# Kyaw-Thiha/animal-vision

Hardware: AMD Instinct MI355X
Metric: megapixels/sec per-frame pipeline (higher is better)
Workload: dtype f16

## Files before the change

### animal-vision_amd/_lib.py

```python
from __future__ import annotations

import ctypes
import os

_HERE = os.path.dirname(os.path.abspath(__file__))
LIB_PATH = os.path.join(_HERE, "libavx.so")

AVX_OK = 0
AVX_ERR_INVALID, AVX_ERR_NO_DEVICE, AVX_ERR_HIP, AVX_ERR_UNSUPPORTED, AVX_ERR_NOMEM = -1, -2, -3, -4, -5
AVX_COLOR_MATRIX, AVX_COLOR_CAT_MERGE = 0, 1
AVX_POST_NONE, AVX_POST_GAUSS, AVX_POST_ROWGAIN, AVX_POST_STREAK = 0, 1, 2, 3
AVX_MAX_KSIZE = 33
AVX_PIX_FMTS = {"yuv420p": 0, "nv12": 1, "yuv422p": 2, "yuv444p": 3, "gray": 4, "yuv420p10le": 5, "yuv422p10le": 6, "yuv444p10le": 7,
                "p010le": 8}
AVX_TRANSFERS = {"pq": 1, "hlg": 2}
AVX_TONEMAPS = {"clip": 0, "mobius": 1}


class AvxError(RuntimeError):
    def __init__(self, code: int, msg: str):
        super().__init__(f"libavx error {code}: {msg}")
        self.code = code


# ... 182 lines not shown
    _fields_ = [("op", ctypes.c_uint8), ("dst", ctypes.c_uint8), ("a", ctypes.c_uint8), ("b", ctypes.c_uint8), ("imm", ctypes.c_uint32)]


class EwPlane(ctypes.Structure):
    _fields_ = [("ptr", ctypes.c_void_p), ("stride", ctypes.c_int32), ("kind", ctypes.c_int32)]


class EwProgram(ctypes.Structure):

    _fields_ = [
        ("struct_size", ctypes.c_uint32),
        ("H", ctypes.c_int32),
        ("W", ctypes.c_int32),
        ("n_insn", ctypes.c_int32),
        ("insn_host", ctypes.POINTER(EwInsn)),
        ("n_planes", ctypes.c_int32),
        ("planes_host", ctypes.POINTER(EwPlane)),
        ("n_acc", ctypes.c_int32),
        ("acc_host", ctypes.POINTER(ctypes.c_int32)),
        ("scalars_dev", ctypes.c_void_p),
        ("n_scalars", ctypes.c_int32),
    ]


AVX_EW_MAX_INSN, AVX_EW_MAX_PLANES, AVX_EW_MAX_REGS, AVX_EW_MAX_ACC = 384, 24, 32, 16
AVX_EW_MAX_FRAMES = 16
_EW_OPS = ("CONST SCALAR LOAD STORE ADD SUB MUL DIV MIN MAX POW ATAN2 NEG ABS SQRT EXP LOG SIN COS FLOOR CEIL CLIP01 TANH "
           "LT LE GT GE EQ AND OR NOT SELECT ACCMIN ACCMAX ACCSUM").split()
EW = {name: i + 1 for i, name in enumerate(_EW_OPS)}
EW_PLANE = {"f32": 0, "u8": 1, "u8_lut": 2, "col": 3, "row": 4, "u8_enc": 5}
EW_ACC = {"min": 0, "max": 1, "sum": 2, "mean": 3}

AVX_MAP = {"falsecolor": 0, "custom_matrix": 1, "opponent": 2, "uv_purple_yellow": 3, "falsecolor_uv_mixed": 4}

if not os.path.exists(LIB_PATH):
    raise ImportError(
        f"{LIB_PATH} not found: build it with `python -c 'import __graft_entry__ as g; g.build()'` "
        "or `make -C animal-vision_amd/csrc` (hipcc --offload-arch=gfx950). There is no CPU fallback."
    )


def _preload_torch_hip_runtime():
    import importlib.util

    try:
        spec = importlib.util.find_spec("torch")
    except (ImportError, ValueError):
        spec = None
    if spec is None or not spec.submodule_search_locations:
        return
    cand = os.path.join(list(spec.submodule_search_locations)[0], "lib", "libamdhip64.so")
    if os.path.exists(cand):
        try:
            ctypes.CDLL(cand, mode=ctypes.RTLD_GLOBAL)
        except OSError:
            pass


_preload_torch_hip_runtime()
lib = ctypes.CDLL(LIB_PATH)

_vp, _i, _sz = ctypes.c_void_p, ctypes.c_int, ctypes.c_size_t
_SIGS = {
    "avx_abi_version": (_i, []),
    "avx_device_count": (_i, []),
    "avx_init": (_i, [_i, ctypes.POINTER(_vp)]),
    "avx_destroy": (None, [_vp]),
    "avx_last_error": (ctypes.c_char_p, [_vp]),
    "avx_malloc": (_i, [_vp, _sz, ctypes.POINTER(_vp)]),
    "avx_free": (_i, [_vp, _vp]),
    "avx_host_alloc": (_i, [_vp, _sz, ctypes.POINTER(_vp)]),
    "avx_host_free": (_i, [_vp, _vp]),
    "avx_memcpy_h2d": (_i, [_vp, _vp, _vp, _sz, _vp]),
    "avx_memcpy_d2h": (_i, [_vp, _vp, _vp, _sz, _vp]),
    "avx_memcpy_d2d": (_i, [_vp, _vp, _vp, _sz, _vp]),
    "avx_memset": (_i, [_vp, _vp, _i, _sz, _vp]),
    "avx_stream_create": (_i, [_vp, ctypes.POINTER(_vp)]),
    "avx_stream_destroy": (_i, [_vp, _vp]),
    "avx_sync": (_i, [_vp, _vp]),
    "avx_stream_wait": (_i, [_vp, _vp, _vp]),
    "avx_device_sync": (_i, [_vp]),
    "avx_timer_start": (_i, [_vp, _vp]),
    "avx_timer_stop": (_i, [_vp, _vp, ctypes.POINTER(ctypes.c_float)]),
    "avx_dichromat_u8": (_i, [_vp, _vp, _vp, _i, _i, _i, ctypes.POINTER(DichromatDesc), _vp]),
    "avx_dichromat_last_launch": (_i, [_vp, ctypes.POINTER(DichromatLaunchInfo)]),
    "avx_get_table": (_i, [_i, _vp, _sz]),
    "avx_percentile": (_i, [_vp, _vp, _sz, ctypes.c_double, ctypes.POINTER(ctypes.c_double), _vp]),
    "avx_spectral_integrate": (_i, [_vp, _vp, _i, _i, _i, _i, _i, _vp, _i, _vp, _vp, _vp]),
    "avx_plane_stats": (_i, [_vp, _vp, _i, _sz, _i, ctypes.c_float, _vp, _vp]),
    "avx_planes_gaussian_blur": (_i, [_vp, _vp, _vp, _i, _i, _i, _i, _vp, _i, _vp]),
    "avx_planes_gaussian_blur_batch": (_i, [_vp, _vp, _sz, _vp, _sz, _i, _i, _i, _i, _i, _vp, _i, _vp]),
    "avx_streak_planes_f32": (_i, [_vp, _vp, _vp, _i, _i, _vp, _i, _vp]),
    "avx_rgb_to_hsi_lobes": (_i, [_vp, _vp, _i, _i, _i, _i, _vp, ctypes.c_float, _vp, _vp]),
    "avx_honeybee_u8": (_i, [_vp, _vp, _vp, _i, _i, _i, ctypes.POINTER(HoneybeeDesc), _vp, _vp]),
    "avx_catch_planes_up": (_i, [_vp, _vp, _i, _i, _vp, _i, _i, _vp, ctypes.POINTER(ctypes.c_int), _vp]),
    "avx_uv_front_u8": (_i, [_vp, _vp, _i, _i, _i, _vp, _vp, _vp]),
    "avx_uv_front_u8_batch": (_i, [_vp, _vp, _i, _sz, _i, _i, _i, _vp, _sz, _vp, _sz, _vp]),
    "avx_panorama_warp_f32": (_i, [_vp, _vp, _i, _i, _i, _vp, _vp]),
    "avx_band_stack": (_i, [_vp, _vp, _i, _i, ctypes.POINTER(BandStackDesc), _vp, _vp]),
    "avx_band_stack_batch": (_i, [_vp, _vp, _i, _sz, _i, _i, ctypes.POINTER(BandStackDesc), _vp, _sz, _vp]),
    "avx_percentile_dev": (_i, [_vp, _vp, _sz, ctypes.c_double, _vp, _vp]),
    "avx_percentiles_dev": (_i, [_vp, _i, ctypes.POINTER(ctypes.c_void_p), ctypes.POINTER(ctypes.c_size_t), ctypes.POINTER(ctypes.c_double),
                                 ctypes.POINTER(ctypes.c_void_p), _vp]),
    "avx_ew_run": (_i, [_vp, ctypes.POINTER(EwProgram), _vp]),
    "avx_ew_run_batch": (_i, [_vp, ctypes.POINTER(EwProgram), _i, ctypes.POINTER(ctypes.c_size_t), _sz, _vp]),
    "avx_ew_spec_stats": (_i, [ctypes.POINTER(ctypes.c_ulonglong), ctypes.POINTER(ctypes.c_ulonglong)]),
    "avx_mantis_u8": (_i, [_vp, _vp, _vp, _vp, _i, _i, ctypes.POINTER(MantisDesc), _vp]),
    "avx_mantis_u8_batch": (_i, [_vp, _vp, _vp, _vp, _i, _i, _i, ctypes.POINTER(MantisDesc), _vp]),
    "avx_resize_hwc": (_i, [_vp, _vp, _i, _i, _i, _i, _vp, _i, _i, _i, _vp]),
    "avx_binocular_warp_u8": (_i, [_vp, _vp, _i, _i, _vp, _vp, _vp, _vp, _vp, _i, _i, _vp, _vp]),
    "avx_cat_wide_u8": (_i, [_vp, _vp, _vp, _i, _i, _i, ctypes.POINTER(DichromatDesc), _vp, _vp, _vp, _vp, _vp, _vp]),
    "avx_center_zoom_u8": (_i, [_vp, _vp, _vp, _i, _i, _i, _i, _i, _i, _i, _vp]),
    "avx_split_compose_u8": (_i, [_vp, _vp, _vp, _vp, _i, _i, _i, _vp]),
    "avx_draw_label_u8": (_i, [_vp, _vp, _i, _i, ctypes.POINTER(ctypes.c_int), _fp, _i, ctypes.c_float, ctypes.c_float, _i, _vp]),
    "avx_gallery_compose_u8": (_i, [_vp, ctypes.POINTER(GalleryTile), _i, _fp, _i, _i, _i, _i, ctypes.POINTER(ctypes.c_int), _vp, _i, _i, _vp]),
    "avx_wall_max_tiles": (_i, []),
    "avx_wall_layout_create": (_i, [_vp, _i, _i, _i, _i, _i, ctypes.POINTER(ctypes.c_int), ctypes.POINTER(ctypes.c_int), _fp, _i, _i, _i, _i,
                                    ctypes.POINTER(ctypes.c_int), ctypes.POINTER(_vp)]),
    "avx_wall_layout_destroy": (_i, [_vp, _vp]),
    "avx_wall_canvas_size": (_i, [_vp, ctypes.POINTER(_i), ctypes.POINTER(_i)]),
    "avx_wall_layout_info": (_i, [_vp, ctypes.POINTER(_i), ctypes.POINTER(_i), ctypes.POINTER(_i), ctypes.POINTER(_sz)]),
    "avx_wall_compose_u8": (_i, [_vp, _vp, ctypes.POINTER(_vp), _sz, _i, _vp, _sz, _vp]),
    "avx_i420_to_rgb_u8": (_i, [_vp, _vp, _vp, _i, _i, _i, _i, _i, _vp]),
    "avx_rgb_to_i420_u8": (_i, [_vp, _vp, _vp, _i, _i, _i, _i, _i, _vp]),
    "avx_yuv_coefficients": (_i, [_i, _i, ctypes.POINTER(ctypes.c_int), ctypes.POINTER(ctypes.c_int)]),
    "avx_yuv_coefficients_d": (_i, [_i, _i, _i, ctypes.POINTER(ctypes.c_int), ctypes.POINTER(ctypes.c_int)]),
    "avx_yuv_frame_size": (_sz, [_i, _i, _i]),
    "avx_yuv_to_rgb_u8": (_i, [_vp, _i, _vp, _vp, _i, _i, _i, _i, _i, _vp]),
    "avx_rgb_to_yuv_u8": (_i, [_vp, _i, _vp, _vp, _i, _i, _i, _i, _i, _vp]),
    "avx_yuv_hdr_to_rgb_u8": (_i, [_vp, _i, _vp, _vp, _i, _i, _i, _i, _i, _i, ctypes.c_double, ctypes.c_double, _vp]),
    "avx_yuv_to_rgb_scaled_u8": (_i, [_vp, _i, _vp, _vp, _i, _i, _i, _i, _i, _i, _i, _vp]),
    "avx_yuv_hdr_to_rgb_scaled_u8": (_i, [_vp, _i, _vp, _vp, _i, _i, _i, _i, _i, _i, _i, _i, ctypes.c_double, ctypes.c_double, _vp]),
    "avx_frame_metrics_u8": (_i, [_vp, _vp, _vp, _i, _i, _i, _i, _vp, _vp]),
    "avx_plane_metrics": (_i, [_vp, _i, _vp, _i, _vp, _i, _i, _i, _i, _vp, _vp]),
    "avx_frame_metrics_ms_u8": (_i, [_vp, _vp, _vp, _i, _i, _i, _vp, _vp, _vp]),
    "avx_diff_map_u8": (_i, [_vp, _vp, _vp, _i, _i, _i, _i, ctypes.c_float, _i, _i, _vp, _vp, _vp, _vp]),
    "avx_delta_e_u8": (_i, [_vp, _vp, _vp, _i, _i, _i, _i, ctypes.c_float, ctypes.c_float, _i, _vp, _vp, _vp, _vp]),
    "avx_scielab_u8": (_i, [_vp, _vp, _vp, _i, _i, _i, ctypes.c_double, _i, ctypes.c_float, ctypes.c_float, _i, _vp, _vp, _vp, _vp]),
    "avx_remap_linear_planes": (_i, [_vp, _vp, _i, _i, _i, _vp, _vp, _vp, ctypes.c_float, _vp]),
    "avx_sobel3_plane": (_i, [_vp, _vp, _i, _i, _vp, _vp, _vp]),
    "avx_mst_gram": (_i, [_vp, _vp, _i, _sz, _i, _i, _vp, _vp, _vp, _vp]),
    "avx_mst_qkv_gram": (_i, [_vp, _vp, _vp, _sz, _i, _vp, _vp, _vp, _vp, _vp]),
    "avx_mst_qkv_gram16": (_i, [_vp, _vp, _vp, _sz, _i, _vp, _vp, _vp, _vp, _vp]),
    "avx_mst_ln_gemm_gelu": (_i, [_vp, _vp, _vp, _vp, ctypes.c_float, _vp, _sz, _i, _vp, _vp]),
    "avx_mst_convt2x2": (_i, [_vp, _vp, _vp, _vp, _vp, _i, _i, _i, _i, _vp]),
    "avx_mst_convt2x2_fuse": (_i, [_vp, _vp, _vp, _vp, _vp, _vp, _vp, _i, _i, _i, _i, _vp]),
    "avx_mst_posemb": (_i, [_vp, _vp, _vp, _vp, _vp, _vp, _vp, _i, _i, _i, _i, _vp]),
    "avx_mst_conv3x3_add": (_i, [_vp, _vp, _vp, _vp, _vp, _i, _i, _i, _i, _vp]),
    "avx_mst_attn_pack": (_i, [_vp, _vp, _vp, _vp, _vp, _vp, _i, _vp, _vp]),
    "avx_mst_rowgemm_add": (_i, [_vp, _vp, _vp, _vp, _vp, _vp, _vp, _sz, _i, _vp]),
    "avx_mst_conv_in_u8": (_i, [_vp, _vp, _i, _i, _i, _i, _i, _i, _vp, _vp, _vp]),
    "avx_mst_conv3x3_lds": (_i, [_vp, _vp, _vp, _vp, _vp, _i, _i, _i, _i, _vp]),
    "avx_mst_down4x4": (_i, [_vp, _vp, _vp, _vp, _i, _i, _i, _i, _vp]),
    "avx_mst_conv3x3_lds_gram": (_i, [_vp, _vp, _vp, _vp, _vp, _i, _i, _i, _vp, _vp, _vp, _vp, _vp]),
    "avx_mst_conv3x3_lds_cin": (_i, [_vp, _vp, _vp, _vp, _i, _i, _i, _i, _i, _i, _vp, _vp, _vp]),
    "avx_mst_conv3x3_lds_spectral_cin": (_i, [_vp, _vp, _vp, _vp, _i, _i, _i, _i, _i, _i, _vp, _fp, _i, _i, _i, _i, _vp, _vp, ctypes.POINTER(ctypes.c_int), _vp]),
    "avx_mst_conv3x3_lds_gram_cin": (_i, [_vp, _vp, _i, _i, _i, _i, _i, _i, _vp, _vp, _vp, _vp, _vp, _vp, _vp, _vp]),
    "avx_mst_convt2x2_fuse_gram": (_i, [_vp, _vp, _vp, _vp, _vp, _vp, _vp, _i, _i, _i, _vp, _vp, _vp, _vp, _vp]),
    "avx_mst_attn_pack16": (_i, [_vp, _vp, _vp, _vp, _vp, _vp, _i, _vp, _vp]),
    "avx_mst_attn_pack_mx": (_i, [_vp, _vp, _vp, _vp, _vp, _vp, _i, _vp, _vp]),
    "avx_mst_attn_tail_mx": (_i, [_vp, _vp, _vp, _vp, _vp, _vp, _vp, _vp, _i, _i, _i, _i, _vp]),
    "avx_mst_attn_tail_sp": (_i, [_vp, _vp, _vp, _vp, _vp, _vp, _vp, _vp, _i, _i, _i, _i, _vp]),
    "avx_mst_attn_tail": (_i, [_vp, _vp, _vp, _vp, _vp, _vp, _vp, _vp, _i, _i, _i, _i, _vp]),
    "avx_mst_attn_tail_x": (_i, [_vp, _vp, _vp, _vp, _vp, _vp, _vp, _vp, _i, _i, _i, _i, _vp]),
    "avx_mst_ffn_fused": (_i, [_vp, _vp, _vp, _vp, ctypes.c_float, _vp, _vp, _vp, _vp, _i, _i, _i, _i, _vp]),
    "avx_mst_conv3x3_lds_spectral": (_i, [_vp, _vp, _vp, _vp, _i, _i, _i, _fp, _i, _i, _i, _i, _vp, _vp, ctypes.POINTER(ctypes.c_int), _vp]),
    "avx_mst_ffn_fused_mx": (_i, [_vp, _vp, _vp, _vp, ctypes.c_float, _vp, _vp, _vp, _vp, _i, _i, _i, _i, _vp]),
    "avx_mst_ffn_fused_sp": (_i, [_vp, _vp, _vp, _vp, ctypes.c_float, _vp, _vp, _vp, _vp, _i, _i, _i, _i, _vp]),
    "avx_mst_ffn_fused_mx_col": (_i, [_vp, _vp, _vp, _vp, ctypes.c_float, _vp, _vp, _vp, _vp, _i, _i, _i, _i, _i, _vp]),
    "avx_mst_ffn_fused_sp_col": (_i, [_vp, _vp, _vp, _vp, ctypes.c_float, _vp, _vp, _vp, _vp, _i, _i, _i, _i, _i, _vp]),
    "avx_mst_gelu_prescale": (ctypes.c_float, []),
    "avx_mst_tile_order": (_i, [_i, _i, _i, _i, _i, ctypes.POINTER(ctypes.c_longlong), _i, ctypes.POINTER(ctypes.c_int)]),
    "avx_mst_tile_order_col": (_i, [_i, _i, _i, _i, ctypes.POINTER(ctypes.c_longlong), ctypes.POINTER(ctypes.c_ubyte), _i, ctypes.POINTER(ctypes.c_int)]),
    "avx_mst_dw_gemm_add": (_i, [_vp, _vp, _vp, _vp, _vp, _vp, _i, _i, _i, _i, _vp]),
    "avx_dwconv3x3_nhwc_add": (_i, [_vp, _vp, _vp, _vp, _i, _i, _i, _i, _i, _vp, _vp, _vp]),
    "avx_dwconv3x3_nhwc": (_i, [_vp, _vp, _vp, _vp, _i, _i, _i, _i, _i, _i, _vp]),
    "avx_layernorm_rows": (_i, [_vp, _vp, _vp, _vp, _vp, _i, _sz, _i, ctypes.c_float, _vp]),
    "avx_layernorm_rows_grouped": (_i, [_vp, _vp, _vp, _vp, _vp, _i, _sz, _i, ctypes.c_float, _i, _i, _vp]),
}
for _name, (_res, _args) in _SIGS.items():
    _fn = getattr(lib, _name)
    _fn.restype = _res
    _fn.argtypes = _args

if lib.avx_abi_version() != 1:
    raise ImportError(f"libavx.so ABI {lib.avx_abi_version()} != 1 expected by this package: rebuild")
```

### animal-vision_amd/csrc/mst_fused.hip

```cpp
#include <hip/hip_fp16.h>

#include <cstdio>
#include <cstdlib>
#include <cstring>

#include "avx_internal.h"
#include "mst_common.h"
#include "mst_tile_order.h"

namespace {

typedef float float4_t __attribute__((ext_vector_type(4)));
#ifndef AVX_FFN32_GM2
#define AVX_FFN32_GM2 1
#endif
constexpr int kFT = 512;
constexpr int TS = 16;
constexpr int HS = TS + 2;
#ifndef AVX_FFN_TH
#define AVX_FFN_TH 16
#endif
constexpr int kFfnTH = AVX_FFN_TH;
static_assert(kFfnTH == 14 || kFfnTH == 16, "FeedForward tile rows");
constexpr int kFfnNGRP = (HS * (kFfnTH + 2) + 31) / 32;
// ... 1201 lines not shown
                for (int k = 0; k < 5; ++k) rraw[k] = (h && k == 4) ? 0u : rraw[k] & 0xffffffu;
                conv_in_mfma(rraw, __builtin_bit_cast(half8_t, cwl[lane]), __builtin_bit_cast(half8_t, cwl[64 + lane]), ar);
            }
            if (ahead.live) {
                if constexpr (CINR) fetch_res(tile_at(ahead, TS, TS));
                if constexpr (CINX) fetch_src(tile_at(ahead, TS, TS));
                else fetch(tile_at(ahead, TS, TS));
            }
            const size_t off = ((t.b * H + (live ? yo : 0)) * (size_t)W + (live ? xo : 0)) * C + 16 * h;
            if constexpr (!CIN) {
                if (add) { ar[0] = reinterpret_cast<const uint4*>(add + off)[0]; ar[1] = reinterpret_cast<const uint4*>(add + off)[1]; }
            }
            float16_t d;
#pragma unroll
            for (int v = 0; v < 16; ++v) d[v] = 0.f;
            const unsigned char* src = xt + (size_t)r * RP + (size_t)c * PP + 16 * h;
#pragma unroll
            for (int tap = 0; tap < 9; ++tap)
#pragma unroll
                for (int s2 = 0; s2 < 2; ++s2)
                    d = mfma16(__builtin_bit_cast(half8_t, wl[(2 * tap + s2) * 64 + lane]), __builtin_bit_cast(half8_t, *reinterpret_cast<const uint4*>(src + (size_t)(tap / 3) * RP + (size_t)(tap % 3) * PP + 32 * s2)), d);
            half8_t o0, o1;
            {
                const half8_t r0 = __builtin_bit_cast(half8_t, ar[0]), r1 = __builtin_bit_cast(half8_t, ar[1]);
#pragma unroll
                for (int v = 0; v < 8; ++v) { o0[v] = (_Float16)(d[v] + (float)r0[v]); o1[v] = (_Float16)(d[8 + v] + (float)r1[v]); }
            }
            if constexpr (SPEC) {
                float a3[3] = {0.f, 0.f, 0.f};
                auto chain = [&]() {
#pragma unroll
                    for (int j = 0; j < 16; ++j) {
                        const float v = (float)(j < 8 ? o0[j] : o1[j - 8]);
                        const float* wb = specw + (16 * h + j) * 4;
#pragma unroll
                        for (int k = 0; k < 3; ++k) a3[k] = __builtin_fmaf(v, wb[k], a3[k]);
                    }
                };
                if (h == 0) chain();
#pragma unroll
                for (int k = 0; k < 3; ++k) { const float lo = __shfl_xor(a3[k], 32); a3[k] = h ? lo : a3[k]; }
                if (h == 1) chain();
                const int yc = yo - crop_t, xc = xo - crop_l;
                if (h == 1 && live && yc >= 0 && yc < Hc && xc >= 0 && xc < Wc) {
#pragma unroll
                    for (int k = 0; k < 3; ++k) {
                        planes[(size_t)k * Hc * Wc + (size_t)yc * Wc + xc] = a3[k];
                        smn[k] = fminf(smn[k], a3[k]); smx[k] = fmaxf(smx[k], a3[k]); ssum[k] += (double)a3[k];
                    }
                }
            } else if (live) {
                reinterpret_cast<uint4*>(out + off)[0] = __builtin_bit_cast(uint4, o0);
                reinterpret_cast<uint4*>(out + off)[1] = __builtin_bit_cast(uint4, o1);
            }
            if constexpr (GRAM) {
                if (!live) { o0 = half8_t{0, 0, 0, 0, 0, 0, 0, 0}; o1 = o0; }
                float16_t dq, dk;
#pragma unroll
                for (int v = 0; v < 16; ++v) { dq[v] = 0.f; dk[v] = 0.f; }
                dq = mfma16(o0, __builtin_bit_cast(half8_t, wq[0 * 64 + lane]), dq);
                dq = mfma16(o1, __builtin_bit_cast(half8_t, wq[1 * 64 + lane]), dq);
                dk = mfma16(o0, __builtin_bit_cast(half8_t, wq[2 * 64 + lane]), dk);
                dk = mfma16(o1, __builtin_bit_cast(half8_t, wq[3 * 64 + lane]), dk);
                unsigned aq[8], ak[8];
#pragma unroll
                for (int j = 0; j < 8; ++j) {
                    aq[j] = pack_f16(dq[2 * j], dq[2 * j + 1]);
                    ak[j] = pack_f16(dk[2 * j], dk[2 * j + 1]);
                    fma_mix_lo(nq, aq[j], aq[j]); fma_mix_hi(nq, aq[j], aq[j]);
                    fma_mix_lo(nk, ak[j], ak[j]); fma_mix_hi(nk, ak[j], ak[j]);
                }
#pragma unroll
                for (int b2 = 0; b2 < 2; ++b2)
                    G = mfma16(__builtin_bit_cast(half8_t, uint4{ak[4 * b2], ak[4 * b2 + 1], ak[4 * b2 + 2], ak[4 * b2 + 3]}),
                               __builtin_bit_cast(half8_t, uint4{aq[4 * b2], aq[4 * b2 + 1], aq[4 * b2 + 2], aq[4 * b2 + 3]}), G);
            }
        }
        if (!ahead.live) break;
        t = tile_at(ahead, TS, TS);
        ahead.advance();
        __syncthreads();
    }
    if constexpr (SPEC) {
        __syncthreads();
        float* redf = reinterpret_cast<float*>(xt);
        double* redd = reinterpret_cast<double*>(xt + 256);
#pragma unroll
        for (int k = 0; k < 3; ++k) {
            float a = smn[k], b2 = smx[k];
            double c2 = ssum[k];
#pragma unroll
            for (int o = 32; o > 0; o >>= 1) { a = fminf(a, __shfl_xor(a, o)); b2 = fmaxf(b2, __shfl_xor(b2, o)); c2 += __shfl_xor(c2, o); }
            if (lane == 0) { redf[(wave * 3 + k) * 2] = a; redf[(wave * 3 + k) * 2 + 1] = b2; redd[wave * 3 + k] = c2; }
        }
        __syncthreads();
        if (tid < 3) {
            float a = 3.4e38f, b2 = -3.4e38f;
            double c2 = 0.0;
            for (int w8 = 0; w8 < 8; ++w8) { a = fminf(a, redf[(w8 * 3 + tid) * 2]); b2 = fmaxf(b2, redf[(w8 * 3 + tid) * 2 + 1]); c2 += redd[w8 * 3 + tid]; }
            spart[(size_t)blockIdx.x * 3 + tid] = SpecStat3{a, b2, c2};
        }
    }
    if constexpr (GRAM) {
        static_assert(sizeof(xt) >= sizeof(float) * 4 * 34 * 32, "the halo tile's LDS holds four waves' results at a time");
        float* red = reinterpret_cast<float*>(xt);
        const float sq = nq + __shfl_xor(nq, 32), sk = nk + __shfl_xor(nk, 32);
        float sum[3] = {0.f, 0.f, 0.f};
#pragma unroll
        for (int half = 0; half < 2; ++half) {
            __syncthreads();
            if ((wave >> 2) == half) {
                float* mine = red + (size_t)(wave & 3) * 34 * 32;
#pragma unroll
                for (int v = 0; v < 16; ++v) mine[(8 * (v / 4) + 4 * h + (v % 4)) * 32 + p] = G[v];
                if (h == 0) { mine[32 * 32 + p] = sq; mine[33 * 32 + p] = sk; }
            }
            __syncthreads();
#pragma unroll
            for (int q = 0; q < 3; ++q) {
                const int i = tid + q * kFT;
                if (i < 34 * 32)
#pragma unroll
                    for (int w4 = 0; w4 < 4; ++w4) sum[q] += red[(size_t)w4 * 34 * 32 + i];
            }
        }
#pragma unroll
        for (int q = 0; q < 3; ++q) {
            const int i = tid + q * kFT;
            if (i < 34 * 32) partial[(size_t)blockIdx.x * 34 * 32 + i] = sum[q];
        }
    }
}


template <int C>
struct DownGeo {
    static constexpr int OH = C == 32 ? 8 : 4, OW = 16, IH = 2 * OH + 2, IW = 2 * OW + 2;
    static constexpr int NP = C / 8;
    static constexpr int RPS = IW * NP + (C == 32 ? 2 : 4);
    static constexpr int NI = ((IH * RPS + 63) / 64 + 7) / 8 * 8;
    static constexpr int PER_WAVE = NI / 8, BUF = NI * 1024, NBUF = C == 32 ? 3 : 2, GROUPS = OH / 2;
    static constexpr int PART = C == 32 ? 0 : 2 * 4 * 4096;
    __device__ static int swz(int col) { return C == 32 ? (col >> 2) & 3 : (col >> 1) & 7; }
};
#pragma clang diagnostic push
#pragma clang diagnostic ignored "-Winline-asm"
__device__ __forceinline__ void lds_dma16(const void* g, unsigned lds_base ) {
    asm volatile("s_mov_b32 m0, %0\n\ts_nop 0\n\tglobal_load_lds_dwordx4 %1, off" ::"s"(__builtin_amdgcn_readfirstlane(lds_base)), "v"(g) : "memory", "m0");
}
__device__ __forceinline__ void lds_dma16(const void* base , unsigned ofs, unsigned lds_base) {
    asm volatile("s_mov_b32 m0, %0\n\ts_nop 0\n\tglobal_load_lds_dwordx4 %1, %2" ::"s"(__builtin_amdgcn_readfirstlane(lds_base)), "v"(ofs), "s"(base) : "memory", "m0");
}
#pragma clang diagnostic pop
template <int C>
__global__ __launch_bounds__(kFT, 2) void k_mst_down4x4_dma(const __half* __restrict__ x , const uint4* __restrict__ wpack ,
                                                            __half* __restrict__ out , const void* __restrict__ zero, int B, int H, int W, int order ) {
    using G = DownGeo<C>;
    constexpr int CO = 2 * C, NT = CO / 32, KS = C / 16;
    __shared__ __align__(1024) unsigned char lds[G::NBUF * G::BUF + G::PART];
    const int tid = threadIdx.x, lane = tid & 63, wave = __builtin_amdgcn_readfirstlane(tid >> 6) , p = lane & 31, h = lane >> 5;
    const int g0 = C == 32 ? wave & 3 : 0, nt = C == 32 ? wave >> 2 : wave & 3, kh = C == 32 ? 0 : wave >> 2;
    half8_t wf[32];
#pragma unroll
    for (int i = 0; i < 32; ++i) {
        const int tap = C == 32 ? i >> 1 : 8 * kh + (i >> 2), s2 = C == 32 ? i & 1 : i & 3;
        wf[i] = __builtin_bit_cast(half8_t, wpack[((size_t)(tap * NT + nt) * KS + s2) * 64 + lane]);
    }
    const int Ho = H / 2, Wo = W / 2;
    const int tx = (Wo + G::OW - 1) / G::OW, ty = (Ho + G::OH - 1) / G::OH;
    struct T2 { int ox0, oy0, b; };
    auto tile_at = [&](const TileWalk& w) { return T2{w.xi * G::OW, w.yi * G::OH, w.b}; };
    int rel[G::PER_WAVE], rc[G::PER_WAVE];
#pragma unroll
    for (int k = 0; k < G::PER_WAVE; ++k) {
        const int L = (wave + 8 * k) * 64 + lane, row = L / G::RPS, rem = L - row * G::RPS, col = rem / G::NP, j = (rem - col * G::NP) ^ G::swz(col);
        const bool inside = row < G::IH && col < G::IW;
        rel[k] = inside ? (row * W + col) * (C * 2) + 16 * j : 0;
        rc[k] = inside ? row << 8 | col : -1;
    }
    const unsigned lds0 = __builtin_amdgcn_readfirstlane((unsigned)(size_t)(__attribute__((address_space(3))) unsigned char*)lds);
    auto fill = [&](const TileWalk& w, int slot) {
        const bool exists = w.live;
        const T2 t = tile_at(w);
        const int y0 = 2 * t.oy0 - 1, x0 = 2 * t.ox0 - 1;
        const char* origin = reinterpret_cast<const char*>(x) + (((long)t.b * H + y0) * W + x0) * (long)(C * 2);
        const unsigned lb = lds0 + slot * G::BUF + wave * 1024;
        if (exists && y0 >= 0 && y0 + G::IH <= H && x0 >= 0 && x0 + G::IW <= W) {
#pragma unroll
            for (int k = 0; k < G::PER_WAVE; ++k) lds_dma16(origin , (unsigned)rel[k], lb + k * 8192);
        } else {
#pragma unroll
            for (int k = 0; k < G::PER_WAVE; ++k) {
                const int yy = y0 + (rc[k] >> 8), xx = x0 + (rc[k] & 255);
                const bool ok = exists && rc[k] >= 0 && yy >= 0 && yy < H && xx >= 0 && xx < W;
                lds_dma16(ok ? (const void*)(origin + rel[k]) : zero, lb + k * 8192);
            }
        }
    };
    TileWalk walk, look;
    walk.init(blockIdx.x, gridDim.x, B, ty, tx, order);
    if (!walk.live) return;
    look = walk;
#pragma unroll
    for (int a = 0; a < G::NBUF - 1; ++a) { fill(look, a); look.advance(); }
    const int c2 = 2 * (p & 15);
    int colofs[4];
#pragma unroll
    for (int kx = 0; kx < 4; ++kx) colofs[kx] = (c2 + kx) * G::NP;
    int slot = 0, plain_stores = 0;
    for (;;) {
        if (plain_stores == G::NBUF - 1 && (C == 32 || kh == 0)) asm volatile("s_waitcnt vmcnt(%0)" ::"n"(G::PER_WAVE * (G::NBUF - 2) + 2 * (C == 32 ? 1 : G::GROUPS) * (G::NBUF - 1)) : "memory");
        else asm volatile("s_waitcnt vmcnt(%0)" ::"n"(G::PER_WAVE * (G::NBUF - 2)) : "memory");
        __syncthreads();
        {
            int nslot = slot + G::NBUF - 1;
            nslot -= nslot >= G::NBUF ? G::NBUF : 0;
            fill(look, nslot);
            look.advance();
        }
        const T2 t = tile_at(walk);
        const bool whole = t.oy0 + G::OH <= Ho && t.ox0 + G::OW <= Wo;
        const unsigned char* bt = lds + slot * G::BUF;
#pragma unroll 1
        for (int g = g0; g < (C == 32 ? g0 + 1 : G::GROUPS); ++g) {
            const int r = 2 * g + (p >> 4);
            float16_t d, d1;
#pragma unroll
            for (int v = 0; v < 16; ++v) d[v] = 0.f, d1[v] = 0.f;
            const unsigned char* src = bt + (size_t)(2 * r) * (G::RPS * 16);
            auto frag = [&](int i) {
                const int tap = C == 32 ? i >> 1 : 8 * kh + (i >> 2), s2 = C == 32 ? i & 1 : i & 3, ky = tap >> 2, kx = tap & 3;
                return *reinterpret_cast<const uint4*>(src + ky * (G::RPS * 16) + (colofs[kx] + ((2 * s2 + h) ^ G::swz(c2 + kx))) * 16);
            };
            constexpr int AHEAD = 6;
            uint4 bq[AHEAD];
#pragma unroll
            for (int i = 0; i < AHEAD; ++i) bq[i] = frag(i);
#pragma unroll
            for (int i = 0; i < 32; ++i) {
                if (i & 1) d1 = mfma16(wf[i], __builtin_bit_cast(half8_t, bq[i % AHEAD]), d1);
                else d = mfma16(wf[i], __builtin_bit_cast(half8_t, bq[i % AHEAD]), d);
                if (i + AHEAD < 32) bq[i % AHEAD] = frag(i + AHEAD);
            }
            __builtin_amdgcn_sched_group_barrier(0x100, AHEAD, 0);
#pragma unroll
            for (int i = 0; i < 32; ++i) {
                __builtin_amdgcn_sched_group_barrier(0x008, 1, 0);
                if (i + AHEAD < 32) __builtin_amdgcn_sched_group_barrier(0x100, 1, 0);
            }
#pragma unroll
            for (int v = 0; v < 16; ++v) d[v] += d1[v];
            if constexpr (C == 64) {
                float4* part = reinterpret_cast<float4*>(lds + G::NBUF * G::BUF + ((g & 1) * 4 + nt) * 4096);
                if (kh == 1) {
#pragma unroll
                    for (int v4 = 0; v4 < 4; ++v4) part[v4 * 64 + lane] = float4{d[4 * v4], d[4 * v4 + 1], d[4 * v4 + 2], d[4 * v4 + 3]};
                }
                __syncthreads();
                if (kh == 1) continue;
#pragma unroll
                for (int v4 = 0; v4 < 4; ++v4) {
                    const float4 q = part[v4 * 64 + lane];
                    d[4 * v4] += q.x; d[4 * v4 + 1] += q.y; d[4 * v4 + 2] += q.z; d[4 * v4 + 3] += q.w;
                }
            }
            const int yo = t.oy0 + r, xo = t.ox0 + (p & 15);
            half8_t o0, o1;
#pragma unroll
            for (int v = 0; v < 8; ++v) { o0[v] = (_Float16)d[v]; o1[v] = (_Float16)d[8 + v]; }
            __half* dst = out + (((size_t)t.b * Ho + yo) * Wo + xo) * CO + 32 * nt + 16 * h;
            if (whole) {
                reinterpret_cast<uint4*>(dst)[0] = __builtin_bit_cast(uint4, o0);
                reinterpret_cast<uint4*>(dst)[1] = __builtin_bit_cast(uint4, o1);
            } else if (yo < Ho && xo < Wo) {
                reinterpret_cast<uint4*>(dst)[0] = __builtin_bit_cast(uint4, o0);
                reinterpret_cast<uint4*>(dst)[1] = __builtin_bit_cast(uint4, o1);
            }
        }
        plain_stores = whole ? (plain_stores < G::NBUF - 1 ? plain_stores + 1 : plain_stores) : 0;
        walk.advance();
        if (!walk.live) break;
        slot = slot + 1 == G::NBUF ? 0 : slot + 1;
    }
    asm volatile("s_waitcnt vmcnt(0)" ::: "memory");
}

__global__ __launch_bounds__(256) void k_mst_conv_in_u8(const uint8_t* __restrict__ frame , const float* __restrict__ w ,
                                                        __half* __restrict__ out , int H, int W, int pt, int pl, int Hp, int Wp) {
    __shared__ __align__(16) float wl[27 * 32];
    for (int i = threadIdx.x; i < 27 * 32; i += 256) wl[i] = w[i];
    __syncthreads();
    const size_t total = (size_t)Hp * Wp;
    for (size_t i = (size_t)blockIdx.x * 256 + threadIdx.x; i < total; i += (size_t)gridDim.x * 256) {
        const int y = (int)(i / Wp), x = (int)(i - (size_t)y * Wp);
        float in[27];
#pragma unroll
        for (int t = 0; t < 9; ++t) {
            const int yy = y + t / 3 - 1, xx = x + t % 3 - 1;
            const bool ok = yy >= 0 && yy < Hp && xx >= 0 && xx < Wp;
            int sy = (ok ? yy : 0) - pt, sx = (ok ? xx : 0) - pl;
            sy = sy < 0 ? -sy : (sy >= H ? 2 * (H - 1) - sy : sy);
            sx = sx < 0 ? -sx : (sx >= W ? 2 * (W - 1) - sx : sx);
            const uint8_t* q = frame + ((size_t)sy * W + sx) * 3;
#pragma unroll
            for (int c = 0; c < 3; ++c) in[3 * t + c] = ok ? (float)(_Float16)((float)q[c] / 255.0f) : 0.f;
        }
        uint4* dst = reinterpret_cast<uint4*>(out + i * 32);
#pragma unroll 1
        for (int v = 0; v < 4; ++v) {
            float acc[8];
#pragma unroll
            for (int j = 0; j < 8; ++j) acc[j] = 0.f;
#pragma unroll
            for (int k = 0; k < 27; ++k) {
                const float4 wa = *reinterpret_cast<const float4*>(wl + k * 32 + 8 * v), wb = *reinterpret_cast<const float4*>(wl + k * 32 + 8 * v + 4);
                acc[0] = __builtin_fmaf(in[k], wa.x, acc[0]); acc[1] = __builtin_fmaf(in[k], wa.y, acc[1]);
                acc[2] = __builtin_fmaf(in[k], wa.z, acc[2]); acc[3] = __builtin_fmaf(in[k], wa.w, acc[3]);
                acc[4] = __builtin_fmaf(in[k], wb.x, acc[4]); acc[5] = __builtin_fmaf(in[k], wb.y, acc[5]);
                acc[6] = __builtin_fmaf(in[k], wb.z, acc[6]); acc[7] = __builtin_fmaf(in[k], wb.w, acc[7]);
            }
            half8_t o8;
#pragma unroll
            for (int j = 0; j < 8; ++j) o8[j] = (_Float16)acc[j];
            dst[v] = __builtin_bit_cast(uint4, o8);
        }
    }
}

__global__ __launch_bounds__(256) void k_mst_conv_in_u8_mfma(const uint8_t* __restrict__ frame , const float* __restrict__ w ,
                                                             __half* __restrict__ out , int H, int W, int pt, int pl, int Hp, int Wp) {
    const int lane = threadIdx.x & 63, p = lane & 31, h = lane >> 5;
    const half8_t a0 = conv_in_afrag(w, lane, 0), a1 = conv_in_afrag(w, lane, 1);
    const ConvInFrame cf{frame, H, W, pt, pl, Hp, Wp};
    const size_t total = (size_t)Hp * Wp, ngroups = (total + 31) / 32;
    for (size_t g = (size_t)blockIdx.x * 4 + (threadIdx.x >> 6); g < ngroups; g += (size_t)gridDim.x * 4) {
        const size_t i = g * 32 + p, ic = i < total ? i : total - 1;
        const int y = (int)(ic / Wp), x = (int)(ic - (size_t)y * Wp);
        unsigned raw[5];
        conv_in_fetch(cf, y, x, h, raw);
        uint4 o[2];
        conv_in_mfma(raw, a0, a1, o);
        if (i < total) {
            reinterpret_cast<uint4*>(out + i * 32 + 16 * h)[0] = o[0];
            reinterpret_cast<uint4*>(out + i * 32 + 16 * h)[1] = o[1];
        }
    }
}

}

static int ffn_fused_launch(avx_ctx* ctx, const void* x, const float* gamma, const float* beta, float eps, const void* w1pack, const void* taps_9xhid, const void* dwpack,
                            const void* w2pack, void* out, int B, int H, int W, int C, void* stream, bool sparse = false, bool march = false, int max_workgroups = 0);

extern "C" float avx_mst_gelu_prescale(void) { return kGeluPrescale; }

extern "C" int avx_mst_tile_order(int frames, int ty, int tx, int nwg, int raster, long long* visit, int steps_cap, int* steps_out) {
    if (frames <= 0 || ty <= 0 || tx <= 0 || nwg <= 0 || (visit && steps_cap <= 0) || (long long)frames * ty * tx > 0x7fffffffll) return AVX_ERR_INVALID;
    int most = 0;
    for (int wg = 0; wg < nwg; ++wg) {
        TileWalk wk;
        wk.init((unsigned)wg, (unsigned)nwg, frames, ty, tx, raster ? AVX_TILE_ORDER_RASTER : AVX_TILE_ORDER_XCD);
        int k = 0;
        for (; wk.live; wk.advance(), ++k)
            if (visit && k < steps_cap) visit[(size_t)wg * steps_cap + k] = ((long long)wk.b * ty + wk.yi) * tx + wk.xi;
        if (visit)
            for (int r = k; r < steps_cap; ++r) visit[(size_t)wg * steps_cap + r] = -1;
        most = k > most ? k : most;
    }
    if (steps_out) *steps_out = most;
    return AVX_OK;
}

extern "C" int avx_mst_tile_order_col(int frames, int ty, int tx, int nwg, long long* visit, unsigned char* seg, int steps_cap, int* steps_out) {
    if (frames <= 0 || ty <= 0 || tx <= 0 || nwg <= 0 || ((visit || seg) && steps_cap <= 0) || (long long)frames * ty * tx > 0x7fffffffll) return AVX_ERR_INVALID;
    int most = 0;
    for (int wg = 0; wg < nwg; ++wg) {
        ColumnWalk wk;
        wk.init((unsigned)wg, (unsigned)nwg, frames, ty, tx);
        int k = 0;
        for (; wk.live; wk.advance(), ++k)
            if (k < steps_cap) {
                if (visit) visit[(size_t)wg * steps_cap + k] = ((long long)wk.b * ty + wk.yi) * tx + wk.xi;
                if (seg) seg[(size_t)wg * steps_cap + k] = wk.seg ? 1 : 0;
            }
        for (int r = k; r < steps_cap; ++r) {
            if (visit) visit[(size_t)wg * steps_cap + r] = -1;
            if (seg) seg[(size_t)wg * steps_cap + r] = 0;
        }
        most = k > most ? k : most;
    }
    if (steps_out) *steps_out = most;
    return AVX_OK;
}

extern "C" int avx_mst_ffn_fused(avx_ctx* ctx, const void* x, const float* gamma, const float* beta, float eps, const void* w1pack, const void* taps_9xhid,
                                 const void* w2pack, void* out, int B, int H, int W, int C, void* stream) {
    if (!ctx) return AVX_ERR_INVALID;
    AVX_REQUIRE(ctx, taps_9xhid, "avx_mst_ffn_fused: NULL pointer");
    return ffn_fused_launch(ctx, x, gamma, beta, eps, w1pack, taps_9xhid, nullptr, w2pack, out, B, H, W, C, stream);
}

extern "C" int avx_mst_ffn_fused_mx(avx_ctx* ctx, const void* x, const float* gamma, const float* beta, float eps, const void* w1pack, const void* dwpack,
                                    const void* w2pack, void* out, int B, int H, int W, int C, void* stream) {
    if (!ctx) return AVX_ERR_INVALID;
    AVX_REQUIRE(ctx, dwpack && (((uintptr_t)dwpack) & 15u) == 0, "avx_mst_ffn_fused_mx: dwpack NULL or not 16-byte aligned");
    return ffn_fused_launch(ctx, x, gamma, beta, eps, w1pack, nullptr, dwpack, w2pack, out, B, H, W, C, stream);
}

extern "C" int avx_mst_ffn_fused_sp(avx_ctx* ctx, const void* x, const float* gamma, const float* beta, float eps, const void* w1pack, const void* dwpack,
                                    const void* w2pack, void* out, int B, int H, int W, int C, void* stream) {
    if (!ctx) return AVX_ERR_INVALID;
    AVX_REQUIRE(ctx, dwpack && (((uintptr_t)dwpack) & 15u) == 0, "avx_mst_ffn_fused_sp: dwpack NULL or not 16-byte aligned");
    return ffn_fused_launch(ctx, x, gamma, beta, eps, w1pack, nullptr, dwpack, w2pack, out, B, H, W, C, stream, true);
}

extern "C" int avx_mst_ffn_fused_mx_col(avx_ctx* ctx, const void* x, const float* gamma, const float* beta, float eps, const void* w1pack, const void* dwpack,
                                        const void* w2pack, void* out, int B, int H, int W, int C, int max_workgroups, void* stream) {
    if (!ctx) return AVX_ERR_INVALID;
    AVX_REQUIRE(ctx, dwpack && (((uintptr_t)dwpack) & 15u) == 0, "avx_mst_ffn_fused_mx_col: dwpack NULL or not 16-byte aligned");
    AVX_REQUIRE(ctx, (C == 32 || C == 64) && max_workgroups >= 0, "avx_mst_ffn_fused_mx_col: C=%d (32 or 64), max_workgroups=%d (>= 0)", C, max_workgroups);
    return ffn_fused_launch(ctx, x, gamma, beta, eps, w1pack, nullptr, dwpack, w2pack, out, B, H, W, C, stream, false, true, max_workgroups);
}
extern "C" int avx_mst_ffn_fused_sp_col(avx_ctx* ctx, const void* x, const float* gamma, const float* beta, float eps, const void* w1pack, const void* dwpack,
                                        const void* w2pack, void* out, int B, int H, int W, int C, int max_workgroups, void* stream) {
    if (!ctx) return AVX_ERR_INVALID;
    AVX_REQUIRE(ctx, dwpack && (((uintptr_t)dwpack) & 15u) == 0, "avx_mst_ffn_fused_sp_col: dwpack NULL or not 16-byte aligned");
    AVX_REQUIRE(ctx, (C == 32 || C == 64) && max_workgroups >= 0, "avx_mst_ffn_fused_sp_col: C=%d (32 or 64), max_workgroups=%d (>= 0)", C, max_workgroups);
    return ffn_fused_launch(ctx, x, gamma, beta, eps, w1pack, nullptr, dwpack, w2pack, out, B, H, W, C, stream, true, true, max_workgroups);
}

static int ffn_fused_launch(avx_ctx* ctx, const void* x, const float* gamma, const float* beta, float eps, const void* w1pack, const void* taps_9xhid, const void* dwpack,
                            const void* w2pack, void* out, int B, int H, int W, int C, void* stream, bool sparse, bool march, int max_workgroups) {
    AVX_REQUIRE(ctx, x && gamma && beta && w1pack && w2pack && out && B > 0 && H > 0 && W > 0, "avx_mst_ffn_fused: NULL pointer or empty tensor");
    AVX_REQUIRE(ctx, C == 32 || C == 64 || C == 128, "avx_mst_ffn_fused: C=%d (32, 64 or 128: 31-channel groups stored 32 wide)", C);
    AVX_REQUIRE(ctx, ((((uintptr_t)x | (uintptr_t)w1pack | (uintptr_t)w2pack | (uintptr_t)out | (uintptr_t)taps_9xhid)) & 15u) == 0,
                "avx_mst_ffn_fused: pointers must be 16-byte aligned");
    AVX_REQUIRE(ctx, x != out, "avx_mst_ffn_fused: neighbouring tiles read each other's halo: the output cannot be the input");
// ... 175 lines not shown
extern "C" int avx_mst_conv3x3_lds_gram(avx_ctx* ctx, const void* x, const void* wpack16, const void* add, void* out, int H, int W, int C, const void* wqk16, float* gram,
                                        float* nq, float* nk, void* stream) {
    if (!ctx) return AVX_ERR_INVALID;
    AVX_REQUIRE(ctx, x && wpack16 && out && wqk16 && gram && nq && nk && H > 0 && W > 0, "avx_mst_conv3x3_lds_gram: NULL pointer or empty tensor");
    AVX_REQUIRE(ctx, C == 32, "avx_mst_conv3x3_lds_gram: C=%d (32: the 31-channel full-resolution convs)", C);
    AVX_REQUIRE(ctx, ((((uintptr_t)x | (uintptr_t)wpack16 | (uintptr_t)add | (uintptr_t)out | (uintptr_t)wqk16)) & 15u) == 0, "avx_mst_conv3x3_lds_gram: pointers must be 16-byte aligned");
    AVX_REQUIRE(ctx, x != out, "avx_mst_conv3x3_lds_gram: in-place convolution is not possible");
    AVX_HIP(ctx, hipSetDevice(ctx->device));
    hipStream_t s = avx_pick_stream(ctx, stream);
    avx_ws* ws = avx_workspace(ctx, s);
    if (!ws) return AVX_ERR_NOMEM;
    const long total = (long)((H + TS - 1) / TS) * ((W + TS - 1) / TS);
    const long cap = (long)ctx->num_cus * 2;
    const long blocks = total < cap ? total : cap;
    int rc = avx_ensure_scratch(ctx, ws, sizeof(float) * (size_t)blocks * 34 * 32);
    if (rc) return rc;
    float* partial = (float*)ws->d_scratch;
    hipLaunchKernelGGL((k_mst_conv3x3_lds<4, true>), dim3((unsigned)blocks), dim3(kFT), 0, s, (const __half*)x, (const uint4*)wpack16, (const __half*)add, (__half*)out, 1, H, W,
                       (const uint4*)wqk16, partial);
    AVX_HIP(ctx, hipGetLastError());
    return avx_mst_qkv_final_launch(ctx, partial, (int)blocks, 1, gram, nq, nk, s);
}

extern "C" int avx_mst_conv_in_u8(avx_ctx* ctx, const uint8_t* frame_hwc, int H, int W, int pad_top, int pad_bottom, int pad_left, int pad_right,
                                  const float* w_27x32_dev, void* out, void* stream) {
    if (!ctx) return AVX_ERR_INVALID;
    AVX_REQUIRE(ctx, frame_hwc && w_27x32_dev && out && H > 1 && W > 1, "avx_mst_conv_in_u8: NULL pointer or a frame too small to reflect");
    AVX_REQUIRE(ctx, pad_top >= 0 && pad_bottom >= 0 && pad_left >= 0 && pad_right >= 0 && pad_top < H && pad_bottom < H && pad_left < W && pad_right < W,
                "avx_mst_conv_in_u8: reflect padding must be smaller than the frame");
    AVX_REQUIRE(ctx, ((uintptr_t)out & 15u) == 0, "avx_mst_conv_in_u8: out must be 16-byte aligned");
    AVX_HIP(ctx, hipSetDevice(ctx->device));
    hipStream_t s = avx_pick_stream(ctx, stream);
    const int Hp = H + pad_top + pad_bottom, Wp = W + pad_left + pad_right;
    const size_t total = (size_t)Hp * Wp;
    const size_t want = (total + 255) / 256, cap = (size_t)ctx->num_cus * 16;
    if (getenv("AVX_MST_CONV_IN_VALU"))
        hipLaunchKernelGGL(k_mst_conv_in_u8, dim3((unsigned)(want < cap ? want : cap)), dim3(256), 0, s, frame_hwc, w_27x32_dev, (__half*)out, H, W, pad_top, pad_left, Hp, Wp);
    else {
        const size_t wantm = (total + 127) / 128;
        hipLaunchKernelGGL(k_mst_conv_in_u8_mfma, dim3((unsigned)(wantm < cap ? wantm : cap)), dim3(256), 0, s, frame_hwc, w_27x32_dev, (__half*)out, H, W, pad_top,
                           pad_left, Hp, Wp);
    }
    AVX_HIP(ctx, hipGetLastError());
    return AVX_OK;
}

static int conv_in_frame_check(avx_ctx* ctx, const char* fn, const uint8_t* frame_hwc, int H, int W, int pad_top, int pad_bottom, int pad_left, int pad_right, const float* w_27x32_dev,
                               ConvInFrame* cf) {
    AVX_REQUIRE(ctx, frame_hwc && w_27x32_dev && H > 1 && W > 1, "%s: NULL pointer or a frame too small to reflect", fn);
    AVX_REQUIRE(ctx, pad_top >= 0 && pad_bottom >= 0 && pad_left >= 0 && pad_right >= 0 && pad_top < H && pad_bottom < H && pad_left < W && pad_right < W,
                "%s: reflect padding must be smaller than the frame", fn);
    AVX_REQUIRE(ctx, (long)(H + pad_top + pad_bottom) * (W + pad_left + pad_right) * 3 < (1l << 31), "%s: frame larger than 2 GiB", fn);
    *cf = ConvInFrame{frame_hwc, H, W, pad_top, pad_left, H + pad_top + pad_bottom, W + pad_left + pad_right};
    return AVX_OK;
}

extern "C" int avx_mst_conv3x3_lds_cin(avx_ctx* ctx, const void* x, const void* wpack16, const uint8_t* frame_hwc, int H, int W, int pad_top, int pad_bottom, int pad_left,
                                       int pad_right, const float* w_27x32_dev, void* out, void* stream) {
    if (!ctx) return AVX_ERR_INVALID;
    AVX_REQUIRE(ctx, x && wpack16 && out, "avx_mst_conv3x3_lds_cin: NULL pointer");
    ConvInFrame cf;
    int rc = conv_in_frame_check(ctx, "avx_mst_conv3x3_lds_cin", frame_hwc, H, W, pad_top, pad_bottom, pad_left, pad_right, w_27x32_dev, &cf);
    if (rc) return rc;
    AVX_REQUIRE(ctx, ((((uintptr_t)x | (uintptr_t)wpack16 | (uintptr_t)out)) & 15u) == 0, "avx_mst_conv3x3_lds_cin: pointers must be 16-byte aligned");
    AVX_REQUIRE(ctx, x != out, "avx_mst_conv3x3_lds_cin: in-place convolution is not possible");
    AVX_HIP(ctx, hipSetDevice(ctx->device));
    hipStream_t s = avx_pick_stream(ctx, stream);
    const long total = (long)((cf.Hp + TS - 1) / TS) * ((cf.Wp + TS - 1) / TS);
    const long cap = (long)ctx->num_cus * 3;
    hipLaunchKernelGGL((k_mst_conv3x3_lds<6, false, false, true>), dim3((unsigned)(total < cap ? total : cap)), dim3(kFT), 0, s, (const __half*)x, (const uint4*)wpack16, (const __half*)nullptr,
                       (__half*)out, 1, cf.Hp, cf.Wp, (const uint4*)nullptr, (float*)nullptr, (const float*)nullptr, (float*)nullptr, (SpecStat3*)nullptr, 0, 0, 0, 0, mst_tile_order(), cf,
                       w_27x32_dev);
    AVX_HIP(ctx, hipGetLastError());
    return AVX_OK;
}

extern "C" int avx_mst_conv3x3_lds_spectral_cin(avx_ctx* ctx, const void* x, const void* wpack16, const uint8_t* frame_hwc, int H, int W, int pad_top, int pad_bottom, int pad_left,
                                                int pad_right, const float* w_27x32_dev, const float* weights_host, int crop_t, int crop_l, int Hc, int Wc, float* planes_out,
                                                void* partials_out, int* n_partials, void* stream) {
    if (!ctx) return AVX_ERR_INVALID;
    AVX_REQUIRE(ctx, x && wpack16 && weights_host && planes_out && partials_out && n_partials, "avx_mst_conv3x3_lds_spectral_cin: NULL pointer");
    ConvInFrame cf;
    int rc = conv_in_frame_check(ctx, "avx_mst_conv3x3_lds_spectral_cin", frame_hwc, H, W, pad_top, pad_bottom, pad_left, pad_right, w_27x32_dev, &cf);
    if (rc) return rc;
    AVX_REQUIRE(ctx, crop_t >= 0 && crop_l >= 0 && Hc > 0 && Wc > 0 && crop_t + Hc <= cf.Hp && crop_l + Wc <= cf.Wp, "avx_mst_conv3x3_lds_spectral_cin: the crop window must lie inside the padded frame");
    AVX_REQUIRE(ctx, ((((uintptr_t)x | (uintptr_t)wpack16 | (uintptr_t)partials_out)) & 15u) == 0, "avx_mst_conv3x3_lds_spectral_cin: pointers must be 16-byte aligned");
    AVX_HIP(ctx, hipSetDevice(ctx->device));
    hipStream_t s = avx_pick_stream(ctx, stream);
    avx_ws* ws = avx_workspace(ctx, s);
    if (!ws) return AVX_ERR_NOMEM;
    float wT[32 * 4];
    for (int b = 0; b < 32; ++b)
        for (int k = 0; k < 4; ++k) wT[b * 4 + k] = k < 3 ? weights_host[(size_t)k * 32 + b] : 0.0f;
    float* dwT = nullptr;
    rc = avx_const_upload(ctx, ws, 2, wT, sizeof(wT), s, (void**)&dwT);
    if (rc) return rc;
    const long total = (long)((cf.Hp + TS - 1) / TS) * ((cf.Wp + TS - 1) / TS);
    const long cap = (long)ctx->num_cus * 2;
    const long blocks = total < cap ? total : cap;
    *n_partials = (int)blocks;
    hipLaunchKernelGGL((k_mst_conv3x3_lds<4, false, true, true>), dim3((unsigned)blocks), dim3(kFT), 0, s, (const __half*)x, (const uint4*)wpack16, (const __half*)nullptr, (__half*)nullptr, 1,
                       cf.Hp, cf.Wp, (const uint4*)nullptr, (float*)nullptr, (const float*)dwT, planes_out, (SpecStat3*)partials_out, crop_t, crop_l, Hc, Wc, (int)AVX_TILE_ORDER_RASTER, cf,
                       w_27x32_dev);
    AVX_HIP(ctx, hipGetLastError());
    return AVX_OK;
}

extern "C" int avx_mst_conv3x3_lds_gram_cin(avx_ctx* ctx, const uint8_t* frame_hwc, int H, int W, int pad_top, int pad_bottom, int pad_left, int pad_right, const float* w_27x32_dev,
                                            const void* wpack16, void* out, const void* wqk16, float* gram, float* nq, float* nk, void* stream) {
    if (!ctx) return AVX_ERR_INVALID;
    AVX_REQUIRE(ctx, wpack16 && out && wqk16 && gram && nq && nk, "avx_mst_conv3x3_lds_gram_cin: NULL pointer");
    ConvInFrame cf;
    int rc = conv_in_frame_check(ctx, "avx_mst_conv3x3_lds_gram_cin", frame_hwc, H, W, pad_top, pad_bottom, pad_left, pad_right, w_27x32_dev, &cf);
    if (rc) return rc;
    AVX_REQUIRE(ctx, ((((uintptr_t)wpack16 | (uintptr_t)out | (uintptr_t)wqk16)) & 15u) == 0, "avx_mst_conv3x3_lds_gram_cin: pointers must be 16-byte aligned");
    AVX_HIP(ctx, hipSetDevice(ctx->device));
    hipStream_t s = avx_pick_stream(ctx, stream);
    avx_ws* ws = avx_workspace(ctx, s);
    if (!ws) return AVX_ERR_NOMEM;
    const long total = (long)((cf.Hp + TS - 1) / TS) * ((cf.Wp + TS - 1) / TS);
    const long cap = (long)ctx->num_cus * 2;
    const long blocks = total < cap ? total : cap;
    rc = avx_ensure_scratch(ctx, ws, sizeof(float) * (size_t)blocks * 34 * 32);
    if (rc) return rc;
    float* partial = (float*)ws->d_scratch;
    hipLaunchKernelGGL((k_mst_conv3x3_lds<4, true, false, false, true>), dim3((unsigned)blocks), dim3(kFT), 0, s, (const __half*)nullptr, (const uint4*)wpack16, (const __half*)nullptr, (__half*)out, 1,
                       cf.Hp, cf.Wp, (const uint4*)wqk16, partial, (const float*)nullptr, (float*)nullptr, (SpecStat3*)nullptr, 0, 0, 0, 0, (int)AVX_TILE_ORDER_RASTER, cf, w_27x32_dev);
    AVX_HIP(ctx, hipGetLastError());
    return avx_mst_qkv_final_launch(ctx, partial, (int)blocks, 1, gram, nq, nk, s);
}

extern "C" int avx_mst_down4x4(avx_ctx* ctx, const void* x, const void* wpack16, void* out, int B, int H, int W, int C, void* stream) {
    if (!ctx) return AVX_ERR_INVALID;
    AVX_REQUIRE(ctx, x && wpack16 && out && B > 0 && H > 0 && W > 0, "avx_mst_down4x4: NULL pointer or empty tensor");
    AVX_REQUIRE(ctx, C == 32 || C == 64, "avx_mst_down4x4: C=%d (32 or 64: the encoder steps 31 -> 62 and 62 -> 124 channels as stored)", C);
    AVX_REQUIRE(ctx, H % 2 == 0 && W % 2 == 0, "avx_mst_down4x4: H and W must be even (the model pads frames to multiples of 8)");
    AVX_REQUIRE(ctx, (long)B * H * W * C * 2 < (1l << 31), "avx_mst_down4x4: input larger than 2 GiB");
    AVX_REQUIRE(ctx, ((((uintptr_t)x | (uintptr_t)wpack16 | (uintptr_t)out)) & 15u) == 0, "avx_mst_down4x4: pointers must be 16-byte aligned");
    AVX_HIP(ctx, hipSetDevice(ctx->device));
    hipStream_t s = avx_pick_stream(ctx, stream);
    const long cap = (long)ctx->num_cus;
    if (C == 32) {
        using G = DownGeo<32>;
        const long total = (long)B * ((H / 2 + G::OH - 1) / G::OH) * ((W / 2 + G::OW - 1) / G::OW);
        hipLaunchKernelGGL(k_mst_down4x4_dma<32>, dim3((unsigned)(total < cap ? total : cap)), dim3(kFT), 0, s, (const __half*)x, (const uint4*)wpack16, (__half*)out, (const void*)ctx->d_zero, B, H, W, mst_tile_order());
    } else {
        using G = DownGeo<64>;
        const long total = (long)B * ((H / 2 + G::OH - 1) / G::OH) * ((W / 2 + G::OW - 1) / G::OW);
        hipLaunchKernelGGL(k_mst_down4x4_dma<64>, dim3((unsigned)(total < cap ? total : cap)), dim3(kFT), 0, s, (const __half*)x, (const uint4*)wpack16, (__half*)out, (const void*)ctx->d_zero, B, H, W, mst_tile_order());
    }
    AVX_HIP(ctx, hipGetLastError());
    return AVX_OK;
}
```

### animal-vision_amd/csrc/mst_mfma.hip

```cpp
#include <hip/hip_fp16.h>

#include "avx_internal.h"
#include "mst_common.h"

namespace {

constexpr int kT = 256;

__device__ __forceinline__ float16_t mfma(half4_t a, half4_t b, float16_t c) { return __builtin_amdgcn_mfma_f32_32x32x8f16(a, b, c, 0, 0, 0); }
__device__ __forceinline__ float16_t mfma16(half8_t a, half8_t b, float16_t c) { return __builtin_amdgcn_mfma_f32_32x32x16_f16(a, b, c, 0, 0, 0); }

template <int C>
__device__ __forceinline__ void load_x(const __half* __restrict__ x, size_t tile, size_t n, int lane, half4_t (&xf)[C / 8]) {
    const int p = lane & 31, h = lane >> 5;
    const size_t row = tile * 32 + p;
    if (row < n) {
        const uint4* src = reinterpret_cast<const uint4*>(x + row * (size_t)C + h * (C / 2));
#pragma unroll
        for (int q = 0; q < C / 16; ++q) {
            const uint4 v = src[q];
            const half8_t h8 = __builtin_bit_cast(half8_t, v);
            xf[2 * q] = half4_t{h8[0], h8[1], h8[2], h8[3]};
            xf[2 * q + 1] = half4_t{h8[4], h8[5], h8[6], h8[7]};
        }
// ... 464 lines not shown
        }
#pragma unroll
        for (int t = 0; t < NT; ++t) {
            float16_t d;
#pragma unroll
            for (int v = 0; v < 16; ++v) d[v] = 0.f;
#pragma unroll
            for (int tap = 0; tap < 9; ++tap)
#pragma unroll
                for (int s = 0; s < KS; ++s) d = mfma(__builtin_bit_cast(half4_t, wl[((tap * NT + t) * KS + s) * 64 + lane]), xf[tap][s], d);
            if (xw < W) {
                const size_t off = ((b * H + y) * (size_t)W + xw) * C + 32 * t + 16 * h;
                half8_t r0 = {0, 0, 0, 0, 0, 0, 0, 0}, r1 = r0;
                if (add) {
                    r0 = __builtin_bit_cast(half8_t, reinterpret_cast<const uint4*>(add + off)[0]);
                    r1 = __builtin_bit_cast(half8_t, reinterpret_cast<const uint4*>(add + off)[1]);
                }
                _Float16 o[16];
#pragma unroll
                for (int v = 0; v < 8; ++v) { o[v] = (_Float16)(d[v] + (float)r0[v]); o[8 + v] = (_Float16)(d[8 + v] + (float)r1[v]); }
                store_tile16(out + off, o);
            }
        }
    }
}

template <int C, int TH, int TW>
__global__ __launch_bounds__(kT) void k_mst_posemb(const __half* __restrict__ v, const float* __restrict__ w1 , const float* __restrict__ w2 ,
                                                   const __half* __restrict__ res, const float* __restrict__ bias , __half* __restrict__ out, int B, int H,
                                                   int W) {
    constexpr int CV = C / 8, PH = TH + 2, PW = TW + 2;
    static_assert(PH % 2 == 0 && kT % CV == 0, "row pairs in phase 1; fixed channel group per thread");
    extern __shared__ __align__(16) unsigned char smem[];
    __half* wl = reinterpret_cast<__half*>(smem);
    float* bl = reinterpret_cast<float*>(wl + 2 * 9 * C);
    unsigned char* mid = reinterpret_cast<unsigned char*>(bl + C);
    const int tid = threadIdx.x;
    for (int i = tid; i < 9 * C; i += kT) { const int c = i / 9, t = i - 9 * c; wl[t * C + c] = __float2half(w1[i]); wl[9 * C + t * C + c] = __float2half(w2[i]); }
    for (int i = tid; i < C; i += kT) bl[i] = bias ? bias[i] : 0.f;
    const int tx = (W + TW - 1) / TW, ty = (H + TH - 1) / TH;
    const long total = (long)B * ty * tx;
    const int cg = tid % CV;
    auto taps = [&](const __half* wbase, uint4 (&wt)[9]) {
#pragma unroll
        for (int t = 0; t < 9; ++t) wt[t] = *reinterpret_cast<const uint4*>(wbase + t * C + cg * 8);
    };
    auto mac8 = [&](float (&acc)[8], const uint4& hv, const uint4& wv) {
        fma_mix_lo(acc[0], hv.x, wv.x); fma_mix_hi(acc[1], hv.x, wv.x);
        fma_mix_lo(acc[2], hv.y, wv.y); fma_mix_hi(acc[3], hv.y, wv.y);
        fma_mix_lo(acc[4], hv.z, wv.z); fma_mix_hi(acc[5], hv.z, wv.z);
        fma_mix_lo(acc[6], hv.w, wv.w); fma_mix_hi(acc[7], hv.w, wv.w);
    };
    __syncthreads();
    for (long tile = blockIdx.x; tile < total; tile += gridDim.x) {
        const int x0 = (int)(tile % tx) * TW, y0 = (int)((tile / tx) % ty) * TH;
        const long b = tile / ((long)tx * ty);
        const bool interior = y0 >= 2 && y0 + TH + 2 <= H && x0 >= 2 && x0 + TW + 2 <= W;
        __syncthreads();
        uint4 wt1[9];
        taps(wl, wt1);
#pragma unroll 1
        for (int it = tid; it < (PH / 2) * PW * CV; it += kT) {
            const int pp = it / CV, c = pp % PW, r = 2 * (pp / PW);
            const int yy = y0 - 1 + r, xx = x0 - 1 + c;
            uint4 raw[4][3];
            if (interior) {
                const __half* base = v + ((b * H + yy - 1) * (size_t)W + xx - 1) * C + cg * 8;
#pragma unroll
                for (int rr = 0; rr < 4; ++rr)
#pragma unroll
                    for (int kx = 0; kx < 3; ++kx) raw[rr][kx] = *reinterpret_cast<const uint4*>(base + ((size_t)rr * W + kx) * C);
            } else {
#pragma unroll
                for (int rr = 0; rr < 4; ++rr)
#pragma unroll
                    for (int kx = 0; kx < 3; ++kx) {
                        const int y2 = yy - 1 + rr, x2 = xx + kx - 1;
                        const bool ok = y2 >= 0 && y2 < H && x2 >= 0 && x2 < W;
                        const int yc = y2 < 0 ? 0 : (y2 >= H ? H - 1 : y2), xc = x2 < 0 ? 0 : (x2 >= W ? W - 1 : x2);
                        uint4 rw = *reinterpret_cast<const uint4*>(v + ((b * H + yc) * (size_t)W + xc) * C + cg * 8);
                        rw.x = ok ? rw.x : 0u; rw.y = ok ? rw.y : 0u; rw.z = ok ? rw.z : 0u; rw.w = ok ? rw.w : 0u;
                        raw[rr][kx] = rw;
                    }
            }
            float acc[2][8];
#pragma unroll
            for (int o2 = 0; o2 < 2; ++o2)
#pragma unroll
                for (int q = 0; q < 8; ++q) acc[o2][q] = 0.f;
#pragma unroll
            for (int rr = 0; rr < 4; ++rr)
#pragma unroll
                for (int kx = 0; kx < 3; ++kx)
#pragma unroll
                    for (int o2 = 0; o2 < 2; ++o2) {
                        const int ky = rr - o2;
                        if (ky < 0 || ky > 2) continue;
                        mac8(acc[o2], raw[rr][kx], wt1[ky * 3 + kx]);
                    }
#pragma unroll
            for (int o2 = 0; o2 < 2; ++o2) {
                const int ym = yy + o2;
                const bool inside = interior || (ym >= 0 && ym < H && xx >= 0 && xx < W);
                unsigned o[4];
#pragma unroll
                for (int q = 0; q < 4; ++q) {
                    const float2_t g = gelu_fast2(float2_t{acc[o2][2 * q], acc[o2][2 * q + 1]});
                    o[q] = inside ? pack_f16(g.x, g.y) : 0u;
                }
                *reinterpret_cast<uint4*>(mid + (((size_t)(r + o2) * PW + c) * C + cg * 8) * 2) = uint4{o[0], o[1], o[2], o[3]};
            }
        }
        __syncthreads();
        uint4 wt2[9];
        taps(wl + 9 * C, wt2);
#pragma unroll 1
        for (int it = tid; it < TH * TW * CV; it += kT) {
            const int pp = it / CV, c = pp % TW, r = pp / TW;
            const int yo = y0 + r, xo = x0 + c;
            if (yo >= H || xo >= W) continue;
            float acc[8];
#pragma unroll
            for (int q = 0; q < 8; ++q) acc[q] = 0.f;
#pragma unroll
            for (int t = 0; t < 9; ++t) mac8(acc, *reinterpret_cast<const uint4*>(mid + (((size_t)(r + t / 3) * PW + c + t % 3) * C + cg * 8) * 2), wt2[t]);
            const size_t off = ((b * H + yo) * (size_t)W + xo) * C + cg * 8;
            uint4 rr = uint4{0u, 0u, 0u, 0u};
            if (res) rr = *reinterpret_cast<const uint4*>(res + off);
            const unsigned rw[4] = {rr.x, rr.y, rr.z, rr.w};
            unsigned o[4];
#pragma unroll
            for (int q = 0; q < 4; ++q) {
                float s0 = acc[2 * q], s1 = acc[2 * q + 1];
                fma_mix_lo(s0, rw[q], 0x3c003c00u); fma_mix_hi(s1, rw[q], 0x3c003c00u);
                o[q] = pack_f16(s0 + bl[cg * 8 + 2 * q], s1 + bl[cg * 8 + 2 * q + 1]);
            }
            *reinterpret_cast<uint4*>(out + off) = uint4{o[0], o[1], o[2], o[3]};
        }
    }
}

template <int C, int TH, int TW>
int launch_posemb(avx_ctx* ctx, const void* v, const float* w1, const float* w2, const void* res, const float* bias, void* out, int B, int H, int W, hipStream_t s) {
    const size_t lds = sizeof(__half) * 2 * 9 * C + sizeof(float) * C + (size_t)(TH + 2) * (TW + 2) * C * 2;
    const long total = (long)B * ((H + TH - 1) / TH) * ((W + TW - 1) / TW);
    const long cap = (long)ctx->num_cus * (lds > 40 * 1024 ? 3 : 5);
    auto k = k_mst_posemb<C, TH, TW>;
    AVX_HIP(ctx, hipFuncSetAttribute((const void*)k, hipFuncAttributeMaxDynamicSharedMemorySize, (int)lds));
    hipLaunchKernelGGL(k, dim3((unsigned)(total < cap ? total : cap)), dim3(kT), lds, s, (const __half*)v, w1, w2, (const __half*)res, bias, (__half*)out, B, H, W);
    AVX_HIP(ctx, hipGetLastError());
    return AVX_OK;
}

template <int C, bool GRAM = false>
__global__ __launch_bounds__(kT) void k_mst_convt2x2(const __half* __restrict__ x , const uint2* __restrict__ wpack ,
                                                     const float* __restrict__ bias , const __half* __restrict__ skip ,
                                                     const uint2* __restrict__ wskip , __half* __restrict__ out , int B,
                                                     int H, int W, const uint4* __restrict__ wqk = nullptr , float* __restrict__ partial = nullptr ) {
    constexpr int KS = C / 8, CO = C / 2, NT = CO / 32, KSS = CO / 8;
    static_assert(!GRAM || C == 64, "the Gram epilogue is for the 32-channel output level");
    extern __shared__ __align__(16) unsigned char smem[];
    uint2* wl = reinterpret_cast<uint2*>(smem);
    float* bl = reinterpret_cast<float*>(smem + (size_t)4 * NT * KS * 64 * sizeof(uint2));
    uint2* wsl = reinterpret_cast<uint2*>(bl + CO);
    uint4* wq = reinterpret_cast<uint4*>(wsl + NT * KSS * 64);
    const int tid = threadIdx.x, lane = tid & 63, wave = tid >> 6;
    for (int i = tid; i < 4 * NT * KS * 64; i += kT) wl[i] = wpack[i];
    for (int i = tid; i < CO; i += kT) bl[i] = bias[i];
    if (skip)
        for (int i = tid; i < NT * KSS * 64; i += kT) wsl[i] = wskip[i];
    float16_t G;
    float nq = 0.f, nk = 0.f;
    if constexpr (GRAM) {
        for (int i = tid; i < 4 * 64; i += kT) wq[i] = wqk[i];
#pragma unroll
        for (int v = 0; v < 16; ++v) G[v] = 0.f;
    }
    __syncthreads();
    const int xt = (W + 31) / 32;
    const long total = (long)B * H * xt;
    const int p = lane & 31, h = lane >> 5;
    for (long tile = (long)blockIdx.x * 4 + wave; tile < total; tile += (long)gridDim.x * 4) {
        const int x0 = (int)(tile % xt) * 32, y = (int)((tile / xt) % H);
        const long b = tile / ((long)xt * H);
        const int xw = x0 + p;
        half4_t xf[KS];
        {
            const size_t row = (size_t)((b * H + y) * (long)W + (xw < W ? xw : W - 1));
            const uint4* src = reinterpret_cast<const uint4*>(x + row * C + h * (C / 2));
#pragma unroll
            for (int q = 0; q < C / 16; ++q) {
                const half8_t h8 = __builtin_bit_cast(half8_t, src[q]);
                xf[2 * q] = half4_t{h8[0], h8[1], h8[2], h8[3]};
                xf[2 * q + 1] = half4_t{h8[4], h8[5], h8[6], h8[7]};
            }
        }
        if constexpr (C > 64) asm volatile("" ::: "memory");
#pragma unroll
        for (int tap = 0; tap < 4; ++tap) {
            const size_t opix = ((size_t)(b * 2 * H + 2 * y + (tap >> 1)) * (size_t)(2 * W) + (size_t)(2 * (xw < W ? xw : W - 1) + (tap & 1)));
            half4_t sf[KSS];
            if (skip) {
                const uint4* src = reinterpret_cast<const uint4*>(skip + opix * CO + h * (CO / 2));
#pragma unroll
                for (int q = 0; q < CO / 16; ++q) {
                    const half8_t h8 = __builtin_bit_cast(half8_t, src[q]);
                    sf[2 * q] = half4_t{h8[0], h8[1], h8[2], h8[3]};
                    sf[2 * q + 1] = half4_t{h8[4], h8[5], h8[6], h8[7]};
                }
            }
#pragma unroll
            for (int t = 0; t < NT; ++t) {
                float16_t d;
#pragma unroll
                for (int v = 0; v < 16; ++v) d[v] = 0.f;
#pragma unroll
                for (int s = 0; s < KS; ++s) d = mfma(__builtin_bit_cast(half4_t, wl[((tap * NT + t) * KS + s) * 64 + lane]), xf[s], d);
                if (skip) {
#pragma unroll
                    for (int s = 0; s < KSS; ++s) d = mfma(__builtin_bit_cast(half4_t, wsl[(t * KSS + s) * 64 + lane]), sf[s], d);
                }
                _Float16 o[16];
#pragma unroll
                for (int v = 0; v < 16; ++v) o[v] = (_Float16)(d[v] + bl[32 * t + 16 * h + v]);
                if (xw < W) store_tile16(out + opix * CO + 32 * t + 16 * h, o);
                if constexpr (GRAM) {
                    half8_t o0, o1;
#pragma unroll
                    for (int v = 0; v < 8; ++v) { o0[v] = xw < W ? o[v] : (_Float16)0.f; o1[v] = xw < W ? o[8 + v] : (_Float16)0.f; }
                    float16_t dq, dk;
#pragma unroll
                    for (int v = 0; v < 16; ++v) { dq[v] = 0.f; dk[v] = 0.f; }
                    dq = mfma16(o0, __builtin_bit_cast(half8_t, wq[0 * 64 + lane]), dq);
                    dq = mfma16(o1, __builtin_bit_cast(half8_t, wq[1 * 64 + lane]), dq);
                    dk = mfma16(o0, __builtin_bit_cast(half8_t, wq[2 * 64 + lane]), dk);
                    dk = mfma16(o1, __builtin_bit_cast(half8_t, wq[3 * 64 + lane]), dk);
                    unsigned aq[8], ak[8];
#pragma unroll
                    for (int j = 0; j < 8; ++j) {
                        aq[j] = pack_f16(dq[2 * j], dq[2 * j + 1]);
                        ak[j] = pack_f16(dk[2 * j], dk[2 * j + 1]);
                        fma_mix_lo(nq, aq[j], aq[j]); fma_mix_hi(nq, aq[j], aq[j]);
                        fma_mix_lo(nk, ak[j], ak[j]); fma_mix_hi(nk, ak[j], ak[j]);
                    }
#pragma unroll
                    for (int b2 = 0; b2 < 2; ++b2)
                        G = mfma16(__builtin_bit_cast(half8_t, uint4{ak[4 * b2], ak[4 * b2 + 1], ak[4 * b2 + 2], ak[4 * b2 + 3]}),
                                   __builtin_bit_cast(half8_t, uint4{aq[4 * b2], aq[4 * b2 + 1], aq[4 * b2 + 2], aq[4 * b2 + 3]}), G);
                }
            }
        }
    }
    if constexpr (GRAM) {
        __syncthreads();
        float* red = reinterpret_cast<float*>(smem);
        float* mine = red + (size_t)wave * 34 * 32;
#pragma unroll
        for (int v = 0; v < 16; ++v) mine[(8 * (v / 4) + 4 * h + (v % 4)) * 32 + p] = G[v];
        const float sq = nq + __shfl_xor(nq, 32), sk = nk + __shfl_xor(nk, 32);
        if (h == 0) { mine[32 * 32 + p] = sq; mine[33 * 32 + p] = sk; }
        __syncthreads();
        for (int i = tid; i < 34 * 32; i += kT) {
            float sum = 0.f;
#pragma unroll
            for (int w4 = 0; w4 < 4; ++w4) sum += red[(size_t)w4 * 34 * 32 + i];
            partial[(size_t)blockIdx.x * 34 * 32 + i] = sum;
        }
    }
}

template <int C, int NW>
__global__ __launch_bounds__(64 * NW) void k_mst_qkv16(const __half* __restrict__ x, const uint4* __restrict__ wpack , size_t n,
                                                      __half* __restrict__ v_out , float* __restrict__ partial ) {
    constexpr int KS = C / 16, HD = C / 32, NT = 3 * HD;
    extern __shared__ __align__(16) unsigned char smem[];
    uint4* wl = reinterpret_cast<uint4*>(smem);
    const int tid = threadIdx.x, lane = tid & 63, wave = tid >> 6;
    for (int i = tid; i < NT * KS * 64; i += 64 * NW) wl[i] = wpack[i];
    __syncthreads();
    auto W = [&](int t, int s) { return __builtin_bit_cast(half8_t, wl[(t * KS + s) * 64 + lane]); };
    float16_t G[HD];
    float nq[HD], nk[HD];
#pragma unroll
    for (int hd = 0; hd < HD; ++hd) {
#pragma unroll
        for (int v = 0; v < 16; ++v) G[hd][v] = 0.f;
        nq[hd] = 0.f;
        nk[hd] = 0.f;
    }
    const size_t ntiles = (n + 31) / 32;
    const int p = lane & 31, h = lane >> 5;
    auto load_row = [&](size_t tile, uint4 (&u)[KS]) {
        const size_t row = tile * 32 + p;
        const uint4* src = reinterpret_cast<const uint4*>(x + (row < n ? row : n - 1) * (size_t)C + h * (C / 2));
#pragma unroll
        for (int q = 0; q < KS; ++q) u[q] = src[q];
    };
    constexpr bool PF = C <= 64;
    uint4 xn[KS];
    size_t tile = (size_t)blockIdx.x * NW + wave;
    if (PF && tile < ntiles) load_row(tile, xn);
    for (; tile < ntiles; tile += (size_t)gridDim.x * NW) {
        const size_t row = tile * 32 + p;
        half8_t xf[KS];
        if (!PF) load_row(tile, xn);
#pragma unroll
        for (int q = 0; q < KS; ++q) xf[q] = __builtin_bit_cast(half8_t, row < n ? xn[q] : uint4{0u, 0u, 0u, 0u});
        if (PF && tile + (size_t)gridDim.x * NW < ntiles) load_row(tile + (size_t)gridDim.x * NW, xn);
        if constexpr (C > 32) asm volatile("" ::: "memory");
#pragma unroll
        for (int hd = 0; hd < HD; ++hd) {
            float16_t dq, dk;
#pragma unroll
            for (int v = 0; v < 16; ++v) { dq[v] = 0.f; dk[v] = 0.f; }
#pragma unroll
            for (int s = 0; s < KS; ++s) dq = mfma16(xf[s], W(hd, s), dq);
#pragma unroll
            for (int s = 0; s < KS; ++s) dk = mfma16(xf[s], W(HD + hd, s), dk);
            unsigned aq[8], ak[8];
#pragma unroll
            for (int j = 0; j < 8; ++j) {
                aq[j] = pack_f16(dq[2 * j], dq[2 * j + 1]);
                ak[j] = pack_f16(dk[2 * j], dk[2 * j + 1]);
                fma_mix_lo(nq[hd], aq[j], aq[j]); fma_mix_hi(nq[hd], aq[j], aq[j]);
                fma_mix_lo(nk[hd], ak[j], ak[j]); fma_mix_hi(nk[hd], ak[j], ak[j]);
            }
#pragma unroll
            for (int b2 = 0; b2 < 2; ++b2)
                G[hd] = mfma16(__builtin_bit_cast(half8_t, uint4{ak[4 * b2], ak[4 * b2 + 1], ak[4 * b2 + 2], ak[4 * b2 + 3]}),
                               __builtin_bit_cast(half8_t, uint4{aq[4 * b2], aq[4 * b2 + 1], aq[4 * b2 + 2], aq[4 * b2 + 3]}), G[hd]);
        }
        if (v_out)
#pragma unroll
        for (int hd = 0; hd < HD; ++hd) {
            float16_t dv;
#pragma unroll
            for (int v = 0; v < 16; ++v) dv[v] = 0.f;
#pragma unroll
            for (int s = 0; s < KS; ++s) dv = mfma16(W(2 * HD + hd, s), xf[s], dv);
            if (row < n) {
                unsigned o[8];
#pragma unroll
                for (int v = 0; v < 8; ++v) o[v] = pack_f16(dv[2 * v], dv[2 * v + 1]);
                uint4* dst = reinterpret_cast<uint4*>(v_out + row * (size_t)C + 32 * hd + 16 * h);
                dst[0] = uint4{o[0], o[1], o[2], o[3]};
                dst[1] = uint4{o[4], o[5], o[6], o[7]};
            }
        }
    }
    __syncthreads();
    float* red = reinterpret_cast<float*>(smem);
#pragma unroll
    for (int hd = 0; hd < HD; ++hd) {
        float* mine = red + ((size_t)wave * HD + hd) * 34 * 32;
#pragma unroll
        for (int v = 0; v < 16; ++v) mine[(8 * (v / 4) + 4 * h + (v % 4)) * 32 + p] = G[hd][v];
        const float sq = nq[hd] + __shfl_xor(nq[hd], 32), sk = nk[hd] + __shfl_xor(nk[hd], 32);
        if (h == 0) { mine[32 * 32 + p] = sq; mine[33 * 32 + p] = sk; }
    }
    __syncthreads();
    for (int i = tid; i < HD * 34 * 32; i += 64 * NW) {
        float s = 0.f;
#pragma unroll
        for (int w = 0; w < NW; ++w) s += red[(size_t)w * HD * 34 * 32 + i];
        partial[(size_t)blockIdx.x * HD * 34 * 32 + i] = s;
    }
}

template <int C, int NW>
int launch_qkv16(avx_ctx* ctx, avx_ws* ws, const void* x, const void* wpack, size_t n, void* v_out, float* gram, float* nq, float* nk, hipStream_t s) {
    constexpr int KS = C / 16, HD = C / 32;
    const size_t wbytes = (size_t)3 * HD * KS * 64 * sizeof(uint4), rbytes = sizeof(float) * NW * HD * 34 * 32;
    const size_t lds = wbytes > rbytes ? wbytes : rbytes;
    const size_t ntiles = (n + 31) / 32;
    long blocks = (long)((ntiles + NW - 1) / NW);
    long per_cu = (long)(160 * 1024 / lds);
    if (per_cu > 16 / NW * 2) per_cu = 16 / NW * 2;
    if (per_cu < 1) per_cu = 1;
    const long cap = (long)ctx->num_cus * per_cu;
    if (blocks > cap) blocks = cap;
    int rc = avx_ensure_scratch(ctx, ws, sizeof(float) * (size_t)blocks * HD * 34 * 32);
    if (rc) return rc;
    float* partial = (float*)ws->d_scratch;
    auto k = k_mst_qkv16<C, NW>;
    AVX_HIP(ctx, hipFuncSetAttribute((const void*)k, hipFuncAttributeMaxDynamicSharedMemorySize, (int)lds));
    hipLaunchKernelGGL(k, dim3((unsigned)blocks), dim3(64 * NW), lds, s, (const __half*)x, (const uint4*)wpack, n, (__half*)v_out, partial);
    AVX_HIP(ctx, hipGetLastError());
    const int tot = HD * 34 * 32;
    hipLaunchKernelGGL(k_mst_qkv_final, dim3((tot / 4 * 64 + 255) / 256), dim3(256), 0, s, partial, (int)blocks, HD, gram, nq, nk);
    AVX_HIP(ctx, hipGetLastError());
    return AVX_OK;
}

template <int C>
int launch_qkv(avx_ctx* ctx, avx_ws* ws, const void* x, const void* wpack, size_t n, void* v_out, float* gram, float* nq, float* nk, hipStream_t s) {
    constexpr int KS = C / 8, HD = C / 32;
    const size_t wbytes = (size_t)3 * HD * KS * 64 * sizeof(uint2), rbytes = sizeof(float) * 4 * HD * 34 * 32;
    const size_t lds = wbytes > rbytes ? wbytes : rbytes;
    const size_t ntiles = (n + 31) / 32;
    long blocks = (long)((ntiles + 3) / 4);
    const long cap = (long)ctx->num_cus * (lds > 64 * 1024 ? 1 : (lds > 32 * 1024 ? 2 : 4));
    if (blocks > cap) blocks = cap;
    int rc = avx_ensure_scratch(ctx, ws, sizeof(float) * (size_t)blocks * HD * 34 * 32);
    if (rc) return rc;
    float* partial = (float*)ws->d_scratch;
    auto k = k_mst_qkv<C>;
    AVX_HIP(ctx, hipFuncSetAttribute((const void*)k, hipFuncAttributeMaxDynamicSharedMemorySize, (int)lds));
    hipLaunchKernelGGL(k, dim3((unsigned)blocks), dim3(kT), lds, s, (const __half*)x, (const uint2*)wpack, n, (__half*)v_out, partial);
    AVX_HIP(ctx, hipGetLastError());
    const int tot = HD * 34 * 32;
    hipLaunchKernelGGL(k_mst_qkv_final, dim3((tot / 4 * 64 + 255) / 256), dim3(256), 0, s, partial, (int)blocks, HD, gram, nq, nk);
    AVX_HIP(ctx, hipGetLastError());
    return AVX_OK;
}

template <int C>
int launch_ffn1(avx_ctx* ctx, const void* x, const float* gamma, const float* beta, float eps, const void* wpack, size_t n, void* out, hipStream_t s) {
    constexpr int KS = C / 8, HD = C / 32;
    const size_t lds = (size_t)4 * HD * KS * 64 * sizeof(uint2) + sizeof(float) * 2 * C;
    const size_t ntiles = (n + 31) / 32;
    long blocks = (long)((ntiles + 3) / 4);
    const long cap = (long)ctx->num_cus * (lds > 64 * 1024 ? 1 : (lds > 32 * 1024 ? 2 : 8));
    if (blocks > cap) blocks = cap;
    auto k = k_mst_ffn1<C>;
    AVX_HIP(ctx, hipFuncSetAttribute((const void*)k, hipFuncAttributeMaxDynamicSharedMemorySize, (int)lds));
    hipLaunchKernelGGL(k, dim3((unsigned)blocks), dim3(kT), lds, s, (const __half*)x, gamma, beta, eps, (const uint2*)wpack, n, (__half*)out);
    AVX_HIP(ctx, hipGetLastError());
    return AVX_OK;
}

template <int C, int ROWS, int PXT, bool PF, int MINW>
int launch_ffn2(avx_ctx* ctx, const void* hid, const float* w9, const void* w2pack, const void* res, void* out, int B, int H, int W, hipStream_t s) {
    constexpr int C4 = 4 * C, KS2 = C4 / 8, NT = C / 32, PITCH = C4 * 2 + 16;
    const size_t lds = (size_t)NT * KS2 * 64 * sizeof(uint2) + sizeof(float) * 9 * C4 + (size_t)ROWS * 32 * PXT * PITCH;
    const long total = (long)B * ((H + ROWS - 1) / ROWS) * ((W + 32 * PXT - 1) / (32 * PXT));
    const long cap = (long)ctx->num_cus * MINW;
    auto k = k_mst_ffn2<C, ROWS, PXT, PF, MINW>;
    AVX_HIP(ctx, hipFuncSetAttribute((const void*)k, hipFuncAttributeMaxDynamicSharedMemorySize, (int)lds));
    hipLaunchKernelGGL(k, dim3((unsigned)(total < cap ? total : cap)), dim3(kT), lds, s, (const __half*)hid, w9, (const uint2*)w2pack, (const __half*)res,
                       (__half*)out, B, H, W);
    AVX_HIP(ctx, hipGetLastError());
    return AVX_OK;
}

}

int avx_mst_qkv_final_launch(avx_ctx* ctx, const float* partial, int blocks, int heads, float* gram, float* nq, float* nk, hipStream_t s) {
    const int tot = heads * 34 * 32;
    hipLaunchKernelGGL(k_mst_qkv_final, dim3((tot / 4 * 64 + 255) / 256), dim3(256), 0, s, partial, blocks, heads, gram, nq, nk);
    AVX_HIP(ctx, hipGetLastError());
    return AVX_OK;
}

extern "C" {

int avx_mst_qkv_gram(avx_ctx* ctx, const void* x, const void* wpack, size_t n_pix, int C, void* v_out, float* gram, float* nq, float* nk, void* stream) {
    if (!ctx) return AVX_ERR_INVALID;
    AVX_REQUIRE(ctx, x && wpack && gram && nq && nk && n_pix > 0, "avx_mst_qkv_gram: NULL pointer or empty tensor");
    AVX_REQUIRE(ctx, C == 32 || C == 64 || C == 128, "avx_mst_qkv_gram: C=%d (32, 64 or 128: 31-channel groups stored 32 wide)", C);
    AVX_REQUIRE(ctx, ((((uintptr_t)x | (uintptr_t)wpack | (uintptr_t)v_out)) & 15u) == 0, "avx_mst_qkv_gram: pointers must be 16-byte aligned");
    AVX_HIP(ctx, hipSetDevice(ctx->device));
    hipStream_t s = avx_pick_stream(ctx, stream);
    avx_ws* ws = avx_workspace(ctx, s);
    if (!ws) return AVX_ERR_NOMEM;
    if (C == 32) return launch_qkv<32>(ctx, ws, x, wpack, n_pix, v_out, gram, nq, nk, s);
    if (C == 64) return launch_qkv<64>(ctx, ws, x, wpack, n_pix, v_out, gram, nq, nk, s);
    return launch_qkv<128>(ctx, ws, x, wpack, n_pix, v_out, gram, nq, nk, s);
}

int avx_mst_qkv_gram16(avx_ctx* ctx, const void* x, const void* wpack16, size_t n_pix, int C, void* v_out, float* gram, float* nq, float* nk, void* stream) {
    if (!ctx) return AVX_ERR_INVALID;
    AVX_REQUIRE(ctx, x && wpack16 && gram && nq && nk && n_pix > 0, "avx_mst_qkv_gram16: NULL pointer or empty tensor");
    AVX_REQUIRE(ctx, C == 32 || C == 64 || C == 128, "avx_mst_qkv_gram16: C=%d (32, 64 or 128: 31-channel groups stored 32 wide)", C);
    AVX_REQUIRE(ctx, ((((uintptr_t)x | (uintptr_t)wpack16 | (uintptr_t)v_out)) & 15u) == 0, "avx_mst_qkv_gram16: pointers must be 16-byte aligned");
    AVX_HIP(ctx, hipSetDevice(ctx->device));
    hipStream_t s = avx_pick_stream(ctx, stream);
    avx_ws* ws = avx_workspace(ctx, s);
    if (!ws) return AVX_ERR_NOMEM;
    if (C == 32) return launch_qkv16<32, 4>(ctx, ws, x, wpack16, n_pix, v_out, gram, nq, nk, s);
    if (C == 64) return launch_qkv16<64, 4>(ctx, ws, x, wpack16, n_pix, v_out, gram, nq, nk, s);
    return launch_qkv16<128, 8>(ctx, ws, x, wpack16, n_pix, v_out, gram, nq, nk, s);
}

int avx_mst_ln_gemm_gelu(avx_ctx* ctx, const void* x, const float* gamma, const float* beta, float eps, const void* wpack, size_t rows, int C, void* out,
                         void* stream) {
    if (!ctx) return AVX_ERR_INVALID;
    AVX_REQUIRE(ctx, x && gamma && beta && wpack && out && rows > 0, "avx_mst_ln_gemm_gelu: NULL pointer or empty tensor");
    AVX_REQUIRE(ctx, C == 32 || C == 64 || C == 128, "avx_mst_ln_gemm_gelu: C=%d (32, 64 or 128: 31-channel groups stored 32 wide)", C);
    AVX_REQUIRE(ctx, ((((uintptr_t)x | (uintptr_t)wpack | (uintptr_t)out)) & 15u) == 0, "avx_mst_ln_gemm_gelu: pointers must be 16-byte aligned");
    AVX_HIP(ctx, hipSetDevice(ctx->device));
    hipStream_t s = avx_pick_stream(ctx, stream);
    if (C == 32) return launch_ffn1<32>(ctx, x, gamma, beta, eps, wpack, rows, out, s);
    if (C == 64) return launch_ffn1<64>(ctx, x, gamma, beta, eps, wpack, rows, out, s);
    return launch_ffn1<128>(ctx, x, gamma, beta, eps, wpack, rows, out, s);
}

int avx_mst_dw_gemm_add(avx_ctx* ctx, const void* hidden, const float* w_c9, const void* w2pack, const void* residual, void* out, int B, int H, int W,
                        int C, void* stream) {
    if (!ctx) return AVX_ERR_INVALID;
    AVX_REQUIRE(ctx, hidden && w_c9 && w2pack && residual && out && B > 0 && H > 0 && W > 0, "avx_mst_dw_gemm_add: NULL pointer or empty tensor");
    AVX_REQUIRE(ctx, C == 32 || C == 64, "avx_mst_dw_gemm_add: C=%d (32 or 64)", C);
    AVX_REQUIRE(ctx, ((((uintptr_t)hidden | (uintptr_t)w2pack | (uintptr_t)residual | (uintptr_t)out)) & 15u) == 0,
                "avx_mst_dw_gemm_add: pointers must be 16-byte aligned");
    AVX_REQUIRE(ctx, hidden != out, "avx_mst_dw_gemm_add: the hidden tensor cannot be the output (the residual can)");
    AVX_HIP(ctx, hipSetDevice(ctx->device));
    hipStream_t s = avx_pick_stream(ctx, stream);
    if (C == 32) return launch_ffn2<32, 2, 2, false, 3>(ctx, hidden, w_c9, w2pack, residual, out, B, H, W, s);
    return launch_ffn2<64, 2, 1, true, 2>(ctx, hidden, w_c9, w2pack, residual, out, B, H, W, s);
}

int avx_mst_rowgemm_add(avx_ctx* ctx, const void* a, const void* wpack, const void* a2, const void* wpack2, const void* add, void* out, size_t rows, int C,
                        void* stream) {
    if (!ctx) return AVX_ERR_INVALID;
    AVX_REQUIRE(ctx, a && wpack && out && rows > 0 && (!a2 == !wpack2), "avx_mst_rowgemm_add: NULL pointer or empty tensor");
    AVX_REQUIRE(ctx, C == 32 || C == 64 || C == 128, "avx_mst_rowgemm_add: C=%d (32, 64 or 128)", C);
    AVX_REQUIRE(ctx, ((((uintptr_t)a | (uintptr_t)wpack | (uintptr_t)a2 | (uintptr_t)wpack2 | (uintptr_t)add | (uintptr_t)out)) & 15u) == 0,
                "avx_mst_rowgemm_add: pointers must be 16-byte aligned");
    AVX_REQUIRE(ctx, a != out && a2 != out, "avx_mst_rowgemm_add: a GEMM operand cannot be the output (the addend can)");
    AVX_HIP(ctx, hipSetDevice(ctx->device));
    hipStream_t s = avx_pick_stream(ctx, stream);
    if (C == 32) return launch_rowgemm_add<32>(ctx, a, wpack, a2, wpack2, add, out, rows, s);
    if (C == 64) return launch_rowgemm_add<64>(ctx, a, wpack, a2, wpack2, add, out, rows, s);
    return launch_rowgemm_add<128>(ctx, a, wpack, a2, wpack2, add, out, rows, s);
}

static int attn_pack_impl(avx_ctx* ctx, const float* gram, const float* nq, const float* nk, const float* rescale, const float* wproj_t, int C, void* mpack,
                          int layout, void* stream) {
    if (!ctx) return AVX_ERR_INVALID;
    AVX_REQUIRE(ctx, gram && nq && nk && rescale && wproj_t && mpack, "avx_mst_attn_pack: NULL pointer");
    AVX_REQUIRE(ctx, C == 32 || C == 64 || C == 128, "avx_mst_attn_pack: C=%d (32, 64 or 128)", C);
    AVX_HIP(ctx, hipSetDevice(ctx->device));
    hipStream_t s = avx_pick_stream(ctx, stream);
    hipLaunchKernelGGL(k_mst_attn_pack, dim3((unsigned)((layout == 2 ? 4 : 1) * C * C / 256)), dim3(256), 0, s, gram, nq, nk, rescale, wproj_t, C, (__half*)mpack, layout);
    AVX_HIP(ctx, hipGetLastError());
    return AVX_OK;
}

int avx_mst_attn_pack(avx_ctx* ctx, const float* gram, const float* nq, const float* nk, const float* rescale, const float* wproj_t, int C, void* mpack,
                      void* stream) {
    return attn_pack_impl(ctx, gram, nq, nk, rescale, wproj_t, C, mpack, 0, stream);
}

int avx_mst_attn_pack16(avx_ctx* ctx, const float* gram, const float* nq, const float* nk, const float* rescale, const float* wproj_t, int C, void* mpack,
                        void* stream) {
    return attn_pack_impl(ctx, gram, nq, nk, rescale, wproj_t, C, mpack, 1, stream);
}

int avx_mst_attn_pack_mx(avx_ctx* ctx, const float* gram, const float* nq, const float* nk, const float* rescale, const float* wproj_t, int C, void* mpack,
                         void* stream) {
    return attn_pack_impl(ctx, gram, nq, nk, rescale, wproj_t, C, mpack, 2, stream);
}

int avx_mst_conv3x3_add(avx_ctx* ctx, const void* x, const void* wpack, const void* add, void* out, int B, int H, int W, int C, void* stream) {
    if (!ctx) return AVX_ERR_INVALID;
    AVX_REQUIRE(ctx, x && wpack && out && B > 0 && H > 0 && W > 0, "avx_mst_conv3x3_add: NULL pointer or empty tensor");
    AVX_REQUIRE(ctx, C == 32, "avx_mst_conv3x3_add: C=%d (32: the 31-channel full-resolution convs)", C);
    AVX_REQUIRE(ctx, ((((uintptr_t)x | (uintptr_t)wpack | (uintptr_t)add | (uintptr_t)out)) & 15u) == 0, "avx_mst_conv3x3_add: pointers must be 16-byte aligned");
    AVX_REQUIRE(ctx, x != out, "avx_mst_conv3x3_add: in-place convolution is not possible");
    AVX_HIP(ctx, hipSetDevice(ctx->device));
    hipStream_t s = avx_pick_stream(ctx, stream);
    constexpr int KS = 4, NT = 1;
    const size_t lds = (size_t)9 * NT * KS * 64 * sizeof(uint2);
    const long total = (long)B * H * ((W + 31) / 32);
    long blocks = (total + 3) / 4;
    const long cap = (long)ctx->num_cus * 8;
    if (blocks > cap) blocks = cap;
    auto k = k_mst_conv3x3<32>;
    AVX_HIP(ctx, hipFuncSetAttribute((const void*)k, hipFuncAttributeMaxDynamicSharedMemorySize, (int)lds));
    hipLaunchKernelGGL(k, dim3((unsigned)blocks), dim3(kT), lds, s, (const __half*)x, (const uint2*)wpack, (const __half*)add, (__half*)out, B, H, W);
    AVX_HIP(ctx, hipGetLastError());
    return AVX_OK;
}

int avx_mst_posemb(avx_ctx* ctx, const void* v, const float* w1_c9, const float* w2_c9, const void* residual, const float* bias, void* out, int B, int H, int W,
                   int C, void* stream) {
    if (!ctx) return AVX_ERR_INVALID;
    AVX_REQUIRE(ctx, v && w1_c9 && w2_c9 && out && B > 0 && H > 0 && W > 0, "avx_mst_posemb: NULL pointer or empty tensor");
    AVX_REQUIRE(ctx, C == 32 || C == 64 || C == 128, "avx_mst_posemb: C=%d (32, 64 or 128)", C);
    AVX_REQUIRE(ctx, ((((uintptr_t)v | (uintptr_t)residual | (uintptr_t)out)) & 15u) == 0, "avx_mst_posemb: pointers must be 16-byte aligned");
    AVX_REQUIRE(ctx, v != out, "avx_mst_posemb: in-place convolution is not possible");
    AVX_HIP(ctx, hipSetDevice(ctx->device));
    hipStream_t s = avx_pick_stream(ctx, stream);
    if (C == 32) return launch_posemb<32, 8, 32>(ctx, v, w1_c9, w2_c9, residual, bias, out, B, H, W, s);
    if (C == 64) return launch_posemb<64, 8, 16>(ctx, v, w1_c9, w2_c9, residual, bias, out, B, H, W, s);
    return launch_posemb<128, 4, 16>(ctx, v, w1_c9, w2_c9, residual, bias, out, B, H, W, s);
}

static int convt2x2_impl(avx_ctx* ctx, const void* x, const void* wpack, const float* bias, const void* skip, const void* wskip, void* out, int B, int H, int W,
                         int C, void* stream);
int avx_mst_convt2x2(avx_ctx* ctx, const void* x, const void* wpack, const float* bias, void* out, int B, int H, int W, int C, void* stream) {
    return convt2x2_impl(ctx, x, wpack, bias, nullptr, nullptr, out, B, H, W, C, stream);
}
int avx_mst_convt2x2_fuse(avx_ctx* ctx, const void* x, const void* wpack, const float* bias, const void* skip, const void* wskip, void* out, int B, int H,
                          int W, int C, void* stream) {
    if (ctx && !(skip && wskip)) return avx_fail(ctx, AVX_ERR_INVALID, "avx_mst_convt2x2_fuse: skip / wskip is NULL");
    if (ctx && ((((uintptr_t)skip | (uintptr_t)wskip)) & 15u)) return avx_fail(ctx, AVX_ERR_INVALID, "avx_mst_convt2x2_fuse: pointers must be 16-byte aligned");
    return convt2x2_impl(ctx, x, wpack, bias, skip, wskip, out, B, H, W, C, stream);
}
int avx_mst_convt2x2_fuse_gram(avx_ctx* ctx, const void* x, const void* wpack, const float* bias, const void* skip, const void* wskip, void* out, int H, int W, int C,
                               const void* wqk16, float* gram, float* nq, float* nk, void* stream) {
    if (!ctx) return AVX_ERR_INVALID;
    AVX_REQUIRE(ctx, x && wpack && bias && skip && wskip && out && wqk16 && gram && nq && nk && H > 0 && W > 0, "avx_mst_convt2x2_fuse_gram: NULL pointer or empty tensor");
    AVX_REQUIRE(ctx, C == 64, "avx_mst_convt2x2_fuse_gram: C=%d (64 input channels: the decoder step back to full resolution)", C);
    AVX_REQUIRE(ctx, ((((uintptr_t)x | (uintptr_t)wpack | (uintptr_t)out | (uintptr_t)skip | (uintptr_t)wskip | (uintptr_t)wqk16)) & 15u) == 0,
                "avx_mst_convt2x2_fuse_gram: pointers must be 16-byte aligned");
    AVX_HIP(ctx, hipSetDevice(ctx->device));
    hipStream_t s = avx_pick_stream(ctx, stream);
    avx_ws* ws = avx_workspace(ctx, s);
    if (!ws) return AVX_ERR_NOMEM;
    const long total = (long)H * ((W + 31) / 32);
    long blocks = (total + 3) / 4;
    const long cap = (long)ctx->num_cus * 4;
    if (blocks > cap) blocks = cap;
    int rc = avx_ensure_scratch(ctx, ws, sizeof(float) * (size_t)blocks * 34 * 32);
    if (rc) return rc;
    float* partial = (float*)ws->d_scratch;
    size_t lds = (size_t)4 * 1 * 8 * 64 * sizeof(uint2) + sizeof(float) * 32 + (size_t)1 * 4 * 64 * sizeof(uint2) + (size_t)4 * 64 * sizeof(uint4);
    if (lds < sizeof(float) * 4 * 34 * 32) lds = sizeof(float) * 4 * 34 * 32;
    auto k = k_mst_convt2x2<64, true>;
    AVX_HIP(ctx, hipFuncSetAttribute((const void*)k, hipFuncAttributeMaxDynamicSharedMemorySize, (int)lds));
    hipLaunchKernelGGL(k, dim3((unsigned)blocks), dim3(kT), lds, s, (const __half*)x, (const uint2*)wpack, bias, (const __half*)skip, (const uint2*)wskip, (__half*)out, 1, H, W,
                       (const uint4*)wqk16, partial);
    AVX_HIP(ctx, hipGetLastError());
    return avx_mst_qkv_final_launch(ctx, partial, (int)blocks, 1, gram, nq, nk, s);
}
static int convt2x2_impl(avx_ctx* ctx, const void* x, const void* wpack, const float* bias, const void* skip, const void* wskip, void* out, int B, int H, int W,
                         int C, void* stream) {
    if (!ctx) return AVX_ERR_INVALID;
    AVX_REQUIRE(ctx, x && wpack && bias && out && B > 0 && H > 0 && W > 0, "avx_mst_convt2x2: NULL pointer or empty tensor");
    AVX_REQUIRE(ctx, C == 64 || C == 128, "avx_mst_convt2x2: C=%d (64 or 128 input channels)", C);
    AVX_REQUIRE(ctx, ((((uintptr_t)x | (uintptr_t)wpack | (uintptr_t)out)) & 15u) == 0, "avx_mst_convt2x2: pointers must be 16-byte aligned");
    AVX_HIP(ctx, hipSetDevice(ctx->device));
    hipStream_t s = avx_pick_stream(ctx, stream);
    const long total = (long)B * H * ((W + 31) / 32);
    long blocks = (total + 3) / 4;
    const long cap = (long)ctx->num_cus * (C == 128 ? 2 : 8);
    if (blocks > cap) blocks = cap;
    if (C == 64) {
        const size_t lds = (size_t)4 * 1 * 8 * 64 * sizeof(uint2) + sizeof(float) * 32 + (size_t)1 * 4 * 64 * sizeof(uint2);
        AVX_HIP(ctx, hipFuncSetAttribute((const void*)k_mst_convt2x2<64, false>, hipFuncAttributeMaxDynamicSharedMemorySize, (int)lds));
        hipLaunchKernelGGL((k_mst_convt2x2<64, false>), dim3((unsigned)blocks), dim3(kT), lds, s, (const __half*)x, (const uint2*)wpack, bias, (const __half*)skip,
                           (const uint2*)wskip, (__half*)out, B, H, W);
    } else {
        const size_t lds = (size_t)4 * 2 * 16 * 64 * sizeof(uint2) + sizeof(float) * 64 + (size_t)2 * 8 * 64 * sizeof(uint2);
        AVX_HIP(ctx, hipFuncSetAttribute((const void*)k_mst_convt2x2<128, false>, hipFuncAttributeMaxDynamicSharedMemorySize, (int)lds));
        hipLaunchKernelGGL((k_mst_convt2x2<128, false>), dim3((unsigned)blocks), dim3(kT), lds, s, (const __half*)x, (const uint2*)wpack, bias, (const __half*)skip,
                           (const uint2*)wskip, (__half*)out, B, H, W);
    }
    AVX_HIP(ctx, hipGetLastError());
    return AVX_OK;
}

}
```

### animal-vision_amd/ml/mst_plus_plus.py

```python
from __future__ import annotations

from typing import Dict, List

import torch
import torch.nn.functional as F

DIM = 31
PAD = 32


def padded(n: int) -> int:
    assert n % DIM == 0
    return n // DIM * PAD


def pad_index(n: int, device=None) -> torch.Tensor:
    i = torch.arange(n, device=device)
    return (i // DIM) * PAD + i % DIM


def pad_channels(t: torch.Tensor, dims) -> torch.Tensor:
    for d in dims:
        n = t.shape[d]
        shape = list(t.shape)
        shape[d] = padded(n)
        out = torch.zeros(shape, dtype=t.dtype, device=t.device)
        out.index_copy_(d, pad_index(n, t.device), t)
        t = out
    return t


def pack_fragments(w_kn: torch.Tensor, transposed: bool) -> torch.Tensor:
    K, N = w_kn.shape
    assert K % 32 == 0 and N % 32 == 0
    dev = w_kn.device
    key = (K, N, transposed, str(dev))
    idx = _FRAG_INDEX.get(key)
    if idx is None:
        lane = torch.arange(64, device=dev)
        c, h = lane % 32, lane // 32
        if transposed:
            c = 16 * ((c % 8) // 4) + 4 * (c // 8) + c % 4
        s = torch.arange(K // 8, device=dev)
        j = torch.arange(4, device=dev)
        k = (h[None, :, None] * (K // 2) + 4 * s[:, None, None] + j[None, None, :])[None]
        col = 32 * torch.arange(N // 32, device=dev)[:, None, None, None] + c[None, None, :, None]
        idx = (k * N + col).contiguous()
        _FRAG_INDEX[key] = idx
    return torch.take(w_kn.contiguous(), idx)


_FRAG_INDEX: Dict[tuple, torch.Tensor] = {}


def pack_fragments16(w_kn: torch.Tensor, halfrow: bool = False) -> torch.Tensor:
    K, N = w_kn.shape
    assert K % 16 == 0 and N % 32 == 0
    dev = w_kn.device
    key = (K, N, "k16h" if halfrow else "k16", str(dev))
    idx = _FRAG_INDEX.get(key)
    if idx is None:
        lane = torch.arange(64, device=dev)
        m, h = lane % 32, lane // 32
        col = 16 * ((m % 8) // 4) + 4 * (m // 8) + m % 4
        s = torch.arange(K // 16, device=dev)
        j = torch.arange(8, device=dev)
        if halfrow:
            k = (8 * s[:, None, None] + (K // 2) * h[None, :, None] + j[None, None, :])[None]
        else:
            k = (16 * s[:, None, None] + 8 * h[None, :, None] + j[None, None, :])[None]
        n = 32 * torch.arange(N // 32, device=dev)[:, None, None, None] + col[None, None, :, None]
        idx = (k * N + n).contiguous()
        _FRAG_INDEX[key] = idx
    return torch.take(w_kn.contiguous(), idx)


def pack_qkv16(wqkv: torch.Tensor) -> torch.Tensor:
    K, N = wqkv.shape
    assert N == 3 * K and K % 32 == 0
    dev = wqkv.device
    key = (K, N, "qkv16", str(dev))
    idx = _FRAG_INDEX.get(key)
    if idx is None:
        lane = torch.arange(64, device=dev)
        m, h = lane % 32, lane // 32
        perm = 16 * ((m % 8) // 4) + 4 * (m // 8) + m % 4
        t = torch.arange(N // 32, device=dev)
        col = 32 * t[:, None] + torch.where(t[:, None] >= 2 * (K // 32), perm[None, :], m[None, :])
        q = torch.arange(K // 16, device=dev)
        j = torch.arange(8, device=dev)
        k = h[None, :, None] * (K // 2) + 8 * q[:, None, None] + j[None, None, :]
        idx = (k[None] * N + col[:, None, :, None]).contiguous()
        _FRAG_INDEX[key] = idx
    return torch.take(wqkv.contiguous(), idx)


def pack_dw_mfma(w: torch.Tensor) -> torch.Tensor:
    ch = w.shape[0]
    assert ch % 8 == 0 and tuple(w.shape[1:]) == (1, 3, 3)
    dev = w.device
    lane = torch.arange(64, device=dev)
    m, q = lane % 16, lane // 16
    s_, c = m // 8, m % 8
    dy = q - s_
    ok = (dy >= 0) & (dy <= 2)
    w8 = w.reshape(ch // 8, 8, 3, 3)
    vals = w8[:, c, dy.clamp(0, 2), :]
    vals = torch.where(ok[None, :, None], vals, torch.zeros_like(vals))
    out = torch.zeros((ch // 8, 3, 64, 8), dtype=w.dtype, device=dev)
    out[:, :, lane, c] = vals.permute(0, 2, 1)
    return out.contiguous()


def pack_dw_smfmac(w: torch.Tensor) -> torch.Tensor:
    ch = w.shape[0]
    assert ch % 8 == 0 and tuple(w.shape[1:]) == (1, 3, 3)
    dev = w.device
    lane = torch.arange(64, device=dev)
    m, qa = lane % 16, lane // 16
    s_, c = m // 8, m % 8
    w8 = w.reshape(ch // 8, 8, 3, 3)
    out = torch.zeros((ch // 8, 3, 64, 8), dtype=w.dtype, device=dev)
    out[:, 1] = pack_dw_mfma(w)[:, 2]
    t = c % 4
    idx = torch.full((64,), 0x4444, dtype=torch.int64, device=dev)
    for hh in range(2):
        r = 2 * (qa % 2) + hh
        dy = r - s_
        ok = (dy >= 0) & (dy <= 2)
        vals = w8[:, c, dy.clamp(0, 2), qa // 2]
        vals = torch.where(ok[None, :], vals, torch.zeros_like(vals))
        e = 4 * hh + 2 * (c // 4) + (t == 3).long()
        out[:, 0, lane, e] = vals
        pair = torch.where(t == 3, 2 | (3 << 2), t | (3 << 2))
        sh = 4 * (2 * hh + c // 4)
        idx = (idx & ~(0xF << sh)) | (pair << sh)
    lo = (((idx & 0xFFFF) ^ 0x8000) - 0x8000).to(torch.int16)
    out.view(torch.int16)[:, 2, :, 0] = lo[None]
    return out.contiguous()


def fold_layernorm(w1_kn: torch.Tensor, gamma: torch.Tensor, beta: torch.Tensor, scale: float) -> torch.Tensor:
    w = w1_kn.float()
    out = w * gamma.float()[:, None]
    out[31, :] = beta.float() @ w
    return (out / scale).contiguous()


def pack_down4x4(w: torch.Tensor) -> torch.Tensor:
    return torch.stack([pack_fragments16(w[:, :, t // 4, t % 4].t().contiguous()) for t in range(16)]).contiguous()


class _AvxOps:

    def __init__(self):
        import os

        self.enabled = os.environ.get("AVX_MST_TORCH_ONLY", "") == ""
        self._mfma = os.environ.get("AVX_MST_NO_MFMA", "") == ""
        self._ffn2 = os.environ.get("AVX_MST_NO_FFN2", "") == ""
        self._posemb = os.environ.get("AVX_MST_NO_POSEMB", "") == ""
        self._conv_lds = os.environ.get("AVX_MST_NO_CONV_LDS", "") == ""
        self._conv_in = os.environ.get("AVX_MST_NO_CONV_IN", "") == ""
        self._upfuse = os.environ.get("AVX_MST_NO_UPFUSE", "") == ""
        self._tail = os.environ.get("AVX_MST_NO_TAIL", "") == ""
        self._tailx = os.environ.get("AVX_MST_NO_TAILX", "") == ""
        self._down = os.environ.get("AVX_MST_NO_DOWN4X4", "") == ""
        self._qkv16 = os.environ.get("AVX_MST_NO_QKV16", "") == ""
        self._convgram = os.environ.get("AVX_MST_NO_CONVGRAM", "") == ""
        self._ffn = os.environ.get("AVX_MST_NO_FFN_FUSED", "") == ""
        self._gelu_pre = None
        self._dwmx = os.environ.get("AVX_MST_NO_DW_MFMA", "") == ""
        self._dwsp = os.environ.get("AVX_MST_NO_DW_SPARSE", "") == ""
        self.DW_SPARSE_FFN_C = (32, 64, 128)
        self.DW_SPARSE_TAIL_C = (32, 64)
        self._specfuse = os.environ.get("AVX_MST_NO_SPEC_FUSE", "") == ""
        self._cinfuse = os.environ.get("AVX_MST_NO_CONV_IN_FUSE", "") == ""
        self.FFN_FUSED_C = tuple(int(v) for v in os.environ.get("AVX_MST_FFN_FUSED_C", "32,64,128").split(",") if v)
        self._ffn_march = os.environ.get("AVX_MST_NO_FFN_MARCH", "") == ""
        self.FFN_MARCH_C = (32, 64)
        self._ctx = {}

    def ctx(self, device: torch.device):
        from ..runtime import get_context

        idx = device.index if device.index is not None else torch.cuda.current_device()
        c = get_context(idx)
        if c.device != idx:
            raise RuntimeError(f"libavx context is on device {c.device}, tensor on cuda:{idx} (one process per GPU)")
        return c

    @staticmethod
    def _dt(t: torch.Tensor) -> int:
        if t.dtype == torch.float32:
            return 0
        if t.dtype == torch.float16:
            return 1
        raise TypeError(f"csrc/mst.hip kernels take float32/float16, got {t.dtype}")

    def gram(self, qkv: torch.Tensor, heads: int):
        from .._lib import lib

        b, n, c3 = qkv.shape
        c = c3 // 3
        d = c // heads
        ctx = self.ctx(qkv.device)
        g = torch.empty((b, heads, 32, 32), dtype=torch.float32, device=qkv.device)
        nq = torch.empty((b, c), dtype=torch.float32, device=qkv.device)
        nk = torch.empty((b, c), dtype=torch.float32, device=qkv.device)
        st = torch.cuda.current_stream(qkv.device).cuda_stream
        for i in range(b):
            ctx._check(lib.avx_mst_gram(ctx._h, qkv[i].data_ptr(), self._dt(qkv), n, c, heads, g[i].data_ptr(), nq[i].data_ptr(), nk[i].data_ptr(), st))
        return g[:, :, :d, :d], nq, nk

    def gelu_prescale(self) -> float:
        if self._gelu_pre is None:
            from .. import _lib
            self._gelu_pre = float(_lib.lib.avx_mst_gelu_prescale())
        return self._gelu_pre

    def fused_ok(self, x: torch.Tensor) -> bool:
        return self.enabled and x.is_cuda and x.dtype == torch.float16 and x.shape[-1] in (32, 64, 128) and self._mfma

    def qkv_gram(self, x2: torch.Tensor, wpack: torch.Tensor, heads: int, want_v: bool = True, k16: bool = False):
        from .._lib import lib

        b, n, c = x2.shape
        x2 = x2.contiguous()
        ctx = self.ctx(x2.device)
        v = torch.empty_like(x2) if want_v else None
        g = torch.empty((b, heads, 32, 32), dtype=torch.float32, device=x2.device)
        nq = torch.empty((b, c), dtype=torch.float32, device=x2.device)
        nk = torch.empty((b, c), dtype=torch.float32, device=x2.device)
        st = torch.cuda.current_stream(x2.device).cuda_stream
        fn = lib.avx_mst_qkv_gram16 if k16 else lib.avx_mst_qkv_gram
        for i in range(b):
            ctx._check(fn(ctx._h, x2[i].data_ptr(), wpack.data_ptr(), n, c, v[i].data_ptr() if want_v else None, g[i].data_ptr(), nq[i].data_ptr(), nk[i].data_ptr(), st))
        return v, g, nq, nk

    def ln_gemm_gelu(self, x2: torch.Tensor, gamma: torch.Tensor, beta: torch.Tensor, wpack: torch.Tensor, eps: float = 1e-5) -> torch.Tensor:
        from .._lib import lib

        rows, c = x2.shape
        x2 = x2.contiguous()
        ctx = self.ctx(x2.device)
        out = torch.empty((rows, 4 * c), dtype=torch.float16, device=x2.device)
        ctx._check(lib.avx_mst_ln_gemm_gelu(ctx._h, x2.data_ptr(), gamma.data_ptr(), beta.data_ptr(), eps, wpack.data_ptr(), rows, c, out.data_ptr(),
                                            torch.cuda.current_stream(x2.device).cuda_stream))
        return out

    def convt2x2(self, x: torch.Tensor, wpack: torch.Tensor, bias: torch.Tensor, skip: torch.Tensor = None, wskip: torch.Tensor = None) -> torch.Tensor:
        from .._lib import lib

        b, h, w, c = x.shape
        x = x.contiguous()
        out = torch.empty((b, 2 * h, 2 * w, c // 2), dtype=torch.float16, device=x.device)
        ctx = self.ctx(x.device)
        st = torch.cuda.current_stream(x.device).cuda_stream
        if skip is None:
            ctx._check(lib.avx_mst_convt2x2(ctx._h, x.data_ptr(), wpack.data_ptr(), bias.data_ptr(), out.data_ptr(), b, h, w, c, st))
        else:
            assert skip.is_contiguous() and skip.shape == out.shape
            ctx._check(lib.avx_mst_convt2x2_fuse(ctx._h, x.data_ptr(), wpack.data_ptr(), bias.data_ptr(), skip.data_ptr(), wskip.data_ptr(), out.data_ptr(), b, h, w, c, st))
        return out

    def convt2x2_gram(self, x: torch.Tensor, wpack: torch.Tensor, bias: torch.Tensor, skip: torch.Tensor, wskip: torch.Tensor, wqk16: torch.Tensor):
        from .._lib import lib

        b, h, w, c = x.shape
        assert c == 64 and skip.is_contiguous() and skip.shape == (b, 2 * h, 2 * w, 32)
        x = x.contiguous()
        out = torch.empty((b, 2 * h, 2 * w, 32), dtype=torch.float16, device=x.device)
        g = torch.empty((b, 1, 32, 32), dtype=torch.float32, device=x.device)
        nq = torch.empty((b, 32), dtype=torch.float32, device=x.device)
        nk = torch.empty((b, 32), dtype=torch.float32, device=x.device)
        ctx = self.ctx(x.device)
        st = torch.cuda.current_stream(x.device).cuda_stream
        for i in range(b):
            ctx._check(lib.avx_mst_convt2x2_fuse_gram(ctx._h, x[i].data_ptr(), wpack.data_ptr(), bias.data_ptr(), skip[i].data_ptr(), wskip.data_ptr(), out[i].data_ptr(), h, w, c,
                                                      wqk16.data_ptr(), g[i].data_ptr(), nq[i].data_ptr(), nk[i].data_ptr(), st))
        return out, g, nq, nk

    def posemb(self, v: torch.Tensor, w1_c9: torch.Tensor, w2_c9: torch.Tensor, residual: torch.Tensor = None, bias: torch.Tensor = None) -> torch.Tensor:
        from .._lib import lib

        b, h, w, c = v.shape
        v = v.contiguous()
        residual = residual.contiguous() if residual is not None else None
        out = torch.empty_like(v)
        ctx = self.ctx(v.device)
        ctx._check(lib.avx_mst_posemb(ctx._h, v.data_ptr(), w1_c9.data_ptr(), w2_c9.data_ptr(), residual.data_ptr() if residual is not None else None,
                                      bias.data_ptr() if bias is not None else None, out.data_ptr(), b, h, w, c, torch.cuda.current_stream(v.device).cuda_stream))
        return out

    def conv3x3(self, x: torch.Tensor, wpack: torch.Tensor, add: torch.Tensor = None) -> torch.Tensor:
        from .._lib import lib

        b, h, w, c = x.shape
        x = x.contiguous()
        add = add.contiguous() if add is not None else None
        out = torch.empty_like(x)
        ctx = self.ctx(x.device)
        ctx._check(lib.avx_mst_conv3x3_add(ctx._h, x.data_ptr(), wpack.data_ptr(), add.data_ptr() if add is not None else None, out.data_ptr(), b, h, w, c,
                                           torch.cuda.current_stream(x.device).cuda_stream))
        return out

    def conv_in_u8(self, frame: torch.Tensor, pads, w_27x32: torch.Tensor) -> torch.Tensor:
        from .._lib import lib

        H, W, _ = frame.shape
        t, b, l, r = pads
        frame = frame.contiguous()
        out = torch.empty((1, H + t + b, W + l + r, 32), dtype=torch.float16, device=frame.device)
        ctx = self.ctx(frame.device)
        ctx._check(lib.avx_mst_conv_in_u8(ctx._h, frame.data_ptr(), H, W, t, b, l, r, w_27x32.data_ptr(), out.data_ptr(),
                                          torch.cuda.current_stream(frame.device).cuda_stream))
        return out

    def down4x4(self, x: torch.Tensor, wpack16: torch.Tensor) -> torch.Tensor:
        from .._lib import lib

        b, h, w, c = x.shape
        assert x.is_contiguous() and c in (32, 64) and h % 2 == 0 and w % 2 == 0
        out = torch.empty((b, h // 2, w // 2, 2 * c), dtype=torch.float16, device=x.device)
        ctx = self.ctx(x.device)
        st = torch.cuda.current_stream(x.device).cuda_stream
        per = max(1, (2**31 - 1) // (h * w * c * 2))
        for i in range(0, b, per):
            ctx._check(lib.avx_mst_down4x4(ctx._h, x[i : i + per].data_ptr(), wpack16.data_ptr(), out[i : i + per].data_ptr(), min(per, b - i), h, w, c, st))
        return out

    def conv3x3_lds_gram(self, x: torch.Tensor, wpack16: torch.Tensor, add: torch.Tensor, wqk16: torch.Tensor):
        from .._lib import lib

        b, h, w, c = x.shape
        x = x.contiguous()
        add = add.contiguous() if add is not None else None
        out = torch.empty_like(x)
        g = torch.empty((b, 1, 32, 32), dtype=torch.float32, device=x.device)
        nq = torch.empty((b, c), dtype=torch.float32, device=x.device)
        nk = torch.empty((b, c), dtype=torch.float32, device=x.device)
        ctx = self.ctx(x.device)
        st = torch.cuda.current_stream(x.device).cuda_stream
        for i in range(b):
            ctx._check(lib.avx_mst_conv3x3_lds_gram(ctx._h, x[i].data_ptr(), wpack16.data_ptr(), add[i].data_ptr() if add is not None else None, out[i].data_ptr(), h, w, c,
                                                    wqk16.data_ptr(), g[i].data_ptr(), nq[i].data_ptr(), nk[i].data_ptr(), st))
        return out, g, nq, nk

    def conv3x3_lds_spectral(self, x: torch.Tensor, wpack16: torch.Tensor, add: torch.Tensor, weights, crop):
        import ctypes

        import numpy as np

        from .._lib import lib

        if isinstance(add, tuple):
            return self.conv3x3_lds_spectral_cin(x, wpack16, add, weights, crop)
        b, h, w, c = x.shape
        assert b == 1 and c == 32 and x.is_contiguous() and (add is None or add.is_contiguous())
        t, l, H, W = crop
        ctx = self.ctx(x.device)
        planes = torch.empty((3, H, W), dtype=torch.float32, device=x.device)
        ncu = torch.cuda.get_device_properties(x.device).multi_processor_count
        partials = torch.empty((ncu * 3, 3, 2), dtype=torch.float64, device=x.device)
        wh = np.ascontiguousarray(weights, dtype=np.float32)
        assert wh.shape == (3, 32)
        n = ctypes.c_int(0)
        ctx._check(lib.avx_mst_conv3x3_lds_spectral(ctx._h, x.data_ptr(), wpack16.data_ptr(), add.data_ptr() if add is not None else None, h, w, c,
                                                    wh.ctypes.data_as(ctypes.POINTER(ctypes.c_float)), t, l, H, W, planes.data_ptr(), partials.data_ptr(), ctypes.byref(n),
                                                    torch.cuda.current_stream(x.device).cuda_stream))
        return planes, partials, int(n.value)

    def conv3x3_lds_gram_cin(self, src, wpack16: torch.Tensor, wqk16: torch.Tensor):
        from .._lib import lib

        frame, (t, b, l, r), w27 = src
        H, W, _ = frame.shape
        frame = frame.contiguous()
        out = torch.empty((1, H + t + b, W + l + r, 32), dtype=torch.float16, device=frame.device)
        g = torch.empty((1, 1, 32, 32), dtype=torch.float32, device=frame.device)
        nq = torch.empty((1, 32), dtype=torch.float32, device=frame.device)
        nk = torch.empty((1, 32), dtype=torch.float32, device=frame.device)
        ctx = self.ctx(frame.device)
        ctx._check(lib.avx_mst_conv3x3_lds_gram_cin(ctx._h, frame.data_ptr(), H, W, t, b, l, r, w27.data_ptr(), wpack16.data_ptr(), out.data_ptr(), wqk16.data_ptr(),
                                                    g.data_ptr(), nq.data_ptr(), nk.data_ptr(), torch.cuda.current_stream(frame.device).cuda_stream))
        return out, g, nq, nk

    def conv3x3_lds_cin(self, x: torch.Tensor, wpack16: torch.Tensor, src) -> torch.Tensor:
        from .._lib import lib

        frame, (t, b, l, r), w27 = src
        H, W, _ = frame.shape
        assert x.shape == (1, H + t + b, W + l + r, 32)
        x, frame = x.contiguous(), frame.contiguous()
        out = torch.empty_like(x)
        ctx = self.ctx(x.device)
        ctx._check(lib.avx_mst_conv3x3_lds_cin(ctx._h, x.data_ptr(), wpack16.data_ptr(), frame.data_ptr(), H, W, t, b, l, r, w27.data_ptr(), out.data_ptr(),
                                               torch.cuda.current_stream(x.device).cuda_stream))
        return out

    def conv3x3_lds_spectral_cin(self, x: torch.Tensor, wpack16: torch.Tensor, src, weights, crop):
        import ctypes

        import numpy as np

        from .._lib import lib

        frame, (t, b, l, r), w27 = src
        H, W, _ = frame.shape
        assert x.shape == (1, H + t + b, W + l + r, 32) and x.is_contiguous()
        frame = frame.contiguous()
        ct, cl, Hc, Wc = crop
        ctx = self.ctx(x.device)
        planes = torch.empty((3, Hc, Wc), dtype=torch.float32, device=x.device)
        ncu = torch.cuda.get_device_properties(x.device).multi_processor_count
        partials = torch.empty((ncu * 3, 3, 2), dtype=torch.float64, device=x.device)
        wh = np.ascontiguousarray(weights, dtype=np.float32)
        assert wh.shape == (3, 32)
        n = ctypes.c_int(0)
        ctx._check(lib.avx_mst_conv3x3_lds_spectral_cin(ctx._h, x.data_ptr(), wpack16.data_ptr(), frame.data_ptr(), H, W, t, b, l, r, w27.data_ptr(),
                                                        wh.ctypes.data_as(ctypes.POINTER(ctypes.c_float)), ct, cl, Hc, Wc, planes.data_ptr(), partials.data_ptr(), ctypes.byref(n),
                                                        torch.cuda.current_stream(x.device).cuda_stream))
        return planes, partials, int(n.value)

    def conv3x3_lds(self, x: torch.Tensor, wpack16: torch.Tensor, add: torch.Tensor = None) -> torch.Tensor:
        from .._lib import lib

        b, h, w, c = x.shape
        x = x.contiguous()
        add = add.contiguous() if add is not None else None
        out = torch.empty_like(x)
        ctx = self.ctx(x.device)
        ctx._check(lib.avx_mst_conv3x3_lds(ctx._h, x.data_ptr(), wpack16.data_ptr(), add.data_ptr() if add is not None else None, out.data_ptr(), b, h, w, c,
                                           torch.cuda.current_stream(x.device).cuda_stream))
        return out

    def attn_pack(self, gram: torch.Tensor, nq: torch.Tensor, nk: torch.Tensor, rescale: torch.Tensor, wproj_t: torch.Tensor) -> torch.Tensor:
        from .._lib import lib

        c = nq.numel()
        ctx = self.ctx(gram.device)
        out = torch.empty((c // 32, c // 8, 64, 4), dtype=torch.float16, device=gram.device)
        ctx._check(lib.avx_mst_attn_pack(ctx._h, gram.data_ptr(), nq.data_ptr(), nk.data_ptr(), rescale.data_ptr(), wproj_t.data_ptr(), c, out.data_ptr(),
                                         torch.cuda.current_stream(gram.device).cuda_stream))
        return out

    def attn_pack16(self, gram: torch.Tensor, nq: torch.Tensor, nk: torch.Tensor, rescale: torch.Tensor, wproj_t: torch.Tensor) -> torch.Tensor:
        from .._lib import lib

        c = nq.numel()
        ctx = self.ctx(gram.device)
        out = torch.empty((c // 32, c // 16, 64, 8), dtype=torch.float16, device=gram.device)
        ctx._check(lib.avx_mst_attn_pack16(ctx._h, gram.data_ptr(), nq.data_ptr(), nk.data_ptr(), rescale.data_ptr(), wproj_t.data_ptr(), c, out.data_ptr(),
                                           torch.cuda.current_stream(gram.device).cuda_stream))
        return out

    def attn_pack_mx(self, gram: torch.Tensor, nq: torch.Tensor, nk: torch.Tensor, rescale: torch.Tensor, wproj_t: torch.Tensor) -> torch.Tensor:
        from .._lib import lib

        c = nq.numel()
        ctx = self.ctx(gram.device)
        out = torch.empty((c // 8, c // 16, 64, 8), dtype=torch.float16, device=gram.device)
        ctx._check(lib.avx_mst_attn_pack_mx(ctx._h, gram.data_ptr(), nq.data_ptr(), nk.data_ptr(), rescale.data_ptr(), wproj_t.data_ptr(), c, out.data_ptr(),
                                            torch.cuda.current_stream(gram.device).cuda_stream))
        return out

    def attn_tail_mx(self, x: torch.Tensor, wvpack16: torch.Tensor, mpack_mx: torch.Tensor, dw1: torch.Tensor, dw2: torch.Tensor, bias: torch.Tensor,
                     out: torch.Tensor = None, sparse: bool = False) -> torch.Tensor:
        from .._lib import lib

        h, w, c = x.shape
        assert x.is_contiguous()
        out = torch.empty_like(x) if out is None else out
        ctx = self.ctx(x.device)
        fn = lib.avx_mst_attn_tail_sp if sparse else lib.avx_mst_attn_tail_mx
        ctx._check(fn(ctx._h, x.data_ptr(), wvpack16.data_ptr(), mpack_mx.data_ptr(), dw1.data_ptr(), dw2.data_ptr(), bias.data_ptr(),
                      out.data_ptr(), 1, h, w, c, torch.cuda.current_stream(x.device).cuda_stream))
        return out

    def attn_tail(self, v: torch.Tensor, x: torch.Tensor, mpack16: torch.Tensor, taps1: torch.Tensor, taps2: torch.Tensor, bias: torch.Tensor,
                  out: torch.Tensor = None) -> torch.Tensor:
        from .._lib import lib

# ... 215 lines not shown
    def _ms_msa(self, x: torch.Tensor, p: str, heads: int, pre=None) -> torch.Tensor:
        b, h, w, c = x.shape
        n = h * w
        x2 = x.reshape(b, n, c)
        wqkv = self._prep(p + ".qkv", lambda: torch.cat([self._w(p + ".to_q.weight", (0, 1)), self._w(p + ".to_k.weight", (0, 1)),
                                                         self._w(p + ".to_v.weight", (0, 1))], 0).t().contiguous())
        d = c // heads
        if _AVX.fused_ok(x):
            tailx = _AVX._tail and _AVX._tailx and (c in (32, 64) or (c == 128 and _AVX._dwmx))
            if _AVX._qkv16:
                wpk = self._prep(p + ".qkv.frag16", lambda: pack_qkv16(wqkv))
            else:
                wpk = self._prep(p + ".qkv.frag", lambda: torch.cat([pack_fragments(wqkv[:, : 2 * c], False), pack_fragments(wqkv[:, 2 * c :], True)], 0).contiguous())
            if pre is not None and tailx:
                v, (gram, nq, nk) = None, pre
            else:
                v, gram, nq, nk = _AVX.qkv_gram(x2, wpk, heads, want_v=not tailx, k16=_AVX._qkv16)
            if self.capture_attn is not None:
                self._capture(gram, nq, nk, p, heads)
            resc = self._prep(p + ".rescale32", lambda: self._p(p + ".rescale").float().reshape(heads).contiguous())
            wpt = self._prep(p + ".proj.t32", lambda: self._w(p + ".proj.weight", (0, 1)).t().float().contiguous())
            bias32 = self._prep(p + ".proj.bias32", lambda: self._w(p + ".proj.bias", (0,)).float().contiguous())
            vi = v.reshape(b, h, w, c) if v is not None else None
            if _AVX._tail and (c in (32, 64) or tailx):
                k1, k2 = p + ".pos_emb.0.weight", p + ".pos_emb.2.weight"
                t1 = self._prep(k1 + ".t9h", lambda: self._w(k1, (0,)).reshape(c, 9).t().contiguous())
                t2 = self._prep(k2 + ".t9h", lambda: self._w(k2, (0,)).reshape(c, 9).t().contiguous())
                xc = x.contiguous()
                out = torch.empty_like(xc)
                if tailx and _AVX._dwmx:
                    wv16 = self._prep(p + ".wv.frag16h", lambda: pack_fragments16(wqkv[:, 2 * c :].contiguous(), halfrow=True))
                    gs = _AVX.gelu_prescale()
                    sp = _AVX._dwsp and c in _AVX.DW_SPARSE_TAIL_C
                    pk, tag = (pack_dw_smfmac, ".dwsp") if sp else (pack_dw_mfma, ".dwmx")
                    d1 = self._prep(k1 + f"{tag}/{gs}", lambda: pk((self._w(k1, (0,)).float() / gs).to(x.dtype)))
                    d2 = self._prep(k2 + f"{tag}*{gs}", lambda: pk((self._w(k2, (0,)).float() * gs).to(x.dtype)))
                    for i in range(b):
                        _AVX.attn_tail_mx(xc[i], wv16, _AVX.attn_pack_mx(gram[i], nq[i], nk[i], resc, wpt), d1, d2, bias32, out[i], sparse=sp)
                    return out
                if tailx:
                    wv16 = self._prep(p + ".wv.frag16", lambda: pack_fragments16(wqkv[:, 2 * c :].contiguous()))
                    for i in range(b):
                        _AVX.attn_tail_x(xc[i], wv16, _AVX.attn_pack16(gram[i], nq[i], nk[i], resc, wpt), t1, t2, bias32, out[i])
                    return out
                for i in range(b):
                    _AVX.attn_tail(vi[i], xc[i], _AVX.attn_pack16(gram[i], nq[i], nk[i], resc, wpt), t1, t2, bias32, out[i])
                return out
            if _AVX._posemb:
                k1, k2 = p + ".pos_emb.0.weight", p + ".pos_emb.2.weight"
                w91 = self._prep(k1 + ".c9f32", lambda: self._w(k1, (0,)).reshape(c, 9).float().contiguous())
                w92 = self._prep(k2 + ".c9f32", lambda: self._w(k2, (0,)).reshape(c, 9).float().contiguous())
                pe = _AVX.posemb(vi, w91, w92, x, bias32)
            else:
                pe = self._dw(self._dw(vi, p + ".pos_emb.0.weight", gelu=True), p + ".pos_emb.2.weight", gelu=False, residual=x, bias=bias32)
            for i in range(b):
                _AVX.rowgemm_add(v[i], _AVX.attn_pack(gram[i], nq[i], nk[i], resc, wpt), pe[i].reshape(n, c))
            return pe
        qkv = x2 @ wqkv
        q, k, v = qkv[..., :c], qkv[..., c : 2 * c], qkv[..., 2 * c :]
        if x.is_cuda and _AVX.enabled:
            gram, nq, nk = _AVX.gram(qkv, heads)
            nq = nq.reshape(b, heads, 1, d).clamp_min(1e-12)
            nk = nk.reshape(b, heads, d, 1).clamp_min(1e-12)
        else:
            qh = q.reshape(b, n, heads, d).permute(0, 2, 1, 3)
            kh = k.reshape(b, n, heads, d).permute(0, 2, 1, 3)
            gram = torch.matmul(kh.transpose(-2, -1), qh).float()
            nq = torch.linalg.vector_norm(q.float(), dim=1).reshape(b, heads, 1, d).clamp_min(1e-12)
            nk = torch.linalg.vector_norm(k.float(), dim=1).reshape(b, heads, d, 1).clamp_min(1e-12)
        attn = gram / (nk * nq)
        attn = attn * self._p(p + ".rescale").float().reshape(1, heads, 1, 1)
        attn[..., DIM:] = float("-inf")
        attn = attn.softmax(dim=-1)
        if self.capture_attn is not None:
            self.capture_attn.append(attn[:, :, :DIM, :DIM].float().cpu())
        wp = self._w(p + ".proj.weight", (0, 1))
        wp_h = wp.t().reshape(heads, d, c).float()
        M = torch.matmul(attn.transpose(-2, -1), wp_h.unsqueeze(0)).reshape(b, c, c).to(x.dtype)
        vi = v.reshape(b, h, w, c)
        out_c = torch.baddbmm(self._w(p + ".proj.bias", (0,)).to(x.dtype).reshape(1, 1, c), v, M).reshape(b, h, w, c)
        pe = self._dw(self._dw(vi, p + ".pos_emb.0.weight", gelu=True), p + ".pos_emb.2.weight", gelu=False)
        return out_c + pe + x

    def _dw(self, x: torch.Tensor, key: str, gelu: bool, residual: torch.Tensor = None, bias: torch.Tensor = None) -> torch.Tensor:
        c = x.shape[-1]
        if x.is_cuda and _AVX.enabled:
            w9 = self._prep(key + ".c9f32", lambda: self._w(key, (0,)).reshape(c, 9).float().contiguous())
            return _AVX.dwconv(x, w9, gelu, residual, bias)
        y = self._conv_nhwc(x, self._w(key, (0,)), padding=1, groups=c)
        y = F.gelu(y) if gelu else y
        if residual is not None:
            y = y + residual
        return y + bias.to(y.dtype) if bias is not None else y

    def _ffn(self, x: torch.Tensor, p: str) -> torch.Tensor:
        b, h, w, c = x.shape
        g32 = self._prep(p + ".g32", lambda: self._w(p + ".norm.weight", (0,)).float().contiguous())
        b32 = self._prep(p + ".b32", lambda: self._w(p + ".norm.bias", (0,)).float().contiguous())
        w2 = self._prep(p + ".w2", lambda: self._w(p + ".fn.net.4.weight", (0, 1)).reshape(c, 4 * c).t().contiguous())
        if _AVX.fused_ok(x) and _AVX._ffn and c in _AVX.FFN_FUSED_C:
            key = p + ".fn.net.2.weight"
            if _AVX._dwmx:
                gs = _AVX.gelu_prescale()
                w1s = self._prep(p + f".w1.frag16.ln/{gs}", lambda: pack_fragments16(fold_layernorm(self._w(p + ".fn.net.0.weight", (0, 1)).reshape(4 * c, c).t(), g32, b32, gs).to(x.dtype)))
                w2s = self._prep(p + f".w2.frag16*{gs}", lambda: pack_fragments16((w2.float() * gs).to(x.dtype).contiguous()))
                march = _AVX._ffn_march and c in _AVX.FFN_MARCH_C
                if _AVX._dwsp and c in _AVX.DW_SPARSE_FFN_C:
                    return _AVX.ffn_fused(x, g32, b32, w1s, None, w2s, dwpack=self._prep(key + ".dwsp", lambda: pack_dw_smfmac(self._w(key, (0,)))), sparse=True, march=march)
                return _AVX.ffn_fused(x, g32, b32, w1s, None, w2s, dwpack=self._prep(key + ".dwmx", lambda: pack_dw_mfma(self._w(key, (0,)))), march=march)
            w1q = self._prep(p + ".w1.frag16", lambda: pack_fragments16(self._w(p + ".fn.net.0.weight", (0, 1)).reshape(4 * c, c).t().contiguous()))
            w2q = self._prep(p + ".w2.frag16", lambda: pack_fragments16(w2))
            t9 = self._prep(key + ".t9h", lambda: self._w(key, (0,)).reshape(4 * c, 9).t().contiguous())
            return _AVX.ffn_fused(x, g32, b32, w1q, t9, w2q)
        if _AVX.fused_ok(x):
            w1p = self._prep(p + ".w1.frag", lambda: pack_fragments(self._w(p + ".fn.net.0.weight", (0, 1)).reshape(4 * c, c).t().contiguous(), True))
            y = _AVX.ln_gemm_gelu(x.reshape(b * h * w, c), g32, b32, w1p).reshape(b, h, w, 4 * c)
            if c in (32, 64) and x.is_contiguous() and _AVX._ffn2:
                key = p + ".fn.net.2.weight"
                w9 = self._prep(key + ".c9f32", lambda: self._w(key, (0,)).reshape(4 * c, 9).float().contiguous())
                w2p = self._prep(p + ".w2.frag", lambda: pack_fragments(w2, True))
                return _AVX.dw_gemm_add(y, w9, w2p, x)
            y = self._dw(y, p + ".fn.net.2.weight", gelu=True)
            return x.reshape(b * h * w, c).addmm_(y.reshape(b * h * w, 4 * c), w2).reshape(b, h, w, c)
        if x.is_cuda and _AVX.enabled:
            y = _AVX.layernorm(x, g32, b32, group=PAD, real=DIM)
        else:
            real = self._prep(p + ".real", lambda: pad_index(c // PAD * DIM, x.device))
            yr = F.layer_norm(x.float().index_select(-1, real), (real.numel(),), g32.index_select(0, real), b32.index_select(0, real))
            y = torch.zeros_like(x, dtype=torch.float32).index_copy_(-1, real, yr).to(x.dtype)
        w1 = self._prep(p + ".w1", lambda: self._w(p + ".fn.net.0.weight", (0, 1)).reshape(4 * c, c).t().contiguous())
        y = F.gelu(y.reshape(b, h * w, c) @ w1).reshape(b, h, w, 4 * c)
        y = self._dw(y, p + ".fn.net.2.weight", gelu=True)
        return (y.reshape(b, h * w, 4 * c) @ w2).reshape(b, h, w, c) + x

    def _msab(self, x: torch.Tensor, p: str, heads: int, pre=None) -> torch.Tensor:
        x = self._ms_msa(x, p + ".blocks.0.0", heads, pre)
        return self._ffn(x, p + ".blocks.0.1")

    def _mst(self, x: torch.Tensor, p: str, src=None) -> torch.Tensor:
        pre = None
        ekey, a0 = p + ".embedding.weight", f"{p}.encoder_layers.0.0.blocks.0.0"
        if src is not None or (_AVX.fused_ok(x) and x.shape[-1] == 32 and _AVX._conv_lds and _AVX._convgram and _AVX._qkv16 and _AVX._tail and _AVX._tailx):
            wq = self._prep(ekey + ".frag9k16", lambda: torch.stack([pack_fragments16(self._w(ekey, (0, 1))[:, :, t // 3, t % 3].t().contiguous()) for t in range(9)]).contiguous())
            wqkv = self._prep(a0 + ".qkv", lambda: torch.cat([self._w(a0 + ".to_q.weight", (0, 1)), self._w(a0 + ".to_k.weight", (0, 1)),
                                                              self._w(a0 + ".to_v.weight", (0, 1))], 0).t().contiguous())
            wqk = self._prep(a0 + ".qkv.frag16", lambda: pack_qkv16(wqkv))
            fea, g, nq, nk = _AVX.conv3x3_lds_gram(x, wq, None, wqk) if src is None else _AVX.conv3x3_lds_gram_cin(src, wq, wqk)
            pre = (g, nq, nk)
        else:
            fea = self._conv3(x, ekey)
        skips: List[torch.Tensor] = []
        heads = 1
        for i in range(2):
            fea = self._msab(fea, f"{p}.encoder_layers.{i}.0", heads, pre if i == 0 else None)
            skips.append(fea)
            dkey = f"{p}.encoder_layers.{i}.1.weight"
            if _AVX.fused_ok(fea) and _AVX._down and fea.shape[-1] in (32, 64) and fea.is_contiguous():
                fea = _AVX.down4x4(fea, self._prep(dkey + ".frag16", lambda: pack_down4x4(self._w(dkey, (0, 1)))))
            else:
                fea = self._conv_nhwc(fea, self._w(dkey, (0, 1)), stride=2, padding=1)
            heads *= 2
        fea = self._msab(fea, p + ".bottleneck", heads)
        for i in range(2):
            kw = f"{p}.decoder_layers.{i}.0.weight"
            if _AVX.fused_ok(fea) and fea.shape[-1] in (64, 128) and _AVX._upfuse:
                ch = fea.shape[-1] // 2
                wfk = f"{p}.fuse{i}"
                wf_ = self._prep(wfk, lambda: self._w(f"{p}.decoder_layers.{i}.1.weight", (0, 1)).reshape(ch, 2 * ch).t().contiguous())
                gt = self._prep(kw + ".upfuse4", lambda: torch.stack([pack_fragments((self._w(kw, (0, 1))[:, :, t // 2, t % 2].float() @ wf_[:ch].float()).half().contiguous(), True)
                                                                     for t in range(4)]).contiguous())
                gb = self._prep(kw + ".upfuse.bias", lambda: (self._w(f"{p}.decoder_layers.{i}.0.bias", (0,)).float() @ wf_[:ch].float()).contiguous())
                wbot_ = self._prep(f"{p}.fuse{i}.bot", lambda: pack_fragments(wf_[ch:].contiguous(), True))
                heads //= 2
                a2 = f"{p}.decoder_layers.{i}.2.blocks.0.0"
                if ch == 32 and _AVX._convgram and _AVX._qkv16 and _AVX._tail and _AVX._tailx:
                    wqkv2 = self._prep(a2 + ".qkv", lambda: torch.cat([self._w(a2 + ".to_q.weight", (0, 1)), self._w(a2 + ".to_k.weight", (0, 1)),
                                                                       self._w(a2 + ".to_v.weight", (0, 1))], 0).t().contiguous())
                    wqk2 = self._prep(a2 + ".qkv.frag16", lambda: pack_qkv16(wqkv2))
                    fea, g2, nq2, nk2 = _AVX.convt2x2_gram(fea, gt, gb, skips[1 - i].contiguous(), wbot_, wqk2)
                    fea = self._msab(fea, f"{p}.decoder_layers.{i}.2", heads, (g2, nq2, nk2))
                    continue
                fea = _AVX.convt2x2(fea, gt, gb, skips[1 - i].contiguous(), wbot_)
                fea = self._msab(fea, f"{p}.decoder_layers.{i}.2", heads)
                continue
            if _AVX.fused_ok(fea) and fea.shape[-1] in (64, 128):
                wt = self._prep(kw + ".frag4", lambda: torch.stack([pack_fragments(self._w(kw, (0, 1))[:, :, t // 2, t % 2].contiguous(), True) for t in range(4)]).contiguous())
                bt = self._prep(kw + ".bias32", lambda: self._w(f"{p}.decoder_layers.{i}.0.bias", (0,)).float().contiguous())
                up = _AVX.convt2x2(fea, wt, bt)
            else:
                up = F.conv_transpose2d(fea.permute(0, 3, 1, 2), self._w(kw, (0, 1)), self._w(f"{p}.decoder_layers.{i}.0.bias", (0,)), stride=2).permute(0, 2, 3, 1)
            heads //= 2
            skip = skips[1 - i]
            b, h, w, ch = up.shape
            c2 = 2 * ch
            wf = self._prep(f"{p}.fuse{i}", lambda: self._w(f"{p}.decoder_layers.{i}.1.weight", (0, 1)).reshape(c2 // 2, c2).t().contiguous())
            if _AVX.fused_ok(skip):
                up, skip = up.contiguous(), skip.contiguous()
                wtop = self._prep(f"{p}.fuse{i}.top", lambda: pack_fragments(wf[:ch].contiguous(), True))
                wbot = self._prep(f"{p}.fuse{i}.bot", lambda: pack_fragments(wf[ch:].contiguous(), True))
                fea = _AVX.rowgemm_add(up.reshape(b * h * w, ch), wtop, None, skip.reshape(b * h * w, ch), wbot).reshape(b, h, w, ch)
            else:
                cat = torch.cat([up, skip], dim=-1)
                fea = (cat.reshape(b, h * w, c2) @ wf).reshape(b, h, w, c2 // 2)
            fea = self._msab(fea, f"{p}.decoder_layers.{i}.2", heads)
        if src is not None:
            return _AVX.conv3x3_lds_cin(fea, self._frag9k16(p + ".mapping.weight"), src)
        return self._conv3(fea, p + ".mapping.weight", add=x)

    @torch.no_grad()
    def forward_from_u8(self, frame: torch.Tensor, pads, spectral=None):
        w27 = self._prep("conv_in.w27x32", lambda: self._w("conv_in.weight", (0,)).permute(2, 3, 1, 0).reshape(27, PAD).float().contiguous())
        H, W, _ = frame.shape
        assert (H + pads[0] + pads[1]) % 8 == 0 and (W + pads[2] + pads[3]) % 8 == 0, "pad the frame to a multiple of 8 (predict_torch.py pads to 16)"
        spec = None if spectral is None else (spectral, (pads[0], pads[2], H, W))
        if self.can_fuse_conv_in_consumers():
            return self._body(None, spectral=spec, src=(frame, tuple(pads), w27))
        return self._body(_AVX.conv_in_u8(frame, pads, w27), spectral=spec)

    def can_fuse_conv_in_consumers(self) -> bool:
        return (self.can_fuse_conv_in() and self.stage >= 1 and _AVX._cinfuse and _AVX._conv_lds and _AVX._convgram and _AVX._qkv16 and _AVX._tail and _AVX._tailx)

    def can_fuse_spectral(self) -> bool:
        return self.can_fuse_conv_in() and _AVX._conv_lds and _AVX._specfuse

    def _frag9k16(self, key: str) -> torch.Tensor:
        return self._prep(key + ".frag9k16", lambda: torch.stack([pack_fragments16(self._w(key, (0, 1))[:, :, t // 3, t % 3].t().contiguous()) for t in range(9)]).contiguous())

    def _body(self, x: torch.Tensor, spectral=None, src=None):
        hfe = x
        for s in range(self.stage):
            hfe = self._mst(hfe, f"body.{s}", src if s == 0 else None)
        key = "conv_out.weight"
        if spectral is not None:
            return _AVX.conv3x3_lds_spectral(hfe.contiguous(), self._frag9k16(key), src if src is not None else x.contiguous(), spectral[0], spectral[1])
        if src is not None:
            return _AVX.conv3x3_lds_cin(hfe, self._frag9k16(key), src)
        return self._conv3(hfe, key, add=x)

    def can_fuse_conv_in(self) -> bool:
        ref = self._p("conv_in.weight")
        return _AVX.enabled and _AVX._mfma and _AVX._conv_in and ref.is_cuda and ref.dtype == torch.float16

    @torch.no_grad()
    def forward_nhwc(self, x: torch.Tensor) -> torch.Tensor:
        b, c, h_inp, w_inp = x.shape
        pad_h, pad_w = (8 - h_inp % 8) % 8, (8 - w_inp % 8) % 8
        if pad_h or pad_w:
            x = F.pad(x, [0, pad_w, 0, pad_h], mode="reflect")
        x = x.to(self._p("conv_in.weight").dtype).contiguous(memory_format=torch.channels_last).permute(0, 2, 3, 1)
        x = self._conv_nhwc(x, self._w("conv_in.weight", (0,)), padding=1)
        return self._body(x)[:, :h_inp, :w_inp, :]

    @torch.no_grad()
    def forward(self, x: torch.Tensor) -> torch.Tensor:
        return self.forward_nhwc(x)[..., :DIM].permute(0, 3, 1, 2)


def hbm_bytes_per_px(stage: int = 3) -> float:

    def msab(c: int) -> float:
        t = 2.0 * c
        if _AVX._tail and _AVX._tailx and (c in (32, 64) or (c == 128 and _AVX._dwmx)):
            b = t
            b += 2 * t
            return b + ((2 * t) if (_AVX._ffn and c in _AVX.FFN_FUSED_C) else (t + 4 * t + ((4 * t + 2 * t) if _AVX._ffn2 else (4 * t + 4 * t + 4 * t + 2 * t))))
        b = 2 * t
        if _AVX._tail and c in (32, 64):
            b += 3 * t
        else:
            b += (3 * t if _AVX._posemb else 5 * t)
            b += 3 * t
        if _AVX._ffn and c in _AVX.FFN_FUSED_C:
            b += 2 * t
        else:
            b += t + 4 * t
            b += (4 * t + 2 * t) if (c in (32, 64) and _AVX._ffn2) else (4 * t + 4 * t + 4 * t + 2 * t)
        return b

    per_stage = 2 * msab(32) + 2 * msab(64) / 4 + msab(128) / 16
    if _AVX._convgram and _AVX._qkv16 and _AVX._tail and _AVX._tailx and _AVX._conv_lds and _AVX._upfuse:
        per_stage -= 2 * 64.0
    t32, t64, t128 = 64.0, 128.0 / 4, 256.0 / 16
    convs = (2 * t32) + (3 * t32)
    convs += (t32 + t64) + (t64 + t128)
    if _AVX._upfuse:
        convs += (t128 + t64 + t64) + (t64 + t32 + t32)
    else:
        convs += (t128 + t64) + (2 * t64 + t64)
        convs += (t64 + t32) + (2 * t32 + t32)
    head = ((3 + t32) if _AVX._conv_in else (3 + 12) + (12 + t32)) + ((2 * t32 + 12) if (_AVX._specfuse and _AVX._conv_lds and _AVX._conv_in) else 3 * t32)
    if stage >= 1 and _AVX._cinfuse and _AVX._conv_in and _AVX._conv_lds and _AVX._convgram and _AVX._qkv16 and _AVX._tail and _AVX._tailx:
        head += 3 * 3 - (4 * t32 + 3)
    return stage * (per_stage + convs) + head
```

### include/avx.h

```cpp
#ifndef AVX_H
#define AVX_H

#include <stddef.h>
#include <stdint.h>

#ifdef __cplusplus
extern "C" {
#endif

#define AVX_ABI_VERSION 1

typedef struct avx_ctx avx_ctx;

typedef enum avx_status {
    AVX_OK = 0,
    AVX_ERR_INVALID = -1,
    AVX_ERR_NO_DEVICE = -2,
    AVX_ERR_HIP = -3,
    AVX_ERR_UNSUPPORTED = -4,
    AVX_ERR_NOMEM = -5
} avx_status;

int avx_abi_version(void);
int avx_device_count(void);
// ... 199 lines not shown
} avx_ms_ssim_rec;

int avx_frame_metrics_ms_u8(avx_ctx* ctx, const uint8_t* a_hwc, const uint8_t* b_hwc, int n_frames, int H, int W,
                            avx_frame_metrics* out_dev, avx_ms_ssim_rec* ms_out_dev, void* stream);

enum avx_diff_mode { AVX_DIFF_ABS = 0, AVX_DIFF_HEAT = 1, AVX_DIFF_SSIM = 2 };
enum avx_diff_layout { AVX_DIFF_MAP = 0, AVX_DIFF_SIDE = 1 };
typedef struct { uint32_t max_d, max_x, max_y, beyond; } avx_diff_rec;

int avx_diff_map_u8(avx_ctx* ctx, const uint8_t* a_hwc, const uint8_t* b_hwc, int n_frames, int H, int W, int mode, float gain, int threshold,
                    int layout, uint8_t* out_hwc, avx_diff_rec* rec_dev, float* ssim_map_dev, void* stream);

enum avx_delta_e_mode { AVX_DELTA_E_HEAT = 0, AVX_DELTA_E_PLAIN = 1 };
enum avx_delta_e_layout { AVX_DELTA_E_MAP = 0, AVX_DELTA_E_SIDE = 1 };
typedef struct avx_delta_e_rec {
    uint32_t hist[256];
    double sum;
    float max_de;
    uint32_t max_x, max_y;
    uint32_t beyond;
} avx_delta_e_rec;

int avx_delta_e_u8(avx_ctx* ctx, const uint8_t* a_hwc, const uint8_t* b_hwc, int n_frames, int H, int W, int mode, float gain, float threshold,
                   int layout, uint8_t* map_out, avx_delta_e_rec* rec_dev, float* de_out, void* stream);

int avx_scielab_u8(avx_ctx* ctx, const uint8_t* a_hwc, const uint8_t* b_hwc, int n_frames, int H, int W, double ppd, int mode, float gain,
                   float threshold, int layout, uint8_t* map_out, avx_delta_e_rec* rec_dev, float* de_out, void* stream);

int avx_remap_linear_planes(avx_ctx* ctx, const float* src_planes, int K, int H, int W, const float* mapx_dev,
                            const float* mapy_dev, float* dst_planes, float border_value, void* stream);

int avx_sobel3_plane(avx_ctx* ctx, const float* plane, int H, int W, float* gx, float* gy, void* stream);

typedef struct avx_mantis_desc {
    uint32_t struct_size;
    int32_t n_bands;
    const float* band_matrix_host;
    const float* band_lut_host;
    int32_t n_wavelengths;
    const float* lobe_gains_host;
    float lobe_denom;
    const float* band_weights_host;
    int32_t pano_new_w;
    int32_t hsi_small_h, hsi_small_w;
    float red_keep;
    float haze, haze_keep, haze_tint[3];
    int32_t pre_soft_ksize; const double* pre_soft_taps_host;
    float cos2_global, sin2_global;
    float orientation_mix, pol_linear_strength, pol_linear_gamma, pol_circular_strength;
    int32_t unsharp_ksize; const double* unsharp_taps_host; float unsharp_amount;
    float barcode_saturation, barcode_opacity, winner_take_most;
    const float* rows_host;
    float scan_row_gain; int32_t scan_ksize; const double* scan_taps_host;
    int32_t periph_ksize; const double* periph_taps_host;
    const float* xx_host; const float* yy_host;
    float periph_radius, periph_softness;
    const float* lin_hwc_in;
    int32_t out_float;
} avx_mantis_desc;

int avx_mantis_u8(avx_ctx* ctx, const uint8_t* in_hwc, uint8_t* out_baseline_hwc, uint8_t* out_hwc, int H, int W,
                  const avx_mantis_desc* desc, void* stream);
int avx_mantis_u8_batch(avx_ctx* ctx, const uint8_t* in_hwc, uint8_t* out_baseline_hwc, uint8_t* out_hwc, int n_frames, int H, int W,
                        const avx_mantis_desc* desc, void* stream);

int avx_uv_front_u8(avx_ctx* ctx, const uint8_t* in_hwc, int H, int W, int pano_new_w, float* lin_hwc_out,
                    uint8_t* baseline_hwc_out, void* stream);
int avx_panorama_warp_f32(avx_ctx* ctx, const float* src_hwc, int H, int W, int new_w, float* dst_hwc, void* stream);
typedef struct avx_band_stack_desc {
    uint32_t struct_size;
    int32_t n_bands;
    const float* band_matrix_host;
    int32_t n_wavelengths;
    const float* lobe_gains_host;
    float lobe_denom;
    const float* band_weights_host;
    int32_t small_h, small_w;
} avx_band_stack_desc;
int avx_band_stack(avx_ctx* ctx, const float* lin_hwc, int H, int W, const avx_band_stack_desc* desc,
                   float* stack_hwk_out, void* stream);
int avx_uv_front_u8_batch(avx_ctx* ctx, const uint8_t* in_hwc, int n_frames, size_t in_frame_stride, int H, int W, int pano_new_w,
                          float* lin_hwc_out, size_t lin_frame_stride, uint8_t* baseline_hwc_out, size_t baseline_frame_stride,
                          void* stream);
int avx_band_stack_batch(avx_ctx* ctx, const float* lin_hwc, int n_frames, size_t lin_frame_stride, int H, int W,
                         const avx_band_stack_desc* desc, float* stack_hwk_out, size_t stack_frame_stride, void* stream);
int avx_percentile_dev(avx_ctx* ctx, const float* data_dev, size_t n, double q, double* out_dev, void* stream);
int avx_percentiles_dev(avx_ctx* ctx, int count, const float* const* data_dev, const size_t* n, const double* q,
                        double* const* out_dev, void* stream);

enum { AVX_EW_MAX_INSN = 384, AVX_EW_MAX_PLANES = 24, AVX_EW_MAX_REGS = 32, AVX_EW_MAX_ACC = 16 };
enum {
    AVX_EW_CONST = 1, AVX_EW_SCALAR, AVX_EW_LOAD, AVX_EW_STORE,
    AVX_EW_ADD, AVX_EW_SUB, AVX_EW_MUL, AVX_EW_DIV, AVX_EW_MIN, AVX_EW_MAX, AVX_EW_POW, AVX_EW_ATAN2,
    AVX_EW_NEG, AVX_EW_ABS, AVX_EW_SQRT, AVX_EW_EXP, AVX_EW_LOG, AVX_EW_SIN, AVX_EW_COS, AVX_EW_FLOOR, AVX_EW_CEIL,
    AVX_EW_CLIP01, AVX_EW_TANH,
    AVX_EW_LT, AVX_EW_LE, AVX_EW_GT, AVX_EW_GE, AVX_EW_EQ, AVX_EW_AND, AVX_EW_OR, AVX_EW_NOT,
    AVX_EW_SELECT,
    AVX_EW_ACCMIN, AVX_EW_ACCMAX, AVX_EW_ACCSUM
};
enum { AVX_EW_OPCODE_MASK = 0x3f, AVX_EW_IMM_A = 0x40, AVX_EW_IMM_B = 0x80 };
enum {
    AVX_EW_PLANE_F32 = 0,
    AVX_EW_PLANE_U8,
    AVX_EW_PLANE_U8_LUT,
    AVX_EW_PLANE_COL,
    AVX_EW_PLANE_ROW,
    AVX_EW_PLANE_U8_ENC
};
enum { AVX_EW_ACC_MIN = 0, AVX_EW_ACC_MAX, AVX_EW_ACC_SUM, AVX_EW_ACC_MEAN };
typedef struct avx_ew_insn { uint8_t op, dst, a, b; uint32_t imm; } avx_ew_insn;
typedef struct avx_ew_plane { void* ptr; int32_t stride; int32_t kind; } avx_ew_plane;
typedef struct avx_ew_program {
    uint32_t struct_size;
    int32_t H, W;
    int32_t n_insn; const avx_ew_insn* insn_host;
    int32_t n_planes; const avx_ew_plane* planes_host;
    int32_t n_acc; const int32_t* acc_host;
    double* scalars_dev; int32_t n_scalars;
} avx_ew_program;
int avx_ew_run(avx_ctx* ctx, const avx_ew_program* program, void* stream);
enum { AVX_EW_MAX_FRAMES = 16 };
int avx_ew_run_batch(avx_ctx* ctx, const avx_ew_program* program, int n_frames, const size_t* plane_frame_stride_bytes_host,
                     size_t scalars_frame_stride, void* stream);
int avx_ew_spec_stats(unsigned long long* hits, unsigned long long* misses);


int avx_mst_gram(avx_ctx* ctx, const void* qkv, int dtype, size_t n_pix, int C, int heads, float* gram, float* nq, float* nk, void* stream);

int avx_mst_qkv_gram(avx_ctx* ctx, const void* x, const void* wpack, size_t n_pix, int C, void* v_out, float* gram, float* nq, float* nk,
                     void* stream);
int avx_mst_qkv_gram16(avx_ctx* ctx, const void* x, const void* wpack16, size_t n_pix, int C, void* v_out, float* gram, float* nq, float* nk,
                       void* stream);
int avx_mst_ln_gemm_gelu(avx_ctx* ctx, const void* x, const float* gamma, const float* beta, float eps, const void* wpack, size_t rows, int C,
                         void* out, void* stream);

int avx_mst_dw_gemm_add(avx_ctx* ctx, const void* hidden, const float* w_c9, const void* w2pack, const void* residual, void* out, int B, int H,
                        int W, int C, void* stream);

int avx_mst_conv_in_u8(avx_ctx* ctx, const uint8_t* frame_hwc, int H, int W, int pad_top, int pad_bottom, int pad_left, int pad_right,
                       const float* w_27x32_dev, void* out, void* stream);

int avx_mst_conv3x3_lds(avx_ctx* ctx, const void* x, const void* wpack16, const void* add, void* out, int B, int H, int W, int C, void* stream);
int avx_mst_conv3x3_lds_gram(avx_ctx* ctx, const void* x, const void* wpack16, const void* add, void* out, int H, int W, int C, const void* wqk16, float* gram,
                             float* nq, float* nk, void* stream);
int avx_mst_conv3x3_lds_cin(avx_ctx* ctx, const void* x, const void* wpack16, const uint8_t* frame_hwc, int H, int W, int pad_top, int pad_bottom, int pad_left, int pad_right,
                            const float* w_27x32_dev, void* out, void* stream);
int avx_mst_conv3x3_lds_spectral_cin(avx_ctx* ctx, const void* x, const void* wpack16, const uint8_t* frame_hwc, int H, int W, int pad_top, int pad_bottom, int pad_left,
                                     int pad_right, const float* w_27x32_dev, const float* weights_host, int crop_t, int crop_l, int Hc, int Wc, float* planes_out,
                                     void* partials_out, int* n_partials, void* stream);
int avx_mst_conv3x3_lds_gram_cin(avx_ctx* ctx, const uint8_t* frame_hwc, int H, int W, int pad_top, int pad_bottom, int pad_left, int pad_right, const float* w_27x32_dev,
                                 const void* wpack16, void* out, const void* wqk16, float* gram, float* nq, float* nk, void* stream);
int avx_mst_convt2x2_fuse_gram(avx_ctx* ctx, const void* x, const void* wpack, const float* bias, const void* skip, const void* wskip, void* out, int H, int W, int C,
                               const void* wqk16, float* gram, float* nq, float* nk, void* stream);
int avx_mst_down4x4(avx_ctx* ctx, const void* x, const void* wpack16, void* out, int B, int H, int W, int C, void* stream);

int avx_mst_attn_pack16(avx_ctx* ctx, const float* gram, const float* nq, const float* nk, const float* rescale, const float* wproj_t, int C, void* mpack,
                        void* stream);
int avx_mst_attn_tail(avx_ctx* ctx, const void* v, const void* x, const void* mpack16, const void* taps1_9xc, const void* taps2_9xc, const float* bias,
                      void* out, int B, int H, int W, int C, void* stream);
int avx_mst_attn_tail_x(avx_ctx* ctx, const void* x, const void* wvpack16, const void* mpack16, const void* taps1_9xc, const void* taps2_9xc,
                        const float* bias, void* out, int B, int H, int W, int C, void* stream);
int avx_mst_attn_tail_mx(avx_ctx* ctx, const void* x, const void* wvpack16, const void* mpack_mx, const void* dw1pack, const void* dw2pack,
                         const float* bias, void* out, int B, int H, int W, int C, void* stream);
int avx_mst_attn_tail_sp(avx_ctx* ctx, const void* x, const void* wvpack16, const void* mpack_mx, const void* dw1pack, const void* dw2pack,
                         const float* bias, void* out, int B, int H, int W, int C, void* stream);
int avx_mst_attn_pack_mx(avx_ctx* ctx, const float* gram, const float* nq, const float* nk, const float* rescale, const float* wproj_t, int C, void* mpack,
                         void* stream);


int avx_mst_conv3x3_lds_spectral(avx_ctx* ctx, const void* x, const void* wpack16, const void* add, int H, int W, int C, const float* weights_host, int crop_t,
                                 int crop_l, int Hc, int Wc, float* planes_out, void* partials_out, int* n_partials, void* stream);

int avx_mst_ffn_fused(avx_ctx* ctx, const void* x, const float* gamma, const float* beta, float eps, const void* w1pack, const void* taps_9xhid,
                      const void* w2pack, void* out, int B, int H, int W, int C, void* stream);
int avx_mst_ffn_fused_mx(avx_ctx* ctx, const void* x, const float* gamma, const float* beta, float eps, const void* w1pack, const void* dwpack,
                         const void* w2pack, void* out, int B, int H, int W, int C, void* stream);
int avx_mst_ffn_fused_sp(avx_ctx* ctx, const void* x, const float* gamma, const float* beta, float eps, const void* w1pack, const void* dwpack,
                         const void* w2pack, void* out, int B, int H, int W, int C, void* stream);
float avx_mst_gelu_prescale(void);

int avx_mst_tile_order(int frames, int ty, int tx, int nwg, int raster, long long* visit, int steps_cap, int* steps_out);

int avx_mst_ffn_fused_mx_col(avx_ctx* ctx, const void* x, const float* gamma, const float* beta, float eps, const void* w1pack, const void* dwpack,
                             const void* w2pack, void* out, int B, int H, int W, int C, int max_workgroups, void* stream);
int avx_mst_ffn_fused_sp_col(avx_ctx* ctx, const void* x, const float* gamma, const float* beta, float eps, const void* w1pack, const void* dwpack,
                             const void* w2pack, void* out, int B, int H, int W, int C, int max_workgroups, void* stream);
int avx_mst_tile_order_col(int frames, int ty, int tx, int nwg, long long* visit, unsigned char* seg, int steps_cap, int* steps_out);

int avx_mst_rowgemm_add(avx_ctx* ctx, const void* a, const void* wpack, const void* a2, const void* wpack2, const void* add, void* out, size_t rows,
                        int C, void* stream);

int avx_mst_attn_pack(avx_ctx* ctx, const float* gram, const float* nq, const float* nk, const float* rescale, const float* wproj_t, int C,
                      void* mpack, void* stream);

int avx_mst_conv3x3_add(avx_ctx* ctx, const void* x, const void* wpack, const void* add, void* out, int B, int H, int W, int C, void* stream);

int avx_mst_posemb(avx_ctx* ctx, const void* v, const float* w1_c9, const float* w2_c9, const void* residual, const float* bias, void* out, int B,
                   int H, int W, int C, void* stream);

int avx_mst_convt2x2(avx_ctx* ctx, const void* x, const void* wpack, const float* bias, void* out, int B, int H, int W, int C, void* stream);
int avx_mst_convt2x2_fuse(avx_ctx* ctx, const void* x, const void* wpack, const float* bias, const void* skip, const void* wskip, void* out, int B, int H,
                          int W, int C, void* stream);

int avx_dwconv3x3_nhwc(avx_ctx* ctx, const void* x, const float* w_c9, void* y, int dtype, int B, int H, int W, int C, int gelu_out, void* stream);
int avx_dwconv3x3_nhwc_add(avx_ctx* ctx, const void* x, const float* w_c9, void* y, int B, int H, int W, int C, int gelu_out,
                           const void* residual, const float* bias, void* stream);

int avx_layernorm_rows(avx_ctx* ctx, const void* x, const float* gamma, const float* beta, void* y, int dtype, size_t rows, int C, float eps, void* stream);
int avx_layernorm_rows_grouped(avx_ctx* ctx, const void* x, const float* gamma, const float* beta, void* y, int dtype, size_t rows, int C, float eps,
                               int group, int real, void* stream);

int avx_get_table(int which, void* dst_host, size_t capacity);

#ifdef __cplusplus
}
#endif
#endif
```

Before: 460.3.

## Fuse Q/K Gram epilogue into down4x4 and 128-channel transposed-conv resampling kernels

Adds a Gram-matrix epilogue to the 32->64 down4x4 DMA kernel: each tile's output is staged in LDS and projected to Q/K with MFMA, and per-frame Gram and norm partials are flushed to scratch for a final reduction. It also generalises the convt2x2 Gram epilogue to multiple heads so the 128->64 upsampling step can produce Gram statistics too. The aim is to avoid re-reading the 64-channel activations in a separate Q/K Gram pass at the next attention block. The cost is extra LDS use (possibly lower occupancy), a __syncthreads per tile, and scratch partial writes.

New measurement: 466.4 (median of 6 runs). About the same (+1.3%).

```diff
diff --git a/animal-vision_amd/_lib.py b/animal-vision_amd/_lib.py
--- a/animal-vision_amd/_lib.py
+++ b/animal-vision_amd/_lib.py
@@ -358,11 +358,13 @@
     "avx_mst_conv_in_u8": (_i, [_vp, _vp, _i, _i, _i, _i, _i, _i, _vp, _vp, _vp]),
     "avx_mst_conv3x3_lds": (_i, [_vp, _vp, _vp, _vp, _vp, _i, _i, _i, _i, _vp]),
     "avx_mst_down4x4": (_i, [_vp, _vp, _vp, _vp, _i, _i, _i, _i, _vp]),
+    "avx_mst_down4x4_gram": (_i, [_vp, _vp, _vp, _vp, _i, _i, _i, _vp, _vp, _vp, _vp, _i, _vp]),
     "avx_mst_conv3x3_lds_gram": (_i, [_vp, _vp, _vp, _vp, _vp, _i, _i, _i, _vp, _vp, _vp, _vp, _vp]),
     "avx_mst_conv3x3_lds_cin": (_i, [_vp, _vp, _vp, _vp, _i, _i, _i, _i, _i, _i, _vp, _vp, _vp]),
     "avx_mst_conv3x3_lds_spectral_cin": (_i, [_vp, _vp, _vp, _vp, _i, _i, _i, _i, _i, _i, _vp, _fp, _i, _i, _i, _i, _vp, _vp, ctypes.POINTER(ctypes.c_int), _vp]),
     "avx_mst_conv3x3_lds_gram_cin": (_i, [_vp, _vp, _i, _i, _i, _i, _i, _i, _vp, _vp, _vp, _vp, _vp, _vp, _vp, _vp]),
     "avx_mst_convt2x2_fuse_gram": (_i, [_vp, _vp, _vp, _vp, _vp, _vp, _vp, _i, _i, _i, _vp, _vp, _vp, _vp, _vp]),
+    "avx_mst_convt2x2_fuse_gram128": (_i, [_vp, _vp, _vp, _vp, _vp, _vp, _vp, _i, _i, _vp, _vp, _vp, _vp, _vp]),
     "avx_mst_attn_pack16": (_i, [_vp, _vp, _vp, _vp, _vp, _vp, _i, _vp, _vp]),
     "avx_mst_attn_pack_mx": (_i, [_vp, _vp, _vp, _vp, _vp, _vp, _i, _vp, _vp]),
     "avx_mst_attn_tail_mx": (_i, [_vp, _vp, _vp, _vp, _vp, _vp, _vp, _vp, _i, _i, _i, _i, _vp]),
diff --git a/animal-vision_amd/csrc/mst_fused.hip b/animal-vision_amd/csrc/mst_fused.hip
--- a/animal-vision_amd/csrc/mst_fused.hip
+++ b/animal-vision_amd/csrc/mst_fused.hip
@@ -1377,12 +1377,16 @@
     asm volatile("s_mov_b32 m0, %0\n\ts_nop 0\n\tglobal_load_lds_dwordx4 %1, %2" ::"s"(__builtin_amdgcn_readfirstlane(lds_base)), "v"(ofs), "s"(base) : "memory", "m0");
 }
 #pragma clang diagnostic pop
-template <int C>
+template <int C, bool GRAM = false>
 __global__ __launch_bounds__(kFT, 2) void k_mst_down4x4_dma(const __half* __restrict__ x , const uint4* __restrict__ wpack ,
-                                                            __half* __restrict__ out , const void* __restrict__ zero, int B, int H, int W, int order ) {
+                                                            __half* __restrict__ out , const void* __restrict__ zero, int B, int H, int W, int order ,
+                                                            const uint4* __restrict__ wqk = nullptr ,
+                                                            float* __restrict__ partial = nullptr ) {
     using G = DownGeo<C>;
+    static_assert(!GRAM || C == 32, "the Gram epilogue is for the 32 -> 64 channel step");
     constexpr int CO = 2 * C, NT = CO / 32, KS = C / 16;
-    __shared__ __align__(1024) unsigned char lds[G::NBUF * G::BUF + G::PART];
+    constexpr int SPITCH = 144, STASH = GRAM ? 128 * SPITCH : 0, WQK = GRAM ? 4 * 4 * 64 * 16 : 0;
+    __shared__ __align__(1024) unsigned char lds[G::NBUF * G::BUF + G::PART + STASH + WQK];
     const int tid = threadIdx.x, lane = tid & 63, wave = __builtin_amdgcn_readfirstlane(tid >> 6) , p = lane & 31, h = lane >> 5;
     const int g0 = C == 32 ? wave & 3 : 0, nt = C == 32 ? wave >> 2 : wave & 3, kh = C == 32 ? 0 : wave >> 2;
     half8_t wf[32];
@@ -1422,8 +1426,59 @@
             }
         }
     };
+    float16_t Gm;
+    float nq = 0.f, nk = 0.f;
+    int gb = -1;
+    if constexpr (GRAM) {
+        uint4* wql = reinterpret_cast<uint4*>(lds + G::NBUF * G::BUF + G::PART + STASH);
+        for (int i = tid; i < 4 * 4 * 64; i += kFT) wql[i] = wqk[i];
+#pragma unroll
+        for (int v = 0; v < 16; ++v) Gm[v] = 0.f;
+    }
+    auto flush = [&](int frame) {
+        float* mine = partial + ((((size_t)frame * gridDim.x + blockIdx.x) * 4 + g0) * 2 + nt) * (34 * 32);
+#pragma unroll
+        for (int v = 0; v < 16; ++v) mine[(8 * (v / 4) + 4 * h + (v % 4)) * 32 + p] = Gm[v];
+        const float sq = nq + __shfl_xor(nq, 32), sk = nk + __shfl_xor(nk, 32);
+        if (h == 0) { mine[32 * 32 + p] = sq; mine[33 * 32 + p] = sk; }
+#pragma unroll
+        for (int v = 0; v < 16; ++v) Gm[v] = 0.f;
+        nq = 0.f; nk = 0.f;
+    };
+    auto consume = [&]() {
+        const unsigned char* row = lds + G::NBUF * G::BUF + G::PART + (g0 * 32 + p) * SPITCH + h * 64;
+        const uint4* wql = reinterpret_cast<const uint4*>(lds + G::NBUF * G::BUF + G::PART + STASH);
+        float16_t dq, dk;
+#pragma unroll
+        for (int v = 0; v < 16; ++v) { dq[v] = 0.f; dk[v] = 0.f; }
+        half8_t a[4];
+#pragma unroll
+        for (int q = 0; q < 4; ++q) a[q] = __builtin_bit_cast(half8_t, *reinterpret_cast<const uint4*>(row + 16 * q));
+#pragma unroll
+        for (int q = 0; q < 4; ++q) dq = mfma16(a[q], __builtin_bit_cast(half8_t, wql[(nt * 4 + q) * 64 + lane]), dq);
+#pragma unroll
+        for (int q = 0; q < 4; ++q) dk = mfma16(a[q], __builtin_bit_cast(half8_t, wql[((2 + nt) * 4 + q) * 64 + lane]), dk);
+        unsigned aq[8], ak[8];
+#pragma unroll
+        for (int j = 0; j < 8; ++j) {
+            aq[j] = pack_f16(dq[2 * j], dq[2 * j + 1]);
+            ak[j] = pack_f16(dk[2 * j], dk[2 * j + 1]);
+            fma_mix_lo(nq, aq[j], aq[j]); fma_mix_hi(nq, aq[j], aq[j]);
+            fma_mix_lo(nk, ak[j], ak[j]); fma_mix_hi(nk, ak[j], ak[j]);
+        }
+#pragma unroll
+        for (int b2 = 0; b2 < 2; ++b2)
+            Gm = mfma16(__builtin_bit_cast(half8_t, uint4{ak[4 * b2], ak[4 * b2 + 1], ak[4 * b2 + 2], ak[4 * b2 + 3]}),
+                        __builtin_bit_cast(half8_t, uint4{aq[4 * b2], aq[4 * b2 + 1], aq[4 * b2 + 2], aq[4 * b2 + 3]}), Gm);
+    };
     TileWalk walk, look;
     walk.init(blockIdx.x, gridDim.x, B, ty, tx, order);
+    if constexpr (GRAM) {
+        if (!walk.live) {
+            for (int f = 0; f < B; ++f) flush(f);
+            return;
+        }
+    }
     if (!walk.live) return;
     look = walk;
 #pragma unroll
@@ -1446,6 +1501,14 @@
         const T2 t = tile_at(walk);
         const bool whole = t.oy0 + G::OH <= Ho && t.ox0 + G::OW <= Wo;
         const unsigned char* bt = lds + slot * G::BUF;
+        bool flushed = false;
+        if constexpr (GRAM) {
+            if (t.b != gb) {
+                for (int f = gb < 0 ? 0 : gb; f < t.b; ++f) flush(f);
+                flushed = gb >= 0 || t.b > 0;
+                gb = t.b;
+            }
+        }
 #pragma unroll 1
         for (int g = g0; g < (C == 32 ? g0 + 1 : G::GROUPS); ++g) {
             const int r = 2 * g + (p >> 4);
@@ -1493,6 +1556,12 @@
             half8_t o0, o1;
 #pragma unroll
             for (int v = 0; v < 8; ++v) { o0[v] = (_Float16)d[v]; o1[v] = (_Float16)d[8 + v]; }
+            if constexpr (GRAM) {
+                const bool in = whole || (yo < Ho && xo < Wo);
+                uint4* sd = reinterpret_cast<uint4*>(lds + G::NBUF * G::BUF + G::PART + (g * 32 + p) * SPITCH + nt * 64 + h * 32);
+                sd[0] = in ? __builtin_bit_cast(uint4, o0) : uint4{0u, 0u, 0u, 0u};
+                sd[1] = in ? __builtin_bit_cast(uint4, o1) : uint4{0u, 0u, 0u, 0u};
+            }
             __half* dst = out + (((size_t)t.b * Ho + yo) * Wo + xo) * CO + 32 * nt + 16 * h;
             if (whole) {
                 reinterpret_cast<uint4*>(dst)[0] = __builtin_bit_cast(uint4, o0);
@@ -1502,12 +1571,19 @@
                 reinterpret_cast<uint4*>(dst)[1] = __builtin_bit_cast(uint4, o1);
             }
         }
-        plain_stores = whole ? (plain_stores < G::NBUF - 1 ? plain_stores + 1 : plain_stores) : 0;
+        if constexpr (GRAM) {
+            __syncthreads();
+            consume();
+        }
+        plain_stores = whole && !flushed ? (plain_stores < G::NBUF - 1 ? plain_stores + 1 : plain_stores) : 0;
         walk.advance();
         if (!walk.live) break;
         slot = slot + 1 == G::NBUF ? 0 : slot + 1;
     }
     asm volatile("s_waitcnt vmcnt(0)" ::: "memory");
+    if constexpr (GRAM) {
+        for (int f = gb; f < B; ++f) flush(f);
+    }
 }
 
 __global__ __launch_bounds__(256) void k_mst_conv_in_u8(const uint8_t* __restrict__ frame , const float* __restrict__ w ,
@@ -1989,3 +2065,32 @@
     AVX_HIP(ctx, hipGetLastError());
     return AVX_OK;
 }
+
+extern "C" int avx_mst_down4x4_gram(avx_ctx* ctx, const void* x, const void* wpack16, void* out, int B, int H, int W, const void* wqk16, float* gram, float* nq, float* nk,
+                                    int max_workgroups, void* stream) {
+    if (!ctx) return AVX_ERR_INVALID;
+    AVX_REQUIRE(ctx, x && wpack16 && out && wqk16 && gram && nq && nk && B > 0 && H > 0 && W > 0, "avx_mst_down4x4_gram: NULL pointer or empty tensor");
+    AVX_REQUIRE(ctx, H % 2 == 0 && W % 2 == 0, "avx_mst_down4x4_gram: H and W must be even (the model pads frames to multiples of 8)");
+    AVX_REQUIRE(ctx, (long)B * H * W * 32 * 2 < (1l << 31), "avx_mst_down4x4_gram: input larger than 2 GiB");
+    AVX_REQUIRE(ctx, ((((uintptr_t)x | (uintptr_t)wpack16 | (uintptr_t)out | (uintptr_t)wqk16)) & 15u) == 0, "avx_mst_down4x4_gram: pointers must be 16-byte aligned");
+    AVX_REQUIRE(ctx, max_workgroups >= 0 && max_workgroups <= 4096, "avx_mst_down4x4_gram: max_workgroups=%d (0 .. 4096)", max_workgroups);
+    AVX_HIP(ctx, hipSetDevice(ctx->device));
+    hipStream_t s = avx_pick_stream(ctx, stream);
+    avx_ws* ws = avx_workspace(ctx, s);
+    if (!ws) return AVX_ERR_NOMEM;
+    using G = DownGeo<32>;
+    const long total = (long)B * ((H / 2 + G::OH - 1) / G::OH) * ((W / 2 + G::OW - 1) / G::OW), cap = (long)ctx->num_cus;
+    const long blocks = max_workgroups > 0 ? max_workgroups : (total < cap ? total : cap);
+    const size_t per_frame = (size_t)blocks * 4 * 2 * 34 * 32;
+    int rc = avx_ensure_scratch(ctx, ws, sizeof(float) * per_frame * B);
+    if (rc) return rc;
+    float* partial = (float*)ws->d_scratch;
+    hipLaunchKernelGGL((k_mst_down4x4_dma<32, true>), dim3((unsigned)blocks), dim3(kFT), 0, s, (const __half*)x, (const uint4*)wpack16, (__half*)out, (const void*)ctx->d_zero, B, H, W,
+                       (int)AVX_TILE_ORDER_RASTER, (const uint4*)wqk16, partial);
+    AVX_HIP(ctx, hipGetLastError());
+    for (int f = 0; f < B; ++f) {
+        rc = avx_mst_qkv_final_launch(ctx, partial + per_frame * f, (int)blocks * 4, 2, gram + (size_t)f * 2 * 32 * 32, nq + (size_t)f * 64, nk + (size_t)f * 64, s);
+        if (rc) return rc;
+    }
+    return AVX_OK;
+}
diff --git a/animal-vision_amd/csrc/mst_mfma.hip b/animal-vision_amd/csrc/mst_mfma.hip
--- a/animal-vision_amd/csrc/mst_mfma.hip
+++ b/animal-vision_amd/csrc/mst_mfma.hip
@@ -640,35 +640,40 @@
     return AVX_OK;
 }
 
-template <int C, bool GRAM = false>
-__global__ __launch_bounds__(kT) void k_mst_convt2x2(const __half* __restrict__ x , const uint2* __restrict__ wpack ,
-                                                     const float* __restrict__ bias , const __half* __restrict__ skip ,
-                                                     const uint2* __restrict__ wskip , __half* __restrict__ out , int B,
-                                                     int H, int W, const uint4* __restrict__ wqk = nullptr , float* __restrict__ partial = nullptr ) {
-    constexpr int KS = C / 8, CO = C / 2, NT = CO / 32, KSS = CO / 8;
-    static_assert(!GRAM || C == 64, "the Gram epilogue is for the 32-channel output level");
+template <int C, bool GRAM = false, int NW = 4>
+__global__ __launch_bounds__(64 * NW) void k_mst_convt2x2(const __half* __restrict__ x , const uint2* __restrict__ wpack ,
+                                                         const float* __restrict__ bias , const __half* __restrict__ skip ,
+                                                         const uint2* __restrict__ wskip , __half* __restrict__ out , int B,
+                                                         int H, int W, const uint4* __restrict__ wqk = nullptr ,
+                                                         float* __restrict__ partial = nullptr ) {
+    constexpr int KS = C / 8, CO = C / 2, NT = CO / 32, KSS = CO / 8, HD = CO / 32, KQ = CO / 16, kTh = 64 * NW;
     extern __shared__ __align__(16) unsigned char smem[];
     uint2* wl = reinterpret_cast<uint2*>(smem);
     float* bl = reinterpret_cast<float*>(smem + (size_t)4 * NT * KS * 64 * sizeof(uint2));
     uint2* wsl = reinterpret_cast<uint2*>(bl + CO);
     uint4* wq = reinterpret_cast<uint4*>(wsl + NT * KSS * 64);
     const int tid = threadIdx.x, lane = tid & 63, wave = tid >> 6;
-    for (int i = tid; i < 4 * NT * KS * 64; i += kT) wl[i] = wpack[i];
-    for (int i = tid; i < CO; i += kT) bl[i] = bias[i];
+    for (int i = tid; i < 4 * NT * KS * 64; i += kTh) wl[i] = wpack[i];
+    for (int i = tid; i < CO; i += kTh) bl[i] = bias[i];
     if (skip)
-        for (int i = tid; i < NT * KSS * 64; i += kT) wsl[i] = wskip[i];
-    float16_t G;
-    float nq = 0.f, nk = 0.f;
+        for (int i = tid; i < NT * KSS * 64; i += kTh) wsl[i] = wskip[i];
+    float16_t G[HD];
+    float nq[HD], nk[HD];
     if constexpr (GRAM) {
-        for (int i = tid; i < 4 * 64; i += kT) wq[i] = wqk[i];
-#pragma unroll
-        for (int v = 0; v < 16; ++v) G[v] = 0.f;
+        for (int i = tid; i < 2 * HD * KQ * 64; i += kTh) wq[i] = wqk[i];
+#pragma unroll
+        for (int hd = 0; hd < HD; ++hd) {
+#pragma unroll
+            for (int v = 0; v < 16; ++v) G[hd][v] = 0.f;
+            nq[hd] = 0.f;
+            nk[hd] = 0.f;
+        }
     }
     __syncthreads();
     const int xt = (W + 31) / 32;
     const long total = (long)B * H * xt;
     const int p = lane & 31, h = lane >> 5;
-    for (long tile = (long)blockIdx.x * 4 + wave; tile < total; tile += (long)gridDim.x * 4) {
+    for (long tile = (long)blockIdx.x * NW + wave; tile < total; tile += (long)gridDim.x * NW) {
         const int x0 = (int)(tile % xt) * 32, y = (int)((tile / xt) % H);
         const long b = tile / ((long)xt * H);
         const int xw = x0 + p;
@@ -697,6 +702,7 @@
                     sf[2 * q + 1] = half4_t{h8[4], h8[5], h8[6], h8[7]};
                 }
             }
+            half8_t oh[GRAM ? KQ : 1];
 #pragma unroll
             for (int t = 0; t < NT; ++t) {
                 float16_t d;
@@ -713,28 +719,35 @@
                 for (int v = 0; v < 16; ++v) o[v] = (_Float16)(d[v] + bl[32 * t + 16 * h + v]);
                 if (xw < W) store_tile16(out + opix * CO + 32 * t + 16 * h, o);
                 if constexpr (GRAM) {
-                    half8_t o0, o1;
-#pragma unroll
-                    for (int v = 0; v < 8; ++v) { o0[v] = xw < W ? o[v] : (_Float16)0.f; o1[v] = xw < W ? o[8 + v] : (_Float16)0.f; }
+#pragma unroll
+                    for (int v = 0; v < 8; ++v) {
+                        oh[2 * t][v] = xw < W ? o[v] : (_Float16)0.f;
+                        oh[2 * t + 1][v] = xw < W ? o[8 + v] : (_Float16)0.f;
+                    }
+                }
+            }
+            if constexpr (GRAM) {
+#pragma unroll
+                for (int hd = 0; hd < HD; ++hd) {
                     float16_t dq, dk;
 #pragma unroll
                     for (int v = 0; v < 16; ++v) { dq[v] = 0.f; dk[v] = 0.f; }
-                    dq = mfma16(o0, __builtin_bit_cast(half8_t, wq[0 * 64 + lane]), dq);
-                    dq = mfma16(o1, __builtin_bit_cast(half8_t, wq[1 * 64 + lane]), dq);
-                    dk = mfma16(o0, __builtin_bit_cast(half8_t, wq[2 * 64 + lane]), dk);
-                    dk = mfma16(o1, __builtin_bit_cast(half8_t, wq[3 * 64 + lane]), dk);
+#pragma unroll
+                    for (int s = 0; s < KQ; ++s) dq = mfma16(oh[s], __builtin_bit_cast(half8_t, wq[(hd * KQ + s) * 64 + lane]), dq);
+#pragma unroll
+                    for (int s = 0; s < KQ; ++s) dk = mfma16(oh[s], __builtin_bit_cast(half8_t, wq[((HD + hd) * KQ + s) * 64 + lane]), dk);
                     unsigned aq[8], ak[8];
 #pragma unroll
                     for (int j = 0; j < 8; ++j) {
                         aq[j] = pack_f16(dq[2 * j], dq[2 * j + 1]);
                         ak[j] = pack_f16(dk[2 * j], dk[2 * j + 1]);
-                        fma_mix_lo(nq, aq[j], aq[j]); fma_mix_hi(nq, aq[j], aq[j]);
-                        fma_mix_lo(nk, ak[j], ak[j]); fma_mix_hi(nk, ak[j], ak[j]);
+                        fma_mix_lo(nq[hd], aq[j], aq[j]); fma_mix_hi(nq[hd], aq[j], aq[j]);
+                        fma_mix_lo(nk[hd], ak[j], ak[j]); fma_mix_hi(nk[hd], ak[j], ak[j]);
                     }
 #pragma unroll
                     for (int b2 = 0; b2 < 2; ++b2)
-                        G = mfma16(__builtin_bit_cast(half8_t, uint4{ak[4 * b2], ak[4 * b2 + 1], ak[4 * b2 + 2], ak[4 * b2 + 3]}),
-                                   __builtin_bit_cast(half8_t, uint4{aq[4 * b2], aq[4 * b2 + 1], aq[4 * b2 + 2], aq[4 * b2 + 3]}), G);
+                        G[hd] = mfma16(__builtin_bit_cast(half8_t, uint4{ak[4 * b2], ak[4 * b2 + 1], ak[4 * b2 + 2], ak[4 * b2 + 3]}),
+                                       __builtin_bit_cast(half8_t, uint4{aq[4 * b2], aq[4 * b2 + 1], aq[4 * b2 + 2], aq[4 * b2 + 3]}), G[hd]);
                 }
             }
         }
@@ -742,17 +755,20 @@
     if constexpr (GRAM) {
         __syncthreads();
         float* red = reinterpret_cast<float*>(smem);
-        float* mine = red + (size_t)wave * 34 * 32;
-#pragma unroll
-        for (int v = 0; v < 16; ++v) mine[(8 * (v / 4) + 4 * h + (v % 4)) * 32 + p] = G[v];
-        const float sq = nq + __shfl_xor(nq, 32), sk = nk + __shfl_xor(nk, 32);
-        if (h == 0) { mine[32 * 32 + p] = sq; mine[33 * 32 + p] = sk; }
+#pragma unroll
+        for (int hd = 0; hd < HD; ++hd) {
+            float* mine = red + ((size_t)wave * HD + hd) * 34 * 32;
+#pragma unroll
+            for (int v = 0; v < 16; ++v) mine[(8 * (v / 4) + 4 * h + (v % 4)) * 32 + p] = G[hd][v];
+            const float sq = nq[hd] + __shfl_xor(nq[hd], 32), sk = nk[hd] + __shfl_xor(nk[hd], 32);
+            if (h == 0) { mine[32 * 32 + p] = sq; mine[33 * 32 + p] = sk; }
+        }
         __syncthreads();
-        for (int i = tid; i < 34 * 32; i += kT) {
+        for (int i = tid; i < HD * 34 * 32; i += kTh) {
             float sum = 0.f;
 #pragma unroll
-            for (int w4 = 0; w4 < 4; ++w4) sum += red[(size_t)w4 * 34 * 32 + i];
-            partial[(size_t)blockIdx.x * 34 * 32 + i] = sum;
+            for (int w4 = 0; w4 < NW; ++w4) sum += red[(size_t)w4 * HD * 34 * 32 + i];
+            partial[(size_t)blockIdx.x * HD * 34 * 32 + i] = sum;
         }
     }
 }
@@ -940,6 +956,31 @@
     return AVX_OK;
 }
 
+template <int C, int NW, int PER_CU>
+static int convt2x2_gram_impl(avx_ctx* ctx, const void* x, const void* wpack, const float* bias, const void* skip, const void* wskip, void* out, int H, int W,
+                              const void* wqk, float* gram, float* nq, float* nk, void* stream) {
+    constexpr int CO = C / 2, NT = CO / 32, HD = CO / 32;
+    AVX_HIP(ctx, hipSetDevice(ctx->device));
+    hipStream_t s = avx_pick_stream(ctx, stream);
+    avx_ws* ws = avx_workspace(ctx, s);
+    if (!ws) return AVX_ERR_NOMEM;
+    const long total = (long)H * ((W + 31) / 32);
+    long blocks = (total + NW - 1) / NW;
+    const long cap = (long)ctx->num_cus * PER_CU;
+    if (blocks > cap) blocks = cap;
+    int rc = avx_ensure_scratch(ctx, ws, sizeof(float) * (size_t)blocks * HD * 34 * 32);
+    if (rc) return rc;
+    float* partial = (float*)ws->d_scratch;
+    size_t lds = (size_t)4 * NT * (C / 8) * 64 * sizeof(uint2) + sizeof(float) * CO + (size_t)NT * (CO / 8) * 64 * sizeof(uint2) + (size_t)2 * HD * (CO / 16) * 64 * sizeof(uint4);
+    if (lds < sizeof(float) * NW * HD * 34 * 32) lds = sizeof(float) * NW * HD * 34 * 32;
+    auto k = k_mst_convt2x2<C, true, NW>;
+    AVX_HIP(ctx, hipFuncSetAttribute((const void*)k, hipFuncAttributeMaxDynamicSharedMemorySize, (int)lds));
+    hipLaunchKernelGGL(k, dim3((unsigned)blocks), dim3(64 * NW), lds, s, (const __half*)x, (const uint2*)wpack, bias, (const __half*)skip, (const uint2*)wskip, (__half*)out, 1, H, W,
+                       (const uint4*)wqk, partial);
+    AVX_HIP(ctx, hipGetLastError());
+    return avx_mst_qkv_final_launch(ctx, partial, (int)blocks, HD, gram, nq, nk, s);
+}
+
 extern "C" {
 
 int avx_mst_qkv_gram(avx_ctx* ctx, const void* x, const void* wpack, size_t n_pix, int C, void* v_out, float* gram, float* nq, float* nk, void* stream) {
@@ -1092,25 +1133,15 @@
     AVX_REQUIRE(ctx, C == 64, "avx_mst_convt2x2_fuse_gram: C=%d (64 input channels: the decoder step back to full resolution)", C);
     AVX_REQUIRE(ctx, ((((uintptr_t)x | (uintptr_t)wpack | (uintptr_t)out | (uintptr_t)skip | (uintptr_t)wskip | (uintptr_t)wqk16)) & 15u) == 0,
                 "avx_mst_convt2x2_fuse_gram: pointers must be 16-byte aligned");
-    AVX_HIP(ctx, hipSetDevice(ctx->device));
-    hipStream_t s = avx_pick_stream(ctx, stream);
-    avx_ws* ws = avx_workspace(ctx, s);
-    if (!ws) return AVX_ERR_NOMEM;
-    const long total = (long)H * ((W + 31) / 32);
-    long blocks = (total + 3) / 4;
-    const long cap = (long)ctx->num_cus * 4;
-    if (blocks > cap) blocks = cap;
-    int rc = avx_ensure_scratch(ctx, ws, sizeof(float) * (size_t)blocks * 34 * 32);
-    if (rc) return rc;
-    float* partial = (float*)ws->d_scratch;
-    size_t lds = (size_t)4 * 1 * 8 * 64 * sizeof(uint2) + sizeof(float) * 32 + (size_t)1 * 4 * 64 * sizeof(uint2) + (size_t)4 * 64 * sizeof(uint4);
-    if (lds < sizeof(float) * 4 * 34 * 32) lds = sizeof(float) * 4 * 34 * 32;
-    auto k = k_mst_convt2x2<64, true>;
-    AVX_HIP(ctx, hipFuncSetAttribute((const void*)k, hipFuncAttributeMaxDynamicSharedMemorySize, (int)lds));
-    hipLaunchKernelGGL(k, dim3((unsigned)blocks), dim3(kT), lds, s, (const __half*)x, (const uint2*)wpack, bias, (const __half*)skip, (const uint2*)wskip, (__half*)out, 1, H, W,
-                       (const uint4*)wqk16, partial);
-    AVX_HIP(ctx, hipGetLastError());
-    return avx_mst_qkv_final_launch(ctx, partial, (int)blocks, 1, gram, nq, nk, s);
+    return convt2x2_gram_impl<64, 4, 4>(ctx, x, wpack, bias, skip, wskip, out, H, W, wqk16, gram, nq, nk, stream);
+}
+int avx_mst_convt2x2_fuse_gram128(avx_ctx* ctx, const void* x, const void* wpack, const float* bias, const void* skip, const void* wskip, void* out, int H, int W,
+                                  const void* wqk_tiles, float* gram, float* nq, float* nk, void* stream) {
+    if (!ctx) return AVX_ERR_INVALID;
+    AVX_REQUIRE(ctx, x && wpack && bias && skip && wskip && out && wqk_tiles && gram && nq && nk && H > 0 && W > 0, "avx_mst_convt2x2_fuse_gram128: NULL pointer or empty tensor");
+    AVX_REQUIRE(ctx, ((((uintptr_t)x | (uintptr_t)wpack | (uintptr_t)out | (uintptr_t)skip | (uintptr_t)wskip | (uintptr_t)wqk_tiles)) & 15u) == 0,
+                "avx_mst_convt2x2_fuse_gram128: pointers must be 16-byte aligned");
+    return convt2x2_gram_impl<128, 8, 1>(ctx, x, wpack, bias, skip, wskip, out, H, W, wqk_tiles, gram, nq, nk, stream);
 }
 static int convt2x2_impl(avx_ctx* ctx, const void* x, const void* wpack, const float* bias, const void* skip, const void* wskip, void* out, int B, int H, int W,
                          int C, void* stream) {
diff --git a/animal-vision_amd/ml/mst_plus_plus.py b/animal-vision_amd/ml/mst_plus_plus.py
--- a/animal-vision_amd/ml/mst_plus_plus.py
+++ b/animal-vision_amd/ml/mst_plus_plus.py
@@ -90,6 +90,24 @@
         q = torch.arange(K // 16, device=dev)
         j = torch.arange(8, device=dev)
         k = h[None, :, None] * (K // 2) + 8 * q[:, None, None] + j[None, None, :]
+        idx = (k[None] * N + col[:, None, :, None]).contiguous()
+        _FRAG_INDEX[key] = idx
+    return torch.take(wqkv.contiguous(), idx)
+
+
+def pack_qk16_tiles(wqkv: torch.Tensor) -> torch.Tensor:
+    K, N = wqkv.shape
+    assert N == 3 * K and K % 32 == 0
+    dev = wqkv.device
+    key = (K, N, "qk16t", str(dev))
+    idx = _FRAG_INDEX.get(key)
+    if idx is None:
+        lane = torch.arange(64, device=dev)
+        m, h = lane % 32, lane // 32
+        col = 32 * torch.arange(2 * K // 32, device=dev)[:, None] + m[None, :]
+        s = torch.arange(K // 16, device=dev)
+        j = torch.arange(8, device=dev)
+        k = 32 * (s[:, None, None] // 2) + 16 * h[None, :, None] + 8 * (s[:, None, None] % 2) + j[None, None, :]
         idx = (k[None] * N + col[:, None, :, None]).contiguous()
         _FRAG_INDEX[key] = idx
     return torch.take(wqkv.contiguous(), idx)
@@ -179,6 +197,7 @@
         self.FFN_FUSED_C = tuple(int(v) for v in os.environ.get("AVX_MST_FFN_FUSED_C", "32,64,128").split(",") if v)
         self._ffn_march = os.environ.get("AVX_MST_NO_FFN_MARCH", "") == ""
         self.FFN_MARCH_C = (32, 64)
+        self._resgram = os.environ.get("AVX_MST_NO_RESAMPLE_GRAM", "") == ""
         self._ctx = {}
 
     def ctx(self, device: torch.device):
@@ -268,17 +287,22 @@
         from .._lib import lib
 
         b, h, w, c = x.shape
-        assert c == 64 and skip.is_contiguous() and skip.shape == (b, 2 * h, 2 * w, 32)
+        co = c // 2
+        assert c in (64, 128) and skip.is_contiguous() and skip.shape == (b, 2 * h, 2 * w, co)
         x = x.contiguous()
-        out = torch.empty((b, 2 * h, 2 * w, 32), dtype=torch.float16, device=x.device)
-        g = torch.empty((b, 1, 32, 32), dtype=torch.float32, device=x.device)
-        nq = torch.empty((b, 32), dtype=torch.float32, device=x.device)
-        nk = torch.empty((b, 32), dtype=torch.float32, device=x.device)
+        out = torch.empty((b, 2 * h, 2 * w, co), dtype=torch.float16, device=x.device)
+        g = torch.empty((b, co // 32, 32, 32), dtype=torch.float32, device=x.device)
+        nq = torch.empty((b, co), dtype=torch.float32, device=x.device)
+        nk = torch.empty((b, co), dtype=torch.float32, device=x.device)
         ctx = self.ctx(x.device)
         st = torch.cuda.current_stream(x.device).cuda_stream
         for i in range(b):
-            ctx._check(lib.avx_mst_convt2x2_fuse_gram(ctx._h, x[i].data_ptr(), wpack.data_ptr(), bias.data_ptr(), skip[i].data_ptr(), wskip.data_ptr(), out[i].data_ptr(), h, w, c,
-                                                      wqk16.data_ptr(), g[i].data_ptr(), nq[i].data_ptr(), nk[i].data_ptr(), st))
+            if c == 64:
+                ctx._check(lib.avx_mst_convt2x2_fuse_gram(ctx._h, x[i].data_ptr(), wpack.data_ptr(), bias.data_ptr(), skip[i].data_ptr(), wskip.data_ptr(), out[i].data_ptr(), h, w, c,
+                                                          wqk16.data_ptr(), g[i].data_ptr(), nq[i].data_ptr(), nk[i].data_ptr(), st))
+            else:
+                ctx._check(lib.avx_mst_convt2x2_fuse_gram128(ctx._h, x[i].data_ptr(), wpack.data_ptr(), bias.data_ptr(), skip[i].data_ptr(), wskip.data_ptr(), out[i].data_ptr(), h, w,
+                                                             wqk16.data_ptr(), g[i].data_ptr(), nq[i].data_ptr(), nk[i].data_ptr(), st))
         return out, g, nq, nk
 
     def posemb(self, v: torch.Tensor, w1_c9: torch.Tensor, w2_c9: torch.Tensor, residual: torch.Tensor = None, bias: torch.Tensor = None) -> torch.Tensor:
@@ -329,6 +353,23 @@
         for i in range(0, b, per):
             ctx._check(lib.avx_mst_down4x4(ctx._h, x[i : i + per].data_ptr(), wpack16.data_ptr(), out[i : i + per].data_ptr(), min(per, b - i), h, w, c, st))
         return out
+
+    def down4x4_gram(self, x: torch.Tensor, wpack16: torch.Tensor, wqk16: torch.Tensor, max_workgroups: int = 0):
+        from .._lib import lib
+
+        b, h, w, c = x.shape
+        assert x.is_contiguous() and c == 32 and h % 2 == 0 and w % 2 == 0
+        out = torch.empty((b, h // 2, w // 2, 64), dtype=torch.float16, device=x.device)
+        g = torch.empty((b, 2, 32, 32), dtype=torch.float32, device=x.device)
+        nq = torch.empty((b, 64), dtype=torch.float32, device=x.device)
+        nk = torch.empty((b, 64), dtype=torch.float32, device=x.device)
+        ctx = self.ctx(x.device)
+        st = torch.cuda.current_stream(x.device).cuda_stream
+        per = max(1, (2**31 - 1) // (h * w * c * 2))
+        for i in range(0, b, per):
+            ctx._check(lib.avx_mst_down4x4_gram(ctx._h, x[i : i + per].data_ptr(), wpack16.data_ptr(), out[i : i + per].data_ptr(), min(per, b - i), h, w, wqk16.data_ptr(),
+                                                g[i : i + per].data_ptr(), nq[i : i + per].data_ptr(), nk[i : i + per].data_ptr(), max_workgroups, st))
+        return out, g, nq, nk
 
     def conv3x3_lds_gram(self, x: torch.Tensor, wpack16: torch.Tensor, add: torch.Tensor, wqk16: torch.Tensor):
         from .._lib import lib
@@ -850,10 +891,20 @@
         skips: List[torch.Tensor] = []
         heads = 1
         for i in range(2):
-            fea = self._msab(fea, f"{p}.encoder_layers.{i}.0", heads, pre if i == 0 else None)
+            fea = self._msab(fea, f"{p}.encoder_layers.{i}.0", heads, pre)
+            pre = None
             skips.append(fea)
             dkey = f"{p}.encoder_layers.{i}.1.weight"
             if _AVX.fused_ok(fea) and _AVX._down and fea.shape[-1] in (32, 64) and fea.is_contiguous():
+                if i == 0 and fea.shape[-1] == 32 and _AVX._resgram and _AVX._convgram and _AVX._qkv16 and _AVX._tail and _AVX._tailx:
+                    a1 = f"{p}.encoder_layers.1.0.blocks.0.0"
+                    wqkv1 = self._prep(a1 + ".qkv", lambda: torch.cat([self._w(a1 + ".to_q.weight", (0, 1)), self._w(a1 + ".to_k.weight", (0, 1)),
+                                                                       self._w(a1 + ".to_v.weight", (0, 1))], 0).t().contiguous())
+                    fea, g1, nq1, nk1 = _AVX.down4x4_gram(fea, self._prep(dkey + ".frag16", lambda: pack_down4x4(self._w(dkey, (0, 1)))),
+                                                          self._prep(a1 + ".qkv.frag16", lambda: pack_qkv16(wqkv1)))
+                    pre = (g1, nq1, nk1)
+                    heads *= 2
+                    continue
                 fea = _AVX.down4x4(fea, self._prep(dkey + ".frag16", lambda: pack_down4x4(self._w(dkey, (0, 1)))))
             else:
                 fea = self._conv_nhwc(fea, self._w(dkey, (0, 1)), stride=2, padding=1)
@@ -875,6 +926,13 @@
                     wqkv2 = self._prep(a2 + ".qkv", lambda: torch.cat([self._w(a2 + ".to_q.weight", (0, 1)), self._w(a2 + ".to_k.weight", (0, 1)),
                                                                        self._w(a2 + ".to_v.weight", (0, 1))], 0).t().contiguous())
                     wqk2 = self._prep(a2 + ".qkv.frag16", lambda: pack_qkv16(wqkv2))
+                    fea, g2, nq2, nk2 = _AVX.convt2x2_gram(fea, gt, gb, skips[1 - i].contiguous(), wbot_, wqk2)
+                    fea = self._msab(fea, f"{p}.decoder_layers.{i}.2", heads, (g2, nq2, nk2))
+                    continue
+                if ch == 64 and _AVX._resgram and _AVX._convgram and _AVX._qkv16 and _AVX._tail and _AVX._tailx:
+                    wqkv2 = self._prep(a2 + ".qkv", lambda: torch.cat([self._w(a2 + ".to_q.weight", (0, 1)), self._w(a2 + ".to_k.weight", (0, 1)),
+                                                                       self._w(a2 + ".to_v.weight", (0, 1))], 0).t().contiguous())
+                    wqk2 = self._prep(a2 + ".qk.frag16t", lambda: pack_qk16_tiles(wqkv2))
                     fea, g2, nq2, nk2 = _AVX.convt2x2_gram(fea, gt, gb, skips[1 - i].contiguous(), wbot_, wqk2)
                     fea = self._msab(fea, f"{p}.decoder_layers.{i}.2", heads, (g2, nq2, nk2))
                     continue
@@ -978,6 +1036,10 @@
     per_stage = 2 * msab(32) + 2 * msab(64) / 4 + msab(128) / 16
     if _AVX._convgram and _AVX._qkv16 and _AVX._tail and _AVX._tailx and _AVX._conv_lds and _AVX._upfuse:
         per_stage -= 2 * 64.0
+        if _AVX._resgram:
+            per_stage -= 128.0 / 4
+            if _AVX._down:
+                per_stage -= 128.0 / 4
     t32, t64, t128 = 64.0, 128.0 / 4, 256.0 / 16
     convs = (2 * t32) + (3 * t32)
     convs += (t32 + t64) + (t64 + t128)
diff --git a/include/avx.h b/include/avx.h
--- a/include/avx.h
+++ b/include/avx.h
@@ -375,7 +375,11 @@
                                  const void* wpack16, void* out, const void* wqk16, float* gram, float* nq, float* nk, void* stream);
 int avx_mst_convt2x2_fuse_gram(avx_ctx* ctx, const void* x, const void* wpack, const float* bias, const void* skip, const void* wskip, void* out, int H, int W, int C,
                                const void* wqk16, float* gram, float* nq, float* nk, void* stream);
+int avx_mst_convt2x2_fuse_gram128(avx_ctx* ctx, const void* x, const void* wpack, const float* bias, const void* skip, const void* wskip, void* out, int H, int W,
+                                  const void* wqk_tiles, float* gram, float* nq, float* nk, void* stream);
 int avx_mst_down4x4(avx_ctx* ctx, const void* x, const void* wpack16, void* out, int B, int H, int W, int C, void* stream);
+int avx_mst_down4x4_gram(avx_ctx* ctx, const void* x, const void* wpack16, void* out, int B, int H, int W, const void* wqk16, float* gram, float* nq, float* nk,
+                         int max_workgroups, void* stream);
 
 int avx_mst_attn_pack16(avx_ctx* ctx, const float* gram, const float* nq, const float* nk, const float* rescale, const float* wproj_t, int C, void* mpack,
                         void* stream);
```
